# fasion-image-generator-project/discogan_modernized

Measured on AMD Instinct MI355X. Metric: images/sec per DiscoGAN train step, higher is better.
Workload: dtype f32x3; 1 GPU; tops2hanbok discogan image_size=512 batch_size=32 per GPU (BASELINE configs[3]); D,G,G cycle, fwd+bwd+Adam, dead backward work skipped; fp32-accurate conv products on the bf16 matrix path: every fp32 operand carried as three bf16 planes (24 significand bits), exact bf16 x bf16 products, fp32 accumulation (no operand rounding); image_size=512, global_batch=32, parallelism=dp1, hipgraph=True, hip_streams=2, allreduce_overlap=False

## Files before the change

discogan_modernized_amd/_lib.py:

```python
from __future__ import annotations

import ctypes as C
import os

_HERE = os.path.dirname(os.path.abspath(__file__))
LIB_PATH = os.environ.get("DG_LIB") or os.path.join(_HERE, "libdiscogan_hip.so")

_p = C.c_void_p
_i = C.c_int
_f = C.c_float
_d = C.c_double
_z = C.c_size_t
_l = C.c_int64

SIGNATURES = {
    "dg_version": (_i, []),
    "dg_build_flags": (_i, []),
    "dg_last_error": (C.c_char_p, []),
    "dg_set_option": (_i, [C.c_char_p, _i]),
    "dg_conv_workspace_bytes": (_z, [_i, _i, _i, _i, _i, _i, _i, _i]),
    "dg_conv_fwd": (_i, [_p, _p, _p, _i, _i, _i, _i, _i, _i, _i, _p, _z, _p]),
    "dg_conv_dgrad": (_i, [_p, _p, _p, _i, _i, _i, _i, _i, _i, _i, _p, _z, _p]),
    "dg_conv_wgrad": (_i, [_p, _p, _p, _i, _i, _i, _i, _i, _i, _i, _i, _p, _z, _p]),
    "dg_conv_workspace_bytes_p": (_z, [_i, _i, _i, _i, _i, _i, _i, _i, _i, _i]),
    "dg_conv_bnstats_rows_p": (_i, [_i, _i, _i, _i, _i, _i, _i, _i, _i]),
    "dg_conv_plan_splits_p": (_i, [_i, _i, _i, _i, _i, _i, _i, _i, _i, _i]),
    "dg_conv_plan_describe": (_i, [_i, _i, _i, _i, _i, _i, _i, _i, _i, _i, _i, _i, C.POINTER(_i), _i]),
    "dg_conv_fwd_g": (_i, [_i, _p, _p, _p, _i, _i, _i, _i, _i, _i, _i, _i, _i, _p, _z, _p, _z, _p]),
    "dg_conv_dgrad_g": (_i, [_i, _p, _p, _p, _i, _i, _i, _i, _i, _i, _i, _i, _i, _p, _z, _p, _z, _p]),
    "dg_conv_wgrad_g": (_i, [_i, _i, _p, _p, _p, _i, _i, _i, _i, _i, _i, _i, _i, _i, _i, _p, _z, _p]),
    "dg_conv4x4s2_c3_fwd_p": (_i, [_p, _p, _p, _i, _i, _i, _i, _i, _i, _f, _i, _p]),
    "dg_conv4x4s2_c3_dgrad_p": (_i, [_p, _i, _p, _p, _i, _i, _i, _i, _i, _i, _p, _z, _p]),
    "dg_c3_dgrad_act_ok": (_i, [_i, _i, _i, _i, _i]),
    "dg_conv4x4s2_c3_dgrad_act_p": (_i, [_p, _i, _p, _i, _f, _p, _p, _i, _i, _i, _i, _i, _i, _p, _z, _p]),
    "dg_conv4x4s2_c3_wgrad_p": (_i, [_p, _p, _i, _i, _f, _p, _p, _i, _i, _i, _i, _i, _i, _p, _z, _p]),
    "dg_conv4x4s2_c3_fwd_g": (_i, [_i, _p, _p, _p, _i, _i, _i, _i, _i, _f, _i, _p]),
    "dg_conv4x4s2_c3_dgrad_g": (_i, [_i, _p, _p, _p, _i, _i, _i, _i, _i, _i, _p]),
    "dg_conv4x4s2_c3_wgrad_g": (_i, [_i, _i, _p, _p, _i, _f, _p, _p, _i, _i, _i, _i, _i, _i, _p, _z, _p]),
    "dg_bn_train_stats_g": (_i, [_i, _i, _p, _i, _i, _f, _f, _p, _p, _p, _p, _p, _z, _p]),
    "dg_bn_act_fwd_g": (_i, [_i, _p, _p, _i, _i, _p, _p, _p, _i, _f, _p]),
    "dg_bn_act_bwd_g": (_i, [_i, _i, _p, _p, _p, _i, _i, _p, _p, _p, _i, _f, _p, _p, _i, _p, _z, _p]),
    "dg_act_fwd_g": (_i, [_i, _p, _p, _z, _i, _f, _p]),
    "dg_act_bwd_g": (_i, [_i, _p, _p, _p, _z, _i, _f, _p]),
    "dg_mse_fwd_g": (_i, [_i, _p, _p, _z, _p, _p, _z, _p]),
    "dg_mse_bwd_g": (_i, [_i, _p, _p, _z, _p, _p, _p]),
    "dg_bce_fwd_g": (_i, [_i, _p, _i, _p, _p, _p]),
    "dg_bce_bwd_g": (_i, [_i, _p, _i, _p, _p, _p, _p]),
    "dg_fm_fwd_g": (_i, [_i, _p, _p, _i, _z, _p, _p, _p, _z, _p]),
    "dg_fm_bwd_g": (_i, [_i, _p, _i, _z, _p, _p, _p, _p]),
    "dg_conv_fwd_bias_act": (_i, [_p, _p, _p, _p, _i, _i, _i, _i, _i, _i, _i, _i, _f, _p, _z, _p]),
    "dg_conv_dgrad_bias_act": (_i, [_p, _p, _p, _p, _i, _i, _i, _i, _i, _i, _i, _i, _f, _p, _z, _p]),
    "dg_conv_plan_splits": (_i, [_i, _i, _i, _i, _i, _i, _i, _i]),
    "dg_conv_bnstats_rows": (_i, [_i, _i, _i, _i, _i, _i, _i, _i]),
    "dg_conv_fwd_bnstats": (_i, [_p, _p, _p, _i, _i, _i, _i, _i, _p, _z, _p, _z, _p]),
    "dg_conv_dgrad_bnstats": (_i, [_p, _p, _p, _i, _i, _i, _i, _i, _p, _z, _p, _z, _p]),
    "dg_conv4x4s2_fwd": (_i, [_p, _p, _p, _i, _i, _i, _i, _i, _p, _z, _p]),
    "dg_conv4x4s2_dgrad": (_i, [_p, _p, _p, _i, _i, _i, _i, _i, _p, _z, _p]),
    "dg_conv4x4s2_wgrad": (_i, [_p, _p, _p, _i, _i, _i, _i, _i, _i, _p, _z, _p]),
    "dg_conv4x4_valid_fwd": (_i, [_p, _p, _p, _i, _i, _i, _p, _z, _p]),
    "dg_conv4x4_valid_dgrad": (_i, [_p, _p, _p, _i, _i, _i, _p, _z, _p]),
    "dg_conv4x4_valid_wgrad": (_i, [_p, _p, _p, _i, _i, _i, _i, _p, _z, _p]),
    "dg_convT4x4s2_fwd": (_i, [_p, _p, _p, _i, _i, _i, _i, _i, _p, _z, _p]),
    "dg_convT4x4s2_dgrad": (_i, [_p, _p, _p, _i, _i, _i, _i, _i, _p, _z, _p]),
    "dg_convT4x4s2_wgrad": (_i, [_p, _p, _p, _i, _i, _i, _i, _i, _i, _p, _z, _p]),
    "dg_convT4x4_1to4_fwd": (_i, [_p, _p, _p, _i, _i, _i, _p, _z, _p]),
    "dg_convT4x4_1to4_dgrad": (_i, [_p, _p, _p, _i, _i, _i, _p, _z, _p]),
    "dg_convT4x4_1to4_wgrad": (_i, [_p, _p, _p, _i, _i, _i, _i, _p, _z, _p]),
    "dg_conv4x4s2_c3_fwd": (_i, [_p, _p, _p, _i, _i, _i, _i, _i, _f, _p]),
    "dg_c3_dgrad_workspace_bytes": (_z, [_i]),
    "dg_conv4x4s2_c3_dgrad": (_i, [_p, _p, _p, _i, _i, _i, _i, _i, _p, _z, _p]),
    "dg_c3_wgrad_workspace_bytes": (_z, [_i, _i, _i, _i]),
    "dg_conv4x4s2_c3_wgrad": (_i, [_p, _p, _p, _i, _i, _i, _i, _i, _p, _z, _p]),
    "dg_conv4x4s2_c3_wgrad_act": (_i, [_p, _p, _i, _f, _p, _p, _i, _i, _i, _i, _i, _p, _z, _p]),
    "dg_bn_workspace_bytes": (_z, [_i, _i]),
    "dg_bn_train_stats": (_i, [_p, _i, _i, _f, _f, _p, _p, _p, _p, _p, _z, _p]),
    "dg_bn_partials_workspace_bytes": (_z, [_i, _i]),
    "dg_bn_stats_from_partials": (_i, [_p, _i, _i, _i, _f, _f, _p, _p, _p, _p, _p, _z, _p]),
    "dg_bn_act_fwd": (_i, [_p, _p, _i, _i, _p, _p, _p, _i, _f, _p]),
    "dg_bn_act_bwd": (_i, [_p, _p, _p, _i, _i, _p, _p, _p, _i, _f, _p, _p, _i, _p, _z, _p]),
    "dg_act_fwd": (_i, [_p, _p, _z, _i, _f, _p]),
    "dg_act_bwd": (_i, [_p, _p, _p, _z, _i, _f, _p]),
    "dg_loss_workspace_bytes": (_z, []),
    "dg_mse_fwd": (_i, [_p, _p, _z, _p, _p, _z, _p]),
    "dg_mse_bwd": (_i, [_p, _p, _z, _p, _p, _p]),
    "dg_bce_fwd": (_i, [_p, _i, _f, _p, _p, _z, _p]),
    "dg_bce_bwd": (_i, [_p, _i, _f, _p, _p, _p]),
    "dg_fm_workspace_bytes": (_z, [_i, _z]),
    "dg_fm_fwd": (_i, [_p, _p, _i, _z, _p, _p, _p, _z, _p]),
    "dg_fm_bwd": (_i, [_p, _i, _z, _p, _p, _p, _p]),
    "dg_debug_igemm_stamps": (_i, [_p, _z]),
    "dg_device_cu_count": (_i, []),
    "dg_loss_mix_fwd": (_i, [_p, _p, _i, _f, _i, _p]),
    "dg_loss_mix_bwd": (_i, [_p, _p, _i, _f, _i, _i, _p]),
    "dg_adam_advance": (_i, [_p, _d, _d, _d, _p]),
    "dg_adam_step_flat": (_i, [_p, _p, _p, _p, _z, _p, _f, _f, _f, _f, _f, _p]),
    "dg_ema_update_flat": (_i, [_p, _p, _z, _f, _p]),
    "dg_swap_flat": (_i, [_p, _p, _z, _p]),
    "dg_grad_stats_workspace_bytes": (_z, []),
    "dg_grad_sumsq_partial": (_i, [_p, _z, _p, _z, _i, C.POINTER(_i), _p]),
    "dg_grad_clip_finalize": (_i, [_p, _i, _d, _d, _i, _p, _p]),
    "dg_adam_advance_c": (_i, [_p, _d, _d, _d, _p, _p]),
    "dg_adam_step_flat_c": (_i, [_p, _p, _p, _p, _z, _p, _f, _f, _f, _f, _p, _p, _i, _z, _p]),
    "dg_bce_target_fwd": (_i, [_p, _p, _i, _p, _p]),
    "dg_bce_target_bwd": (_i, [_p, _p, _i, _p, _p, _p]),
    "dg_hinge_fwd": (_i, [_p, _p, _z, _f, _p, _p, _z, _p]),
    "dg_hinge_bwd": (_i, [_p, _p, _z, _f, _p, _p, _p]),
    "dg_dp_ready": (_i, [_p]),
    "dg_dp_unique_id_bytes": (_i, []),
    "dg_dp_get_unique_id": (_i, [_p, _z]),
    "dg_dp_init": (_i, [_i, _i, _p, _z]),
    "dg_dp_world_size": (_i, []),
    "dg_dp_rank": (_i, []),
    "dg_dp_allreduce_sum": (_i, [_p, _z, _p]),
    "dg_dp_allreduce_max": (_i, [_p, _z, _p]),
    "dg_dp_broadcast": (_i, [_p, _z, _i, _p]),
    "dg_dp_barrier": (_i, [_p, _p]),
    "dg_dp_destroy": (_i, []),
    "dg_u8hwc_to_f32chw": (_i, [_p, _p, _i, _i, _i, _i, _p]),
    "dg_image_prep": (_i, [_p, _p, _i, _i, _i, _i, _i, _i, _i, _i, _p]),
    "dg_sample_grid_u8": (_i, [_p, _i, _i, _i, _i, _i, _p, _p]),
    "dg_image_metrics_workspace_bytes": (_z, [_i, _i]),
    "dg_image_metrics": (_i, [_p, _p, _i, _i, _p, _p, _z, _p]),
    "dg_adam_step_flat_bf16": (_i, [_p, _p, _p, _p, _z, _p, _f, _f, _f, _f, _f, _p, _p]),
    "dg_f32_to_bf16": (_i, [_p, _p, _z, _p]),
    "dg_bn_act_fwd_bf16": (_i, [_p, _p, _p, _i, _i, _p, _p, _p, _i, _f, _p]),
    "dg_bn_act_bwd_bf16": (_i, [_p, _p, _p, _p, _i, _i, _p, _p, _p, _i, _f, _p, _p, _i, _p, _z, _p]),
    "dg_conv_bf16_operands_ok": (_i, [_i, _i, _i, _i, _i, _i, _i, _i]),
    "dg_f32_to_bf16x3": (_i, [_p, _p, _z, _z, _p]),
    "dg_adam_step_flat_x3": (_i, [_p, _p, _p, _p, _z, _p, _f, _f, _f, _f, _f, _p, _z, _p]),
    "dg_conv4x4s2_c3_fwd_x3": (_i, [_p, _p, _p, _p, _z, _i, _i, _i, _i, _i, _f, _p]),
    "dg_conv_x3_planes_ok": (_i, [_i, _i, _i, _i, _i, _i, _i, _i]),
    "dg_bn_act_fwd_x3": (_i, [_p, _p, _p, _z, _i, _i, _i, _p, _p, _p, _i, _f, _p]),
    "dg_bn_act_bwd_x3": (_i, [_p, _p, _p, _p, _z, _i, _i, _i, _p, _p, _p, _i, _f, _p, _p, _i, _p, _z, _p]),
    "dg_conv_x3_bnstats_rows": (_i, [_i, _i, _i, _i, _i, _i, _i, _i]),
    "dg_conv_fwd_x3": (_i, [_p, _l, _p, _l, _i, _p, _i, _i, _i, _i, _i, _i, _i, _p, _z, _p, _z, _p]),
    "dg_x3_transpose_planes": (_i, [_p, _p, _z, _p, _p, _p, _i, _p]),
    "dg_conv_dgrad_x3": (_i, [_p, _l, _i, _p, _l, _p, _i, _i, _i, _i, _i, _i, _i, _p, _z, _p, _z, _p]),
    "dg_conv_wgrad_x3": (_i, [_p, _l, _i, _p, _l, _p, _i, _i, _i, _i, _i, _i, _i, _i, _p, _z, _p]),
    "dg_conv_mixed_bnstats_rows": (_i, [_i, _i, _i, _i, _i, _i, _i, _i, _i, _i]),
    "dg_conv_fwd_mixed": (_i, [_p, _i, _p, _i, _p, _i, _i, _i, _i, _i, _i, _i, _i, _p, _z, _p, _z, _p]),
    "dg_conv_dgrad_mixed": (_i, [_p, _i, _p, _i, _p, _i, _i, _i, _i, _i, _i, _i, _i, _p, _z, _p, _z, _p]),
    "dg_bn_train_stats_t": (_i, [_p, _i, _i, _i, _f, _f, _p, _p, _p, _p, _p, _z, _p]),
    "dg_bn_act_fwd_t": (_i, [_p, _p, _i, _i, _i, _p, _p, _p, _i, _f, _p]),
    "dg_bn_act_bwd_t": (_i, [_p, _p, _p, _i, _i, _i, _p, _p, _p, _i, _f, _p, _p, _i, _p, _z, _p]),
    "dg_act_bwd_t": (_i, [_p, _p, _p, _i, _z, _i, _f, _p]),
    "dg_conv4x4s2_c3_fwd_t": (_i, [_p, _p, _p, _i, _i, _i, _i, _i, _i, _f, _p]),
    "dg_conv4x4s2_c3_dgrad_t": (_i, [_p, _i, _p, _p, _i, _i, _i, _i, _i, _p, _z, _p]),
    "dg_conv4x4s2_c3_wgrad_t": (_i, [_p, _p, _i, _i, _f, _p, _p, _i, _i, _i, _i, _i, _p, _z, _p]),
    "dg_fm_fwd_t": (_i, [_p, _p, _i, _i, _z, _p, _p, _p, _z, _p]),
    "dg_fm_bwd_t": (_i, [_p, _i, _z, _p, _p, _p, _i, _p]),
    "dg_conv_wgrad_mixed": (_i, [_p, _i, _p, _i, _p, _i, _i, _i, _i, _i, _i, _i, _i, _p, _z, _p]),
    "dg_nchw_to_nhwc": (_i, [_p, _p, _i, _i, _i, _i, _p]),
    "dg_nhwc_to_nchw": (_i, [_p, _p, _i, _i, _i, _i, _p]),
}

_lib = None


class DiscoganHipError(RuntimeError):
    pass


def load():
    global _lib
    if _lib is not None:
        return _lib
    if not os.path.exists(LIB_PATH):
        raise DiscoganHipError(
            f"{LIB_PATH} not found: the HIP kernel library is not built. "
            "Run `python -m discogan_modernized_amd.build` (hipcc --offload-arch=gfx950). "
            "There is no CPU fallback for the product path.")
    import torch
    lib = C.CDLL(LIB_PATH)
    for name, (res, args) in SIGNATURES.items():
        fn = getattr(lib, name)
        fn.restype = res
        fn.argtypes = args
    _lib = lib
    for key, val in os.environ.items():
        if key.startswith("DG_OPT_"):
            rc = lib.dg_set_option(key[7:].lower().encode(), int(val))
            if rc != 0:
                raise DiscoganHipError(f"bad option {key}: " + lib.dg_last_error().decode())
    return lib


def check(rc, what=""):
    if rc != 0:
# ... 7 lines not shown
```

discogan_modernized_amd/csrc/dg_common.h:

```cpp
#pragma once
#include <hip/hip_runtime.h>
#include <stdint.h>
#include <stdio.h>
#include <stdarg.h>
#include "../../include/discogan_hip.h"

typedef float f32x4 __attribute__((ext_vector_type(4)));
typedef float f32x16 __attribute__((ext_vector_type(16)));
typedef __bf16 dg_bf16x4_t __attribute__((ext_vector_type(4)));

extern thread_local char dg_err_buf[512];
int dg_fail(int code, const char* fmt, ...);

#define DG_CHECK_ARG(cond, ...)                                   \
    do {                                                          \
        if (!(cond)) return dg_fail(DG_ERR_INVALID, __VA_ARGS__); \
    } while (0)

#define DG_CHECK_LAUNCH(name)                                                                    \
    do {                                                                                         \
        hipError_t e__ = hipGetLastError();                                                      \
        if (e__ != hipSuccess) return dg_fail(DG_ERR_HIP, "%s: %s", name, hipGetErrorString(e__)); \
    } while (0)

static inline int dg_ilog2(int v) {
    int l = 0;
    while ((1 << l) < v) ++l;
    return l;
}
static inline bool dg_is_pow2(int v) { return v > 0 && (v & (v - 1)) == 0; }
static inline size_t dg_align_up(size_t v, size_t a) { return (v + a - 1) / a * a; }

int dg_get_option(int idx);
enum { DG_OPT_SPLITK = 0, DG_OPT_KT = 1, DG_OPT_TARGET_WGS = 2, DG_OPT_RESERVED = 3, DG_OPT_SPLIT_BELOW = 4, DG_OPT_POINTER_PATH = 5, DG_OPT_BF16 = 6, DG_OPT_DBG_ZERO = 7, DG_OPT_NO_DMA = 8, DG_OPT_DMA_MFMA = 9, DG_OPT_X3_MFMA = 10, DG_OPT_DGW_PERSIST = 11, DG_OPT_UNDERSTORY = 12, DG_OPT_BN_ITEMS = 13, DG_OPT_COUNT = 14 };
static inline int dg_resolve_prec(int prec) { return prec >= 0 ? prec : dg_get_option(DG_OPT_BF16); }
__attribute__((visibility("hidden"))) void dg_c3_fwd_tiled(const float* x_nchw, const float* w, float* y_nhwc, int N, int H, int W, int K, int act,
                                                           float slope, bool wide, hipStream_t st);

struct DgPtrs {
    const void* p[DG_MAX_GROUPS];
};
static inline DgPtrs dg_ptrs(const void* const* arr, int n) {
    DgPtrs r;
    for (int i = 0; i < DG_MAX_GROUPS; ++i) r.p[i] = (arr != nullptr && i < n) ? arr[i] : nullptr;
    return r;
}
static inline DgPtrs dg_ptrs1(const void* p0) {
    DgPtrs r;
    for (int i = 0; i < DG_MAX_GROUPS; ++i) r.p[i] = nullptr;
    r.p[0] = p0;
    return r;
}
template <typename T>
__device__ __forceinline__ T* dg_pick(const DgPtrs& t, int g) { return (T*)t.p[g]; }

__device__ __forceinline__ float dg_wave_sum(float v) {
#pragma unroll
    for (int off = 32; off > 0; off >>= 1) v += __shfl_down(v, off, 64);
    return v;
}
__device__ __forceinline__ double dg_wave_sum_d(double v) {
#pragma unroll
    for (int off = 32; off > 0; off >>= 1) v += __shfl_down(v, off, 64);
    return v;
}

__device__ __forceinline__ float dg_block_sum256(float v, float* red ) {
    v = dg_wave_sum(v);
    const int lane = threadIdx.x & 63, w = threadIdx.x >> 6;
    if (lane == 0) red[w] = v;
    __syncthreads();
    float r = 0.f;
    if (threadIdx.x == 0) r = red[0] + red[1] + red[2] + red[3];
    __syncthreads();
    return r;
}

__device__ __forceinline__ float dg_apply_act(float u, int act, float slope) {
    if (act == DG_ACT_LEAKY) return u > 0.f ? u : u * slope;
    if (act == DG_ACT_RELU) return u > 0.f ? u : 0.f;
    if (act == DG_ACT_SIGMOID) return 1.f / (1.f + __expf(-u));
    return u;
}

__device__ __forceinline__ void dg_split3(const f32x4& v, dg_bf16x4_t& hi, dg_bf16x4_t& mid, dg_bf16x4_t& lo) {
    hi = __builtin_convertvector(v, dg_bf16x4_t);
    const f32x4 r = v - __builtin_convertvector(hi, f32x4);
    mid = __builtin_convertvector(r, dg_bf16x4_t);
    lo = __builtin_convertvector(r - __builtin_convertvector(mid, f32x4), dg_bf16x4_t);
}
```

discogan_modernized_amd/csrc/edge.hip:

```cpp
#include "dg_common.h"
#include <type_traits>

__device__ float dg_zero_edge[64];

__device__ __forceinline__ int tap_of(int parity, int d) {
    if (parity == 0) return d == 0 ? 1 : (d == -1 ? 3 : -1);
    return d == 0 ? 2 : (d == 1 ? 0 : -1);
}

__global__ __launch_bounds__(256) void c3_dgrad_valu_kernel(const float* __restrict__ dy, const float* __restrict__ w,
                                                            float* __restrict__ dx, int N, int H, int W, int K,
                                                            int lgHo, int lgWo, int act) {
    const int Ho = H >> 1, Wo = W >> 1;
    const long nquad = (long)N * Ho * Wo;
    const long q = (long)blockIdx.x * 256 + threadIdx.x;
    if (q >= nquad) return;
    const int b = (int)(q & (Wo - 1)), a = (int)((q >> lgWo) & (Ho - 1)), n = (int)(q >> (lgWo + lgHo));
    float acc[3][2][2];
#pragma unroll
    for (int c = 0; c < 3; ++c) acc[c][0][0] = acc[c][0][1] = acc[c][1][0] = acc[c][1][1] = 0.f;
    const float* base = dy + ((long)(n * Ho + a) * Wo + b) * K;
    for (int k0 = 0; k0 < K; k0 += 4) {
        f32x4 g[3][3];
#pragma unroll
        for (int da = -1; da <= 1; ++da)
#pragma unroll
            for (int db = -1; db <= 1; ++db) {
                const bool ok = (unsigned)(a + da) < (unsigned)Ho && (unsigned)(b + db) < (unsigned)Wo;
                g[da + 1][db + 1] = ok ? *(const f32x4*)(base + (long)(da * Wo + db) * K + k0)
                                       : (f32x4){0.f, 0.f, 0.f, 0.f};
            }
#pragma unroll
        for (int kk = 0; kk < 4; ++kk) {
            const float* wk = w + (long)(k0 + kk) * 48;
#pragma unroll
            for (int c = 0; c < 3; ++c)
#pragma unroll
                for (int ph = 0; ph < 2; ++ph)
#pragma unroll
                    for (int ty = 0; ty < 2; ++ty) {
                        const int r = ph == 0 ? (ty == 0 ? 1 : 3) : (ty == 0 ? 2 : 0);
                        const int da = ph == 0 ? (ty == 0 ? 0 : -1) : (ty == 0 ? 0 : 1);
#pragma unroll
                        for (int pw = 0; pw < 2; ++pw)
#pragma unroll
                            for (int tx = 0; tx < 2; ++tx) {
                                const int s = pw == 0 ? (tx == 0 ? 1 : 3) : (tx == 0 ? 2 : 0);
                                const int db = pw == 0 ? (tx == 0 ? 0 : -1) : (tx == 0 ? 0 : 1);
                                acc[c][ph][pw] += g[da + 1][db + 1][kk] * wk[c * 16 + r * 4 + s];
                            }
                    }
        }
    }
#pragma unroll
    for (int c = 0; c < 3; ++c)
#pragma unroll
        for (int ph = 0; ph < 2; ++ph) {
            float v0 = acc[c][ph][0], v1 = acc[c][ph][1];
            if (act == DG_ACT_SIGMOID) {
                v0 = 1.f / (1.f + expf(-v0));
                v1 = 1.f / (1.f + expf(-v1));
            }
            *(float2*)(dx + ((long)(n * 3 + c) * H + 2 * a + ph) * W + 2 * b) = make_float2(v0, v1);
        }
}

#define CD_K 64
#define CD_TR 4
#define CD_TC 16
#define CD_PR (CD_TR + 2)
#define CD_PC (CD_TC + 2)
#define CD_LDP 66
#define CD_NK (9 * CD_K)

__global__ __launch_bounds__(256) void c3_wq_build_kernel(const float* __restrict__ w, float* __restrict__ wq) {
    const int e = blockIdx.x * 256 + threadIdx.x;
    if (e >= CD_NK * 16) return;
    const int col = e & 15, row = e >> 4;
    const int k = row & (CD_K - 1), nb = row >> 6;
    const int da = nb / 3 - 1, db = nb % 3 - 1;
    float v = 0.f;
    if (col < 12) {
        const int c = col >> 2, ph = (col >> 1) & 1, pw = col & 1;
        const int r = tap_of(ph, da), s = tap_of(pw, db);
        if (r >= 0 && s >= 0) v = w[(k * 3 + c) * 16 + r * 4 + s];
    }
    wq[e] = v;
}

#define CD_NV ((CD_PR * CD_PC * (CD_K / 4) + 255) / 256)
__global__ __launch_bounds__(256, 2) void c3_dgrad_mfma_kernel(const float* __restrict__ dy, const float* __restrict__ wq,
                                                               float* __restrict__ dx, int N, int H, int W, int act,
                                                               int tiles_r, int tiles_c, int ntiles) {
    __shared__ __attribute__((aligned(16))) float WqS[CD_NK * 16];
    __shared__ __attribute__((aligned(16))) float dyS[CD_PR * CD_PC * CD_LDP];
    __shared__ float outS[CD_TR][16 * 17];
    const int tid = threadIdx.x, lane = tid & 63, wave = tid >> 6;
    const int Ho = H >> 1, Wo = W >> 1;
    for (int e = tid; e < CD_NK * 4; e += 256) *(f32x4*)(WqS + e * 4) = *(const f32x4*)(wq + e * 4);

    f32x4 pre[CD_NV];
    auto prefetch = [&](int t) {
        const int tc = t % tiles_c, tr = (t / tiles_c) % tiles_r, n = t / (tiles_c * tiles_r);
        const int a0 = tr * CD_TR, b0 = tc * CD_TC;
#pragma unroll
        for (int i = 0; i < CD_NV; ++i) {
            const int idx = tid + i * 256;
            const int q4 = idx & (CD_K / 4 - 1), pix = idx >> 4;
            const int pr = pix / CD_PC, pc = pix - pr * CD_PC;
            const int a = a0 - 1 + pr, b = b0 - 1 + pc;
            const bool ok = idx < CD_PR * CD_PC * (CD_K / 4) && t < ntiles &&
                            (unsigned)a < (unsigned)Ho && (unsigned)b < (unsigned)Wo;
            pre[i] = ok ? *(const f32x4*)(dy + ((long)(n * Ho + a) * Wo + b) * CD_K + q4 * 4) : (f32x4){0.f, 0.f, 0.f, 0.f};
        }
    };
    const int bq = lane & 15, kk = lane >> 4;
    prefetch(blockIdx.x);
    for (int t = blockIdx.x; t < ntiles; t += gridDim.x) {
        const int tc = t % tiles_c, tr = (t / tiles_c) % tiles_r, n = t / (tiles_c * tiles_r);
        const int a0 = tr * CD_TR, b0 = tc * CD_TC;
        __syncthreads();
#pragma unroll
        for (int i = 0; i < CD_NV; ++i) {
            const int idx = tid + i * 256;
            if (idx < CD_PR * CD_PC * (CD_K / 4)) {
                float* d = dyS + (idx >> 4) * CD_LDP + (idx & (CD_K / 4 - 1)) * 4;
                *(float2*)d = make_float2(pre[i][0], pre[i][1]);
                *(float2*)(d + 2) = make_float2(pre[i][2], pre[i][3]);
            }
        }
        __syncthreads();
        prefetch(t + gridDim.x);
        f32x4 acc0 = {0.f, 0.f, 0.f, 0.f}, acc1 = {0.f, 0.f, 0.f, 0.f};
#pragma unroll
        for (int nb = 0; nb < 9; ++nb) {
            const int da = nb / 3 - 1, db = nb % 3 - 1;
            const float* ap = dyS + ((wave + 1 + da) * CD_PC + bq + 1 + db) * CD_LDP + kk;
            const float* bp = WqS + (nb * CD_K + kk) * 16 + bq;
#pragma unroll
            for (int ks = 0; ks < CD_K / 4; ks += 2) {
                acc0 = __builtin_amdgcn_mfma_f32_16x16x4f32(ap[ks * 4], bp[ks * 64], acc0, 0, 0, 0);
                acc1 = __builtin_amdgcn_mfma_f32_16x16x4f32(ap[ks * 4 + 4], bp[ks * 64 + 64], acc1, 0, 0, 0);
            }
        }
#pragma unroll
        for (int r = 0; r < 4; ++r) outS[wave][bq * 17 + kk * 4 + r] = acc0[r] + acc1[r];
        __syncthreads();
        const int a = a0 + wave;
        const int ph = lane >> 5, x = lane & 31;
        const int qd = x >> 1, pw = x & 1;
        if (a < Ho && b0 + qd < Wo) {
#pragma unroll
            for (int c = 0; c < 3; ++c) {
                float v = outS[wave][(c * 4 + ph * 2 + pw) * 17 + qd];
                if (act == DG_ACT_SIGMOID) v = 1.f / (1.f + expf(-v));
                dx[((long)(n * 3 + c) * H + 2 * a + ph) * W + 2 * b0 + x] = v;
            }
        }
    }
}

#define CS_TR 6
#define CS_TC 14
#define CS_PR (CS_TR + 2)
#define CS_PC 16
#define CS_LDP 52
template <bool IN16, bool MF16 = false, bool X3 = false, bool FACT = false>
__global__ __launch_bounds__(256, 2) void c3_dgrad_scatter_kernel(const DgPtrs dys, const DgPtrs ws_, const DgPtrs dxs, int N, int H, int W, int act,
                                                                  int tiles_r, int tiles_c, int ntiles, unsigned dybytes, const DgPtrs aos, float slope) {
    const float* __restrict__ dy = dg_pick<const float>(dys, blockIdx.y);
    const float* __restrict__ w = dg_pick<const float>(ws_, blockIdx.y);
    float* __restrict__ dx = dg_pick<float>(dxs, blockIdx.y);
    static_assert(!MF16 || IN16, "the bf16 MFMA form takes a bf16 dy");
    static_assert(!X3 || (!IN16 && !MF16), "the f32x3 form takes an fp32 dy");
    typedef __bf16 bf16x8_d __attribute__((ext_vector_type(8)));
    typedef float f32x8_d __attribute__((ext_vector_type(8)));
    __shared__ __attribute__((aligned(16))) float Ps[CS_PR * CS_PC * CS_LDP];
    const int tid = threadIdx.x, lane = tid & 63, wave = tid >> 6;
    const int p = lane & 15, kq = lane >> 4;
    const int Ho = H >> 1, Wo = W >> 1;
    float breg[3][(MF16 || X3) ? 1 : 16];
    bf16x8_d breg16[3][2];
    bf16x8_d breg3[X3 ? 3 : 1][3][2];
    auto split8 = [](const f32x8_d& v, bf16x8_d* pl) {
        pl[0] = __builtin_convertvector(v, bf16x8_d);
        const f32x8_d r1 = v - __builtin_convertvector(pl[0], f32x8_d);
        pl[1] = __builtin_convertvector(r1, bf16x8_d);
        pl[2] = __builtin_convertvector(r1 - __builtin_convertvector(pl[1], f32x8_d), bf16x8_d);
    };
#pragma unroll
    for (int blk = 0; blk < 3; ++blk) {
        if constexpr (X3) {
#pragma unroll
            for (int st = 0; st < 2; ++st) {
                f32x8_d t;
#pragma unroll
                for (int j = 0; j < 8; ++j) t[j] = w[(32 * st + 8 * kq + j) * 48 + blk * 16 + p];
                bf16x8_d pl[3];
                split8(t, pl);
#pragma unroll
                for (int q = 0; q < 3; ++q) breg3[q][blk][st] = pl[q];
            }
        } else if constexpr (MF16) {
#pragma unroll
            for (int st = 0; st < 2; ++st) {
                f32x8_d t;
#pragma unroll
                for (int j = 0; j < 8; ++j) t[j] = w[(32 * st + 8 * kq + j) * 48 + blk * 16 + p];
                breg16[blk][st] = __builtin_convertvector(t, bf16x8_d);
            }
        } else {
#pragma unroll
            for (int s = 0; s < 16; ++s) breg[blk][s] = w[(16 * kq + s) * 48 + blk * 16 + p];
        }
    }
    const __amdgpu_buffer_rsrc_t rdy = __builtin_amdgcn_make_buffer_rsrc((void*)dy, 0, (int)dybytes, 0x00020000);
    const __amdgpu_buffer_rsrc_t rao = __builtin_amdgcn_make_buffer_rsrc((void*)(FACT ? dg_pick<const float>(aos, blockIdx.y) : dy), 0, (int)dybytes, 0x00020000);
    constexpr int OOR = (int)0x80000000;
    f32x4 areg[2][2][4];
    f32x4 oreg[FACT ? 2 : 1][4];
    auto apply_act = [&](int set) {
        if constexpr (FACT) {
#pragma unroll
            for (int g = 0; g < 2; ++g)
#pragma unroll
                for (int j = 0; j < (IN16 ? 2 : 4); ++j)
#pragma unroll
                    for (int e = 0; e < 4; ++e) {
                        if constexpr (IN16) {
                            const unsigned dv = __float_as_uint(areg[set][g][j][e]), ov = __float_as_uint(oreg[g][j][e]);
                            float d0 = __builtin_bit_cast(float, dv << 16), d1 = __builtin_bit_cast(float, dv & 0xffff0000u);
                            d0 = __builtin_bit_cast(float, ov << 16) > 0.f ? d0 : d0 * slope;
                            d1 = __builtin_bit_cast(float, ov & 0xffff0000u) > 0.f ? d1 : d1 * slope;
                            typedef __bf16 bf16x2_a __attribute__((ext_vector_type(2)));
                            typedef float f32x2_a __attribute__((ext_vector_type(2)));
                            areg[set][g][j][e] = __uint_as_float(__builtin_bit_cast(unsigned, __builtin_convertvector((f32x2_a){d0, d1}, bf16x2_a)));
                        } else {
                            const float d = areg[set][g][j][e];
                            areg[set][g][j][e] = oreg[g][j][e] > 0.f ? d : d * slope;
                        }
                    }
        }
    };
    auto fetch = [&](int t, int set) {
        const int tc = t % tiles_c, tr = (t / tiles_c) % tiles_r, n = t / (tiles_c * tiles_r);
#pragma unroll
        for (int g = 0; g < 2; ++g) {
            const int a = tr * CS_TR - 1 + wave + 4 * g, b = tc * CS_TC - 1 + p;
            const bool ok = t < ntiles && (unsigned)a < (unsigned)Ho && (unsigned)b < (unsigned)Wo;
            const int off = ok ? (((n * Ho + a) * Wo + b) * CD_K + ((MF16 || X3) ? 8 : 16) * kq) * (IN16 ? 2 : 4) : OOR;
#pragma unroll
            for (int j = 0; j < (IN16 ? 2 : 4); ++j) {
                const int o = off + (X3 ? 128 * (j >> 1) + 16 * (j & 1) : (MF16 ? 64 : 16) * j);
                areg[set][g][j] = __builtin_bit_cast(f32x4, __builtin_amdgcn_raw_buffer_load_b128(rdy, o, 0, 0));
                if constexpr (FACT) oreg[g][j] = __builtin_bit_cast(f32x4, __builtin_amdgcn_raw_buffer_load_b128(rao, o, 0, 0));
            }
        }
    };
    fetch(blockIdx.x, 0);
    apply_act(0);
    auto tile = [&](auto SB, int t) {
        constexpr int S = decltype(SB)::value;
        const int tc = t % tiles_c, tr = (t / tiles_c) % tiles_r, n = t / (tiles_c * tiles_r);
        const int a0 = tr * CS_TR, b0 = tc * CS_TC;
        fetch(t + gridDim.x, S ^ 1);
        f32x4 acc[2][3];
#pragma unroll
        for (int g = 0; g < 2; ++g)
#pragma unroll
            for (int blk = 0; blk < 3; ++blk) acc[g][blk] = (f32x4){0.f, 0.f, 0.f, 0.f};
        if constexpr (X3) {
            constexpr int PA[6] = {2, 0, 1, 1, 0, 0}, PB[6] = {0, 2, 1, 0, 1, 0};
#pragma unroll
            for (int st = 0; st < 2; ++st)
#pragma unroll
                for (int g = 0; g < 2; ++g) {
                    const f32x4 v0 = areg[S][g][2 * st], v1 = areg[S][g][2 * st + 1];
                    bf16x8_d apl[3];
                    split8((f32x8_d){v0[0], v0[1], v0[2], v0[3], v1[0], v1[1], v1[2], v1[3]}, apl);
#pragma unroll
                    for (int blk = 0; blk < 3; ++blk)
#pragma unroll
                        for (int q = 0; q < 6; ++q)
                            acc[g][blk] = __builtin_amdgcn_mfma_f32_16x16x32_bf16(apl[PA[q]], breg3[PB[q]][blk][st], acc[g][blk], 0, 0, 0);
                }
        } else if constexpr (MF16) {
#pragma unroll
            for (int st = 0; st < 2; ++st)
#pragma unroll
                for (int g = 0; g < 2; ++g)
#pragma unroll
                    for (int blk = 0; blk < 3; ++blk)
                        acc[g][blk] = __builtin_amdgcn_mfma_f32_16x16x32_bf16(__builtin_bit_cast(bf16x8_d, areg[S][g][st]), breg16[blk][st],
                                                                              acc[g][blk], 0, 0, 0);
        } else
#pragma unroll
        for (int s = 0; s < 16; ++s)
#pragma unroll
            for (int g = 0; g < 2; ++g)
#pragma unroll
                for (int blk = 0; blk < 3; ++blk)
                {
                    float av;
                    if constexpr (IN16) {
                        const float fv = areg[S][g][s >> 3][(s >> 1) & 3];
                        const unsigned wv = __float_as_uint(fv);
                        av = __builtin_bit_cast(float, (s & 1) ? (wv & 0xffff0000u) : (wv << 16));
                    } else {
                        av = areg[S][g][s >> 2][s & 3];
                    }
                    acc[g][blk] = __builtin_amdgcn_mfma_f32_16x16x4f32(av, breg[blk][s], acc[g][blk], 0, 0, 0);
                }
        __syncthreads();
#pragma unroll
        for (int g = 0; g < 2; ++g)
#pragma unroll
            for (int blk = 0; blk < 3; ++blk)
#pragma unroll
                for (int j = 0; j < 4; ++j) Ps[((wave + 4 * g) * CS_PC + 4 * kq + j) * CS_LDP + blk * 16 + p] = acc[g][blk][j];
        __syncthreads();
        for (int e = tid; e < 3 * 2 * CS_TR * 2 * CS_TC; e += 256) {
            const int xx = e % (2 * CS_TC), yy = (e / (2 * CS_TC)) % (2 * CS_TR), c = e / (4 * CS_TR * CS_TC);
            const int y = 2 * a0 + yy, x = 2 * b0 + xx;
            const int ph = yy & 1, pw = xx & 1, la = (yy >> 1) + 1, lb = (xx >> 1) + 1;
            const int ra2 = la - 1 + 2 * ph, rr1 = 1 + ph, rr2 = 3 - 3 * ph;
            const int cb2 = lb - 1 + 2 * pw, ss1 = 1 + pw, ss2 = 3 - 3 * pw;
            const float* pc = Ps + c * 16;
            float v = pc[(la * CS_PC + lb) * CS_LDP + rr1 * 4 + ss1] + pc[(la * CS_PC + cb2) * CS_LDP + rr1 * 4 + ss2] +
                      pc[(ra2 * CS_PC + lb) * CS_LDP + rr2 * 4 + ss1] + pc[(ra2 * CS_PC + cb2) * CS_LDP + rr2 * 4 + ss2];
            if (act == DG_ACT_SIGMOID) v = 1.f / (1.f + expf(-v));
            if (y < H && x < W) dx[((long)(n * 3 + c) * H + y) * W + x] = v;
        }
        apply_act(S ^ 1);
    };
    for (int t = blockIdx.x; t < ntiles; t += 2 * gridDim.x) {
        tile(std::integral_constant<int, 0>{}, t);
        if (t + (int)gridDim.x < ntiles) tile(std::integral_constant<int, 1>{}, t + gridDim.x);
    }
}

extern "C" size_t dg_c3_dgrad_workspace_bytes(int K) { return K == CD_K ? (size_t)CD_NK * 16 * sizeof(float) : 0; }

using C3Yes = std::true_type;
using C3No = std::false_type;
template <typename F> static void c3_with_flag(bool b, F&& f) { if (b) f(C3Yes{}); else f(C3No{}); }
template <typename F> static void c3_with_fwd_act(int act, F&& f) {
    if (act == DG_ACT_LEAKY) f(std::integral_constant<int, DG_ACT_LEAKY>{});
    else if (act == DG_ACT_RELU) f(std::integral_constant<int, DG_ACT_RELU>{});
    else f(std::integral_constant<int, DG_ACT_NONE>{});
}
#define C3_CHECK_PREC(who, prec) DG_CHECK_ARG((prec) >= DG_PREC_DEFAULT && (prec) <= DG_PREC_F32X3, who ": prec=%d", prec)

struct C3Dgrad {
    const char* who;
    int groups;
    bool grouped;
    const void *const *dy, *const *w;
    void* const* dx;
    int dy_bf16, N, H, W, K, act, prec;
    const void* act_out;
    float slope;
    void* ws;
    size_t ws_bytes;
    hipStream_t st;
};
static C3Dgrad c3_dgrad_call(const char* who, const void* const* dy, int dy_bf16, const float* const* w, float* const* dx, int N, int H, int W, int K,
                             int act, int prec, void* ws, size_t ws_bytes, dg_stream_t stream) {
    C3Dgrad c = C3Dgrad();
    c.who = who; c.groups = 1; c.dy = dy; c.dy_bf16 = dy_bf16; c.w = (const void* const*)w; c.dx = (void* const*)dx;
    c.N = N; c.H = H; c.W = W; c.K = K; c.act = act; c.prec = dg_resolve_prec(prec);
    c.ws = ws; c.ws_bytes = ws_bytes; c.st = (hipStream_t)stream;
    return c;
}
static int c3_dgrad(const C3Dgrad& c);
extern "C" int dg_conv4x4s2_c3_dgrad(const float* dy_nhwc, const float* w, float* dx_nchw, int N, int H, int W, int K,
                                     int act, void* ws, size_t ws_bytes, dg_stream_t stream) {
    return c3_dgrad(c3_dgrad_call("dg_conv4x4s2_c3_dgrad", (const void* const*)&dy_nhwc, 0, &w, &dx_nchw, N, H, W, K, act, DG_PREC_DEFAULT, ws, ws_bytes,
                                  stream));
}
extern "C" int dg_conv4x4s2_c3_dgrad_t(const void* dy_nhwc, int dy_bf16, const float* w, float* dx_nchw, int N, int H, int W, int K,
                                       int act, void* ws, size_t ws_bytes, dg_stream_t stream) {
    return c3_dgrad(c3_dgrad_call("dg_conv4x4s2_c3_dgrad_t", &dy_nhwc, dy_bf16, &w, &dx_nchw, N, H, W, K, act, DG_PREC_DEFAULT, ws, ws_bytes, stream));
}
extern "C" int dg_conv4x4s2_c3_dgrad_p(const void* dy_nhwc, int dy_bf16, const float* w, float* dx_nchw, int N, int H, int W, int K,
                                       int act, int prec, void* ws, size_t ws_bytes, dg_stream_t stream) {
    C3_CHECK_PREC("dg_conv4x4s2_c3_dgrad_p", prec);
    return c3_dgrad(c3_dgrad_call("dg_conv4x4s2_c3_dgrad_p", &dy_nhwc, dy_bf16, &w, &dx_nchw, N, H, W, K, act, prec, ws, ws_bytes, stream));
}
extern "C" int dg_conv4x4s2_c3_dgrad_act_p(const void* dy_nhwc, int dy_bf16, const void* act_out, int in_act, float slope, const float* w, float* dx_nchw,
                                           int N, int H, int W, int K, int act, int prec, void* ws, size_t ws_bytes, dg_stream_t stream) {
    C3_CHECK_PREC("dg_conv4x4s2_c3_dgrad_act_p", prec);
    DG_CHECK_ARG(act_out && in_act == DG_ACT_LEAKY, "dg_conv4x4s2_c3_dgrad_act_p: needs the saved output of a fused LeakyReLU (in_act=%d)", in_act);
    C3Dgrad c = c3_dgrad_call("dg_conv4x4s2_c3_dgrad_act_p", &dy_nhwc, dy_bf16, &w, &dx_nchw, N, H, W, K, act, prec, ws, ws_bytes, stream);
    c.act_out = act_out; c.slope = slope;
    return c3_dgrad(c);
}
extern "C" int dg_conv4x4s2_c3_dgrad_g(int groups, const float* const* dy_nhwc, const float* const* w, float* const* dx_nchw, int N, int H, int W, int K,
                                       int act, int prec, dg_stream_t stream) {
    C3_CHECK_PREC("dg_conv4x4s2_c3_dgrad_g", prec);
    C3Dgrad c = c3_dgrad_call("dg_conv4x4s2_c3_dgrad_g", (const void* const*)dy_nhwc, 0, w, dx_nchw, N, H, W, K, act, prec, nullptr, 0, stream);
    c.groups = groups; c.grouped = true;
    return c3_dgrad(c);
}

static bool c3_dgrad_scatter_fits(int N, int H, int W, int K, int dy_bf16) {
    return K == CD_K && N >= 1 && (long)N * (H / 2) * (W / 2) * CD_K * (dy_bf16 ? 2 : 4) < (1L << 31);
}
extern "C" int dg_c3_dgrad_act_ok(int N, int H, int W, int K, int dy_bf16) {
    return c3_dgrad_scatter_fits(N, H, W, K, dy_bf16) && dg_get_option(DG_OPT_KT) != 16 ? 1 : 0;
}
enum C3DgradForm { C3_DGRAD_SCATTER, C3_DGRAD_GATHER, C3_DGRAD_VALU };
static C3DgradForm c3_dgrad_form(const C3Dgrad& c) {
    if (!c3_dgrad_scatter_fits(c.N, c.H, c.W, c.K, c.dy_bf16)) return C3_DGRAD_VALU;
    return dg_get_option(DG_OPT_KT) != 16 ? C3_DGRAD_SCATTER : C3_DGRAD_GATHER;
}
static int c3_dgrad(const C3Dgrad& c) {
    const int N = c.N, H = c.H, W = c.W, K = c.K, Ho = H / 2, Wo = W / 2;
    DG_CHECK_ARG(c.groups >= 1 && c.groups <= DG_MAX_GROUPS && c.dy && c.w && c.dx, "%s: bad group / null table", c.who);
    for (int i = 0; i < c.groups; ++i) DG_CHECK_ARG(c.dy[i] && c.w[i] && c.dx[i], "%s: null pointer", c.who);
    DG_CHECK_ARG(!c.grouped || (K == CD_K && dg_get_option(DG_OPT_KT) != 16), "%s: the grouped form is the scatter kernel (K == 64, option kt != 16)", c.who);
    DG_CHECK_ARG(!c.dy_bf16 || (K == CD_K && dg_get_option(DG_OPT_KT) != 16), "%s: a bf16 dy needs K == 64 (scatter form)", c.who);
    DG_CHECK_ARG(N >= 1 && K >= 4 && K % 4 == 0, "%s: bad N/K (%d,%d)", c.who, N, K);
    DG_CHECK_ARG(dg_is_pow2(H) && dg_is_pow2(W) && H >= 2 && W >= 2, "%s: H,W must be powers of two", c.who);
    DG_CHECK_ARG(c.act == DG_ACT_NONE || c.act == DG_ACT_SIGMOID, "%s: bad act %d", c.who, c.act);
    DG_CHECK_ARG((long)N * 3 * H * W < (1L << 31), "%s: tensor too large", c.who);
    const C3DgradForm form = c3_dgrad_form(c);
    if (form != C3_DGRAD_SCATTER) {
        DG_CHECK_ARG(c.groups == 1 && !c.act_out, "%s: several problems and the fused form are the scatter kernel (K == 64, dy under 2^31 bytes, option kt != 16)",
                     c.who);
        DG_CHECK_ARG(!c.dy_bf16, "%s: the VALU form reads an fp32 dy (a bf16 dy of %ld bytes is past the scatter form's 2^31)", c.who, (long)N * Ho * Wo * K * 2);
    }
    switch (form) {
    case C3_DGRAD_SCATTER: {
        const int tiles_r = (Ho + CS_TR - 1) / CS_TR, tiles_c = (Wo + CS_TC - 1) / CS_TC;
        const long ntiles = (long)N * tiles_r * tiles_c;
        const dim3 grid((unsigned)(ntiles < 512 ? ntiles : 512), c.groups);
        const DgPtrs pd = dg_ptrs(c.dy, c.groups), pw = dg_ptrs(c.w, c.groups), px = dg_ptrs(c.dx, c.groups);
        const DgPtrs pa = dg_ptrs1(c.act_out ? c.act_out : c.dy[0]);
        const unsigned dyb = (unsigned)((long)N * Ho * Wo * CD_K * (c.dy_bf16 ? 2 : 4));
        auto scatter = [&](auto IN16, auto MF16, auto X3) {
            c3_with_flag(c.act_out != nullptr, [&](auto FACT) {
                hipLaunchKernelGGL((c3_dgrad_scatter_kernel<decltype(IN16)::value, decltype(MF16)::value, decltype(X3)::value, decltype(FACT)::value>), grid,
                                   dim3(256), 0, c.st, pd, pw, px, N, H, W, c.act, tiles_r, tiles_c, (int)ntiles, dyb, pa, c.slope);
            });
        };
        if (c.dy_bf16 && c.prec == DG_PREC_BF16) scatter(C3Yes{}, C3Yes{}, C3No{});
        else if (c.dy_bf16) scatter(C3Yes{}, C3No{}, C3No{});
        else if (c.prec == DG_PREC_F32X3) scatter(C3No{}, C3No{}, C3Yes{});
        else scatter(C3No{}, C3No{}, C3No{});
        break;
    }
    case C3_DGRAD_GATHER: {
        const int tiles_r = (Ho + CD_TR - 1) / CD_TR, tiles_c = (Wo + CD_TC - 1) / CD_TC;
        const long ntiles = (long)N * tiles_r * tiles_c;
        if (c.ws == nullptr || c.ws_bytes < dg_c3_dgrad_workspace_bytes(K))
            return dg_fail(DG_ERR_WORKSPACE, "%s: workspace %zu < %zu", c.who, c.ws_bytes, dg_c3_dgrad_workspace_bytes(K));
        hipLaunchKernelGGL(c3_wq_build_kernel, dim3((CD_NK * 16 + 255) / 256), dim3(256), 0, c.st, (const float*)c.w[0], (float*)c.ws);
        DG_CHECK_LAUNCH("c3_wq_build");
        hipLaunchKernelGGL(c3_dgrad_mfma_kernel, dim3((unsigned)(ntiles < 512 ? ntiles : 512)), dim3(256), 0, c.st, (const float*)c.dy[0], (const float*)c.ws,
                           (float*)c.dx[0], N, H, W, c.act, tiles_r, tiles_c, (int)ntiles);
        break;
    }
    case C3_DGRAD_VALU: {
        const long nquad = (long)N * Ho * Wo;
        hipLaunchKernelGGL(c3_dgrad_valu_kernel, dim3((unsigned)((nquad + 255) / 256)), dim3(256), 0, c.st, (const float*)c.dy[0], (const float*)c.w[0],
                           (float*)c.dx[0], N, H, W, K, dg_ilog2(Ho), dg_ilog2(Wo), c.act);
        break;
    }
    }
    DG_CHECK_LAUNCH(c.who);
    return DG_OK;
}

#define CF_K 64
#define CF_S 24
template <int ACT, bool OUT16>
__global__ __launch_bounds__(256, 2) void c3_fwd_mfma_kernel(const DgPtrs xs, const DgPtrs ws_, const DgPtrs ys, int N, int H, int W, int lgHo, int lgWo,
                                                             long npix, int ngroups, float slope, int xbytes) {
    const float* __restrict__ x = dg_pick<const float>(xs, blockIdx.y);
    const float* __restrict__ w = dg_pick<const float>(ws_, blockIdx.y);
    float* __restrict__ y = dg_pick<float>(ys, blockIdx.y);
    const int lane = threadIdx.x & 63;
    const int p = lane & 31, h = lane >> 5;
    const int Ho = H >> 1, Wo = W >> 1;
    const int wave = blockIdx.x * 4 + (threadIdx.x >> 6), nwaves = gridDim.x * 4;
    const float* const zp = dg_zero_edge;
    __shared__ float wS[CF_K * 49];
    for (int e = threadIdx.x; e < CF_K * 48; e += 256) wS[(e / 48) * 49 + e % 48] = w[e];
    __syncthreads();
    float wb[2][CF_S];
#pragma unroll
    for (int nb = 0; nb < 2; ++nb)
#pragma unroll
        for (int s = 0; s < CF_S; ++s) {
            const int c = s >> 3, r = (s >> 1) & 3, q = 2 * (s & 1) + h;
            wb[nb][s] = wS[(OUT16 ? 2 * p + nb : nb * 32 + p) * 49 + c * 16 + r * 4 + q];
        }
    float a[2][CF_S];
    const __amdgpu_buffer_rsrc_t rx = __builtin_amdgcn_make_buffer_rsrc((void*)x, 0, xbytes, 0x00020000);
    const int HW4 = H * W * 4;
    constexpr int BIG = 0x40000000;
    auto gather = [&](int g, float* dst) {
        const int pix = g * 32 + p;
        const bool okp = g < ngroups && pix < (int)npix;
        const int ox = pix & (Wo - 1), oy = (pix >> lgWo) & (Ho - 1), n = pix >> (lgWo + lgHo);
        const int base = n * 3 * HW4;
        int colb[2];
#pragma unroll
        for (int j = 0; j < 2; ++j) {
            const int ix = 2 * ox - 1 + 2 * j + h;
            colb[j] = (unsigned)ix < (unsigned)W ? ix * 4 : BIG;
        }
#pragma unroll
        for (int r = 0; r < 4; ++r) {
            const int iy = 2 * oy - 1 + r;
            const int rowb = (okp && (unsigned)iy < (unsigned)H) ? base + iy * W * 4 : BIG;
#pragma unroll
            for (int j = 0; j < 2; ++j) {
                const int voff = rowb + colb[j];
#pragma unroll
                for (int c = 0; c < 3; ++c)
                    dst[c * 8 + r * 2 + j] = __builtin_bit_cast(float, __builtin_amdgcn_raw_buffer_load_b32(rx, voff, c * HW4, 0));
            }
        }
    };
    int g = wave;
    if (g < ngroups) gather(g, a[0]);
    auto body = [&](auto PB, int gcur) {
        constexpr int P = decltype(PB)::value;
        gather(gcur + nwaves, a[P ^ 1]);
        f32x16 acc0 = {0.f}, acc1 = {0.f};
#pragma unroll
        for (int s = 0; s < CF_S; ++s) {
            acc0 = __builtin_amdgcn_mfma_f32_32x32x2f32(a[P][s], wb[0][s], acc0, 0, 0, 0);
            acc1 = __builtin_amdgcn_mfma_f32_32x32x2f32(a[P][s], wb[1][s], acc1, 0, 0, 0);
        }
        const long pix0 = (long)gcur * 32;
        if constexpr (OUT16) {
            typedef __bf16 bf16x2_e __attribute__((ext_vector_type(2)));
            typedef float f32x2_e __attribute__((ext_vector_type(2)));
            unsigned* o16 = (unsigned*)((__bf16*)y + (pix0 + h * 4) * CF_K + 2 * p);
            const bool whole = pix0 + 32 <= npix;
#pragma unroll
            for (int v = 0; v < 16; ++v) {
                const int i = (v >> 2) * 8 + (v & 3);
                const f32x2_e pr = {dg_apply_act(acc0[v], ACT, slope), dg_apply_act(acc1[v], ACT, slope)};
                if (whole || pix0 + h * 4 + i < npix)
                    o16[i * (CF_K / 2)] = __builtin_bit_cast(unsigned, __builtin_convertvector(pr, bf16x2_e));
            }
            return;
        }
        float* o = y + (pix0 + h * 4) * CF_K + p;
        if (pix0 + 32 <= npix) {
#pragma unroll
            for (int v = 0; v < 16; ++v) {
                const int i = (v >> 2) * 8 + (v & 3);
                o[i * CF_K] = dg_apply_act(acc0[v], ACT, slope);
                o[i * CF_K + 32] = dg_apply_act(acc1[v], ACT, slope);
            }
        } else {
#pragma unroll
            for (int v = 0; v < 16; ++v) {
                const int i = (v >> 2) * 8 + (v & 3);
                if (pix0 + h * 4 + i < npix) {
                    o[i * CF_K] = dg_apply_act(acc0[v], ACT, slope);
                    o[i * CF_K + 32] = dg_apply_act(acc1[v], ACT, slope);
                }
            }
        }
    };
    for (; g < ngroups; g += 2 * nwaves) {
        body(std::integral_constant<int, 0>{}, g);
        if (g + nwaves < ngroups) body(std::integral_constant<int, 1>{}, g + nwaves);
    }
}

typedef __bf16 bf16x8_e __attribute__((ext_vector_type(8)));
typedef float f32x8_e __attribute__((ext_vector_type(8)));
typedef float f32x2_g __attribute__((ext_vector_type(2)));
template <int ACT, bool OUT16, bool X3 = false, bool PL = false>
__global__ __launch_bounds__(256, 2) void c3_fwd_bf16mfma_kernel(const DgPtrs xs, const DgPtrs ws_, const DgPtrs ys, int N, int H, int W, int lgHo, int lgWo,
                                                                 long npix, int ngroups, float slope, int xbytes,
                                                                 __bf16* __restrict__ planes = nullptr, long pstride = 0) {
    const float* __restrict__ x = dg_pick<const float>(xs, blockIdx.y);
    const float* __restrict__ w = dg_pick<const float>(ws_, blockIdx.y);
    float* __restrict__ y = dg_pick<float>(ys, blockIdx.y);
    static_assert(!PL || (X3 && !OUT16), "planes are written by the f32x3 form with an fp32 output");
    const int lane = threadIdx.x & 63;
    const int p = lane & 31, h = lane >> 5;
    const int Ho = H >> 1, Wo = W >> 1;
    const int wave = blockIdx.x * 4 + (threadIdx.x >> 6), nwaves = gridDim.x * 4;
    constexpr int NPL = X3 ? 3 : 1;
    bf16x8_e wb[NPL][2][3];
    auto split8 = [](const f32x8_e& v, bf16x8_e* pl) {
        pl[0] = __builtin_convertvector(v, bf16x8_e);
        if constexpr (X3) {
            const f32x8_e r1 = v - __builtin_convertvector(pl[0], f32x8_e);
            pl[1] = __builtin_convertvector(r1, bf16x8_e);
            pl[2] = __builtin_convertvector(r1 - __builtin_convertvector(pl[1], f32x8_e), bf16x8_e);
// ... 67 lines not shown
            for (int v = 0; v < 16; ++v) {
                const int i = (v >> 2) * 8 + (v & 3);
                const f32x2_e pr = {dg_apply_act(acc0[v], ACT, slope), dg_apply_act(acc1[v], ACT, slope)};
                if (whole || pix0 + h * 4 + i < npix)
                    o16[i * (CF_K / 2)] = __builtin_bit_cast(unsigned, __builtin_convertvector(pr, bf16x2_e));
            }
        } else if constexpr (PL) {
            typedef __bf16 bf16x2_p __attribute__((ext_vector_type(2)));
            typedef float f32x2_p __attribute__((ext_vector_type(2)));
            float* o = y + (pix0 + h * 4) * CF_K + 2 * p;
            __bf16* pb = planes + (pix0 + h * 4) * CF_K + 2 * p;
#pragma unroll
            for (int v = 0; v < 16; ++v) {
                const int i = (v >> 2) * 8 + (v & 3);
                if (whole || pix0 + h * 4 + i < npix) {
                    const f32x2_p pr = {dg_apply_act(acc0[v], ACT, slope), dg_apply_act(acc1[v], ACT, slope)};
                    *(f32x2_p*)(o + i * CF_K) = pr;
                    const bf16x2_p hi2 = __builtin_convertvector(pr, bf16x2_p);
                    const f32x2_p r1 = pr - __builtin_convertvector(hi2, f32x2_p);
                    const bf16x2_p mid2 = __builtin_convertvector(r1, bf16x2_p);
                    const bf16x2_p lo2 = __builtin_convertvector(r1 - __builtin_convertvector(mid2, f32x2_p), bf16x2_p);
                    *(bf16x2_p*)(pb + i * CF_K) = hi2;
                    *(bf16x2_p*)(pb + pstride + i * CF_K) = mid2;
                    *(bf16x2_p*)(pb + 2 * pstride + i * CF_K) = lo2;
                }
            }
        } else {
            float* o = y + (pix0 + h * 4) * CF_K + p;
#pragma unroll
            for (int v = 0; v < 16; ++v) {
                const int i = (v >> 2) * 8 + (v & 3);
                if (whole || pix0 + h * 4 + i < npix) {
                    o[i * CF_K] = dg_apply_act(acc0[v], ACT, slope);
                    o[i * CF_K + 32] = dg_apply_act(acc1[v], ACT, slope);
                }
            }
        }
    };
    for (; g < ngroups; g += 2 * nwaves) {
        body(std::integral_constant<int, 0>{}, g);
        if (g + nwaves < ngroups) body(std::integral_constant<int, 1>{}, g + nwaves);
    }
}

struct C3Fwd {
    const char* who;
    int groups;
    bool streaming_only;
    const void *const *x, *const *w;
    void* const* y;
    void* planes;
    size_t plane_elems;
    int y_bf16, N, H, W, K, act, prec;
    float slope;
    hipStream_t st;
};
static C3Fwd c3_fwd_call(const char* who, const float* const* x, const float* const* w, void* const* y, int y_bf16, int N, int H, int W, int K, int act,
                         float slope, int prec, dg_stream_t stream) {
    C3Fwd c = C3Fwd();
    c.who = who; c.groups = 1; c.x = (const void* const*)x; c.w = (const void* const*)w; c.y = y; c.y_bf16 = y_bf16;
    c.N = N; c.H = H; c.W = W; c.K = K; c.act = act; c.slope = slope; c.prec = dg_resolve_prec(prec); c.st = (hipStream_t)stream;
    return c;
}
static int c3_fwd(const C3Fwd& c);
extern "C" int dg_conv4x4s2_c3_fwd(const float* x_nchw, const float* w, float* y_nhwc, int N, int H, int W, int K,
                                   int act, float slope, dg_stream_t stream) {
    return c3_fwd(c3_fwd_call("dg_conv4x4s2_c3_fwd", &x_nchw, &w, (void* const*)&y_nhwc, 0, N, H, W, K, act, slope, DG_PREC_DEFAULT, stream));
}
extern "C" int dg_conv4x4s2_c3_fwd_t(const float* x_nchw, const float* w, void* y_nhwc, int y_bf16, int N, int H, int W, int K,
                                     int act, float slope, dg_stream_t stream) {
    return c3_fwd(c3_fwd_call("dg_conv4x4s2_c3_fwd_t", &x_nchw, &w, &y_nhwc, y_bf16, N, H, W, K, act, slope, DG_PREC_DEFAULT, stream));
}
extern "C" int dg_conv4x4s2_c3_fwd_p(const float* x_nchw, const float* w, void* y_nhwc, int y_bf16, int N, int H, int W, int K,
                                     int act, float slope, int prec, dg_stream_t stream) {
    C3_CHECK_PREC("dg_conv4x4s2_c3_fwd_p", prec);
    return c3_fwd(c3_fwd_call("dg_conv4x4s2_c3_fwd_p", &x_nchw, &w, &y_nhwc, y_bf16, N, H, W, K, act, slope, prec, stream));
}
extern "C" int dg_conv4x4s2_c3_fwd_g(int groups, const float* const* x_nchw, const float* const* w, float* const* y_nhwc, int N, int H, int W, int K,
                                     int act, float slope, int prec, dg_stream_t stream) {
    C3_CHECK_PREC("dg_conv4x4s2_c3_fwd_g", prec);
    C3Fwd c = c3_fwd_call("dg_conv4x4s2_c3_fwd_g", x_nchw, w, (void* const*)y_nhwc, 0, N, H, W, K, act, slope, prec, stream);
    c.groups = groups; c.streaming_only = true;
    return c3_fwd(c);
}
extern "C" int dg_conv4x4s2_c3_fwd_x3(const float* x_nchw, const float* w, float* y_nhwc, void* y_planes, size_t plane_elems, int N, int H,
                                      int W, int K, int act, float slope, dg_stream_t stream) {
    DG_CHECK_ARG(y_planes, "dg_conv4x4s2_c3_fwd_x3: null pointer");
    C3Fwd c = c3_fwd_call("dg_conv4x4s2_c3_fwd_x3", &x_nchw, &w, (void* const*)&y_nhwc, 0, N, H, W, K, act, slope, DG_PREC_F32X3, stream);
    c.planes = y_planes; c.plane_elems = plane_elems; c.streaming_only = true;
    return c3_fwd(c);
}

enum C3FwdForm { C3_FWD_MFMA_F32, C3_FWD_MFMA_BF16, C3_FWD_X3, C3_FWD_X3_PLANES, C3_FWD_TILED_NARROW, C3_FWD_TILED_WIDE };
static C3FwdForm c3_fwd_form(const C3Fwd& c) {
    const bool streams = c.K == CF_K && (long)c.N * 3 * c.H * c.W * 4 < (1L << 30) && (long)c.N * (c.H / 2) * (c.W / 2) < (1L << 30) &&
                         (dg_get_option(DG_OPT_KT) != 16 || c.planes);
    if (!streams) return c.K <= 64 ? C3_FWD_TILED_NARROW : C3_FWD_TILED_WIDE;
    if (c.planes) return C3_FWD_X3_PLANES;
    if (c.prec == DG_PREC_F32X3 && !c.y_bf16) return C3_FWD_X3;
    return c.prec == DG_PREC_BF16 ? C3_FWD_MFMA_BF16 : C3_FWD_MFMA_F32;
}
static int c3_fwd(const C3Fwd& c) {
    const int N = c.N, H = c.H, W = c.W, K = c.K, Ho = H / 2, Wo = W / 2;
    DG_CHECK_ARG(c.groups >= 1 && c.groups <= DG_MAX_GROUPS && c.x && c.w && c.y, "%s: bad group / null table", c.who);
    for (int i = 0; i < c.groups; ++i) DG_CHECK_ARG(c.x[i] && c.w[i] && c.y[i], "%s: null pointer", c.who);
    DG_CHECK_ARG(N >= 1 && K >= 4 && K % 4 == 0, "%s: bad N/K (%d,%d)", c.who, N, K);
    DG_CHECK_ARG(dg_is_pow2(H) && dg_is_pow2(W) && H >= 2 && W >= 2, "%s: H,W must be powers of two", c.who);
    DG_CHECK_ARG((long)N * 3 * H * W < (1L << 31), "%s: tensor too large", c.who);
    DG_CHECK_ARG(c.act == DG_ACT_NONE || c.act == DG_ACT_LEAKY || c.act == DG_ACT_RELU, "%s: bad act %d", c.who, c.act);
    const long npix = (long)N * Ho * Wo;
    const C3FwdForm form = c3_fwd_form(c);
    if (form == C3_FWD_TILED_NARROW || form == C3_FWD_TILED_WIDE) {
        DG_CHECK_ARG(!c.streaming_only, "%s: only the streaming kernel has this form: it needs K == 64 (K=%d) and tensors below 1 GiB%s", c.who, K,
                     c.planes ? "" : ", and option kt = 16 asks for the tiled kernel");
        DG_CHECK_ARG(!c.y_bf16, "%s: a bf16 output needs K == 64 and tensors < 1 GiB (the streaming kernel)", c.who);
        dg_c3_fwd_tiled((const float*)c.x[0], (const float*)c.w[0], (float*)c.y[0], N, H, W, K, c.act, c.slope, form == C3_FWD_TILED_WIDE, c.st);
        DG_CHECK_LAUNCH(c.who);
        return DG_OK;
    }
    if (c.planes)
        DG_CHECK_ARG(c.plane_elems >= (size_t)npix * CF_K && c.plane_elems % 8 == 0, "%s: plane distance %zu for %ld elements", c.who, c.plane_elems, npix * CF_K);
    const long ngroups = (npix + 31) / 32;
    long per = 32;
    while (form != C3_FWD_X3_PLANES && per > 4 && ((ngroups + per - 1) / per) * c.groups < 256) per >>= 1;
    long wgs = (ngroups + per - 1) / per;
    if (wgs > 4096) wgs = 4096;
    const dim3 grid((unsigned)wgs, c.groups);
    const DgPtrs px = dg_ptrs(c.x, c.groups), pw = dg_ptrs(c.w, c.groups), py = dg_ptrs(c.y, c.groups);
    const int lgHo = dg_ilog2(Ho), lgWo = dg_ilog2(Wo), xbytes = (int)((long)N * 3 * H * W * 4);
    auto mfma_f32 = [&](auto O16) {
        c3_with_fwd_act(c.act, [&](auto ACT) {
            static const hipError_t once = hipFuncSetAttribute((const void*)c3_fwd_mfma_kernel<decltype(ACT)::value, decltype(O16)::value>,
                                                               hipFuncAttributeMaxDynamicSharedMemorySize, 96 * 1024);
            (void)once;
            hipLaunchKernelGGL((c3_fwd_mfma_kernel<decltype(ACT)::value, decltype(O16)::value>), grid, dim3(256), 96 * 1024, c.st, px, pw, py, N, H, W,
                               lgHo, lgWo, npix, (int)ngroups, c.slope, xbytes);
        });
    };
    auto mfma_bf16 = [&](auto O16, auto X3, auto PL) {
        c3_with_fwd_act(c.act, [&](auto ACT) {
            hipLaunchKernelGGL((c3_fwd_bf16mfma_kernel<decltype(ACT)::value, decltype(O16)::value, decltype(X3)::value, decltype(PL)::value>), grid, dim3(256), 0,
                               c.st, px, pw, py, N, H, W, lgHo, lgWo, npix, (int)ngroups, c.slope, xbytes, (__bf16*)c.planes, (long)c.plane_elems);
        });
    };
    if (form == C3_FWD_X3_PLANES) mfma_bf16(C3No{}, C3Yes{}, C3Yes{});
    else if (form == C3_FWD_X3) mfma_bf16(C3No{}, C3Yes{}, C3No{});
    else if (form == C3_FWD_MFMA_BF16) { if (c.y_bf16) mfma_bf16(C3Yes{}, C3No{}, C3No{}); else mfma_bf16(C3No{}, C3No{}, C3No{}); }
    else { if (c.y_bf16) mfma_f32(C3Yes{}); else mfma_f32(C3No{}); }
    DG_CHECK_LAUNCH(c.who);
    return DG_OK;
}

#define CW_B 8
template <bool BUF, bool FACT, bool IN16 = false>
__global__ __launch_bounds__(256, 2) void c3_wgrad_mfma_kernel(const DgPtrs dys, const DgPtrs xs, const DgPtrs parts, int N, int H, int W, int K,
                                                               int lgHo, int lgWo, long npix, int pix_per_wave,
                                                               const DgPtrs act_outs, float slope) {
    const float* __restrict__ dy = dg_pick<const float>(dys, blockIdx.z);
    const float* __restrict__ x = dg_pick<const float>(xs, blockIdx.z);
    float* __restrict__ part = dg_pick<float>(parts, blockIdx.z);
    const float* __restrict__ act_out = dg_pick<const float>(act_outs, blockIdx.z);
    const int tid = threadIdx.x, lane = tid & 63, wave = tid >> 6;
    const int l31 = lane & 31, lh = lane >> 5;
    const int Ho = H >> 1, Wo = W >> 1;
    const int kg = blockIdx.y;
    const float* const zp = dg_zero_edge;
    f32x16 acc[2][2];
#pragma unroll
    for (int i = 0; i < 2; ++i)
#pragma unroll
        for (int j = 0; j < 2; ++j)
#pragma unroll
            for (int r = 0; r < 16; ++r) acc[i][j][r] = 0.f;
    int jr[2], js[2];
    long joff[2];
    bool jok[2];
#pragma unroll
    for (int jn = 0; jn < 2; ++jn) {
        const int j = jn * 32 + l31;
        jok[jn] = j < 48;
        const int c = (j >> 4) % 3;
        jr[jn] = (j >> 2) & 3;
        js[jn] = j & 3;
        joff[jn] = ((long)c * H + jr[jn]) * W + js[jn];
    }
    const long wave_id = (long)blockIdx.x * 4 + wave;
    const long p_begin = wave_id * pix_per_wave;
    const long p_end = min(npix, p_begin + pix_per_wave);
    const float* dyk = dy + kg * 64 + l31;

    float fa[2][CW_B][2], fb[2][CW_B][2];
    constexpr int BIG = 0x40000000;
    static_assert(!IN16 || BUF, "bf16 operands: buffer path only");
    const __amdgpu_buffer_rsrc_t rdy = __builtin_amdgcn_make_buffer_rsrc((void*)dy, 0, BUF ? (int)(npix * K * (IN16 ? 2 : 4)) : 0, 0x00020000);
    const __amdgpu_buffer_rsrc_t rao = __builtin_amdgcn_make_buffer_rsrc((void*)(FACT ? act_out : dy), 0, BUF ? (int)(npix * K * (IN16 ? 2 : 4)) : 0, 0x00020000);
    const __amdgpu_buffer_rsrc_t rx = __builtin_amdgcn_make_buffer_rsrc((void*)x, 0, BUF ? N * 3 * H * W * 4 : 0, 0x00020000);
    auto bload = [](const __amdgpu_buffer_rsrc_t& r, int off) {
        return __builtin_bit_cast(float, __builtin_amdgcn_raw_buffer_load_b32(r, off, 0, 0));
    };
    auto load_batch = [&](int set, long p0) {
#pragma unroll
        for (int st = 0; st < CW_B; ++st) {
            if constexpr (BUF) {
                const int pp = (int)p0 + 2 * st + lh;
                const bool pok = pp < (int)p_end;
                const int ox = pp & (Wo - 1), oy = (pp >> lgWo) & (Ho - 1), n = pp >> (lgWo + lgHo);
                const int iy0 = 2 * oy - 1, ix0 = 2 * ox - 1;
                const int xb = (n * 3 * H + iy0) * W + ix0;
                float a0, a1;
                if constexpr (IN16) {
                    const int aoff = pok ? (pp * K + kg * 64 + 2 * l31) * 2 : BIG;
                    const unsigned wv = __builtin_bit_cast(unsigned, bload(rdy, aoff));
                    a0 = __builtin_bit_cast(float, wv << 16);
                    a1 = __builtin_bit_cast(float, wv & 0xffff0000u);
                    if constexpr (FACT) {
                        const unsigned ov = __builtin_bit_cast(unsigned, bload(rao, aoff));
                        a0 = __builtin_bit_cast(float, ov << 16) > 0.f ? a0 : a0 * slope;
                        a1 = __builtin_bit_cast(float, ov & 0xffff0000u) > 0.f ? a1 : a1 * slope;
                    }
                } else {
                const int aoff = pok ? (pp * K + kg * 64 + l31) * 4 : BIG;
                a0 = bload(rdy, aoff);
                a1 = bload(rdy, aoff + 128);
                if constexpr (FACT) {
                    const float o0 = bload(rao, aoff), o1 = bload(rao, aoff + 128);
                    a0 = o0 > 0.f ? a0 : a0 * slope;
                    a1 = o1 > 0.f ? a1 : a1 * slope;
                }
                }
                fa[set][st][0] = a0;
                fa[set][st][1] = a1;
#pragma unroll
                for (int jn = 0; jn < 2; ++jn) {
                    const bool ok = pok && jok[jn] && (unsigned)(iy0 + jr[jn]) < (unsigned)H && (unsigned)(ix0 + js[jn]) < (unsigned)W;
                    fb[set][st][jn] = bload(rx, ok ? (xb + (int)joff[jn]) * 4 : BIG);
                }
            } else {
                const long pp = p0 + 2 * st + lh;
                const bool pok = pp < p_end;
                const int ox = (int)(pp & (Wo - 1)), oy = (int)((pp >> lgWo) & (Ho - 1)), n = (int)(pp >> (lgWo + lgHo));
                const int iy0 = 2 * oy - 1, ix0 = 2 * ox - 1;
                const long xb = ((long)n * 3 * H + iy0) * W + ix0;
                const float* ap = pok ? dyk + pp * K : zp;
                float a0 = ap[0], a1 = ap[32];
                if constexpr (FACT) {
                    const float* op = pok ? act_out + kg * 64 + l31 + pp * K : zp;
                    const float o0 = op[0], o1 = op[32];
                    a0 = o0 > 0.f ? a0 : a0 * slope;
                    a1 = o1 > 0.f ? a1 : a1 * slope;
                }
                fa[set][st][0] = a0;
                fa[set][st][1] = a1;
#pragma unroll
                for (int jn = 0; jn < 2; ++jn) {
                    const bool ok = pok && jok[jn] && (unsigned)(iy0 + jr[jn]) < (unsigned)H && (unsigned)(ix0 + js[jn]) < (unsigned)W;
                    const float* bp = ok ? x + xb + joff[jn] : zp;
                    fb[set][st][jn] = *bp;
                }
            }
        }
    };
    auto mma_batch = [&](int set) {
#pragma unroll
        for (int st = 0; st < CW_B; ++st)
#pragma unroll
            for (int i = 0; i < 2; ++i)
#pragma unroll
                for (int jn = 0; jn < 2; ++jn)
                    acc[i][jn] = __builtin_amdgcn_mfma_f32_32x32x2f32(fa[set][st][i], fb[set][st][jn], acc[i][jn], 0, 0, 0);
    };
    load_batch(0, p_begin);
    for (long p0 = p_begin; p0 < p_end; p0 += 4 * CW_B) {
        load_batch(1, p0 + 2 * CW_B);
        mma_batch(0);
        load_batch(0, p0 + 4 * CW_B);
        mma_batch(1);
    }
    __shared__ float slabS[4][64 * 48];
#pragma unroll
    for (int i = 0; i < 2; ++i)
#pragma unroll
        for (int r = 0; r < 16; ++r) {
            const int rho = (r & 3) + 8 * (r >> 2) + 4 * lh;
            const int k = IN16 ? 2 * rho + i : i * 32 + rho;
#pragma unroll
            for (int jn = 0; jn < 2; ++jn) {
                const int j = jn * 32 + l31;
                if (j < 48) slabS[wave][k * 48 + j] = acc[i][jn][r];
            }
        }
    __syncthreads();
    float* slab = part + ((long)blockIdx.x * K + kg * 64) * 48;
    for (int e = tid; e < 64 * 48; e += 256) slab[e] = ((slabS[0][e] + slabS[1][e]) + slabS[2][e]) + slabS[3][e];
}

typedef __bf16 bf16x8_w __attribute__((ext_vector_type(8)));
typedef float f32x8_w __attribute__((ext_vector_type(8)));
typedef unsigned u32x4_w __attribute__((ext_vector_type(4)));
template <bool FACT>
__global__ __launch_bounds__(256, 2) void c3_wgrad_bf16mfma_kernel(const float* __restrict__ dy, const float* __restrict__ x,
                                                                   float* __restrict__ part, int N, int H, int W, int K,
                                                                   int lgHo, int lgWo, long npix, int pix_per_wave,
                                                                   const float* __restrict__ act_out, float slope) {
    const int tid = threadIdx.x, lane = tid & 63, wave = tid >> 6;
    const int l31 = lane & 31, lh = lane >> 5;
    const int Ho = H >> 1, Wo = W >> 1;
    const int kg = blockIdx.y;
    f32x16 acc[2][2];
#pragma unroll
    for (int i = 0; i < 2; ++i)
#pragma unroll
        for (int j = 0; j < 2; ++j)
#pragma unroll
            for (int r = 0; r < 16; ++r) acc[i][j][r] = 0.f;
    int jr[2], js[2], joff[2];
    bool jok[2];
#pragma unroll
    for (int jn = 0; jn < 2; ++jn) {
        const int j = jn * 32 + l31;
        jok[jn] = j < 48;
        const int c = (j >> 4) % 3;
        jr[jn] = (j >> 2) & 3;
        js[jn] = j & 3;
        joff[jn] = (c * H + jr[jn]) * W + js[jn];
    }
    const long wave_id = (long)blockIdx.x * 4 + wave;
    const long p_begin = wave_id * pix_per_wave;
    const long p_end = min(npix, p_begin + pix_per_wave);
    constexpr int BIG = 0x40000000;
    const __amdgpu_buffer_rsrc_t rdy = __builtin_amdgcn_make_buffer_rsrc((void*)dy, 0, (int)(npix * K * 2), 0x00020000);
    const __amdgpu_buffer_rsrc_t rao = __builtin_amdgcn_make_buffer_rsrc((void*)(FACT ? act_out : dy), 0, (int)(npix * K * 2), 0x00020000);
    const __amdgpu_buffer_rsrc_t rx = __builtin_amdgcn_make_buffer_rsrc((void*)x, 0, N * 3 * H * W * 4, 0x00020000);
    auto bload = [](const __amdgpu_buffer_rsrc_t& r, int off) -> unsigned {
        return (unsigned)__builtin_amdgcn_raw_buffer_load_b32(r, off, 0, 0);
    };
    unsigned wa[2][8], wo[2][FACT ? 8 : 1];
    float fb[2][2][8];
    auto load_batch = [&](int set, long p0) {
#pragma unroll
        for (int t = 0; t < 8; ++t) {
            const int pp = (int)p0 + 8 * lh + t;
            const bool pok = pp < (int)p_end;
            const int ox = pp & (Wo - 1), oy = (pp >> lgWo) & (Ho - 1), n = pp >> (lgWo + lgHo);
            const int iy0 = 2 * oy - 1, ix0 = 2 * ox - 1;
            const int xb = (n * 3 * H + iy0) * W + ix0;
            const int aoff = pok ? (pp * K + kg * 64 + 2 * l31) * 2 : BIG;
            wa[set][t] = bload(rdy, aoff);
            if constexpr (FACT) wo[set][t] = bload(rao, aoff);
#pragma unroll
            for (int jn = 0; jn < 2; ++jn) {
                const bool ok = pok && jok[jn] && (unsigned)(iy0 + jr[jn]) < (unsigned)H && (unsigned)(ix0 + js[jn]) < (unsigned)W;
                fb[set][jn][t] = __builtin_bit_cast(float, bload(rx, ok ? (xb + joff[jn]) * 4 : BIG));
            }
        }
    };
    auto mma_batch = [&](int set) {
        unsigned w8[8];
#pragma unroll
        for (int t = 0; t < 8; ++t) {
            unsigned wv = wa[set][t];
            if constexpr (FACT) {
                const unsigned ov = wo[set][t];
                float a0 = __builtin_bit_cast(float, wv << 16), a1 = __builtin_bit_cast(float, wv & 0xffff0000u);
                a0 = __builtin_bit_cast(float, ov << 16) > 0.f ? a0 : a0 * slope;
                a1 = __builtin_bit_cast(float, ov & 0xffff0000u) > 0.f ? a1 : a1 * slope;
                typedef __bf16 bf16x2_w __attribute__((ext_vector_type(2)));
                typedef float f32x2_w __attribute__((ext_vector_type(2)));
                wv = __builtin_bit_cast(unsigned, __builtin_convertvector((f32x2_w){a0, a1}, bf16x2_w));
            }
            w8[t] = wv;
        }
        bf16x8_w fa[2], fbv[2];
        u32x4_w ev, od;
#pragma unroll
        for (int u = 0; u < 4; ++u) {
            ev[u] = __builtin_amdgcn_perm(w8[2 * u + 1], w8[2 * u], 0x05040100u);
            od[u] = __builtin_amdgcn_perm(w8[2 * u + 1], w8[2 * u], 0x07060302u);
        }
        fa[0] = __builtin_bit_cast(bf16x8_w, ev);
        fa[1] = __builtin_bit_cast(bf16x8_w, od);
#pragma unroll
        for (int jn = 0; jn < 2; ++jn) {
            f32x8_w t8;
#pragma unroll
            for (int t = 0; t < 8; ++t) t8[t] = fb[set][jn][t];
            fbv[jn] = __builtin_convertvector(t8, bf16x8_w);
        }
#pragma unroll
        for (int i = 0; i < 2; ++i)
#pragma unroll
            for (int jn = 0; jn < 2; ++jn) acc[i][jn] = __builtin_amdgcn_mfma_f32_32x32x16_bf16(fa[i], fbv[jn], acc[i][jn], 0, 0, 0);
    };
    load_batch(0, p_begin);
    for (long p0 = p_begin; p0 < p_end; p0 += 32) {
        load_batch(1, p0 + 16);
        mma_batch(0);
        load_batch(0, p0 + 32);
        mma_batch(1);
    }
    __shared__ float slabS[4][64 * 48];
#pragma unroll
    for (int i = 0; i < 2; ++i)
#pragma unroll
        for (int r = 0; r < 16; ++r) {
            const int rho = (r & 3) + 8 * (r >> 2) + 4 * lh;
            const int k = 2 * rho + i;
#pragma unroll
            for (int jn = 0; jn < 2; ++jn) {
                const int j = jn * 32 + l31;
                if (j < 48) slabS[wave][k * 48 + j] = acc[i][jn][r];
            }
        }
    __syncthreads();
    float* slab = part + ((long)blockIdx.x * K + kg * 64) * 48;
    for (int e = tid; e < 64 * 48; e += 256) slab[e] = ((slabS[0][e] + slabS[1][e]) + slabS[2][e]) + slabS[3][e];
}

#define CWL_WOMAX 256
template <typename F>
__device__ __forceinline__ void c3_static_for4(F&& f) {
    f(std::integral_constant<int, 0>{});
    f(std::integral_constant<int, 1>{});
    f(std::integral_constant<int, 2>{});
    f(std::integral_constant<int, 3>{});
}
template <bool FACT, bool X3 = false>
__global__ __launch_bounds__(256, X3 ? 1 : 2) void c3_wgrad_lds_kernel(const DgPtrs dys, const DgPtrs xs, const DgPtrs parts, int N, int H, int W, int K,
                                                              long npix, int rows_per_wg, const DgPtrs act_outs, float slope) {
    const float* __restrict__ dy = dg_pick<const float>(dys, blockIdx.z);
    const float* __restrict__ x = dg_pick<const float>(xs, blockIdx.z);
    float* __restrict__ part = dg_pick<float>(parts, blockIdx.z);
    const float* __restrict__ act_out = dg_pick<const float>(act_outs, blockIdx.z);
    constexpr int ROWE = CWL_WOMAX + 8;
    typedef typename std::conditional<X3, float, __bf16>::type ET;
    __shared__ __attribute__((aligned(16))) ET img[2][4][12][ROWE];
    const int tid = threadIdx.x, lane = tid & 63, wave = tid >> 6;
    const int l31 = lane & 31, lh = lane >> 5;
    const int Ho = H >> 1, Wo = W >> 1;
    const int kg = blockIdx.y;
    f32x16 acc[2][2];
#pragma unroll
    for (int i = 0; i < 2; ++i)
#pragma unroll
        for (int j = 0; j < 2; ++j)
#pragma unroll
            for (int r = 0; r < 16; ++r) acc[i][j][r] = 0.f;
    int jrow[2], jarr[2];
    bool jok[2];
#pragma unroll
    for (int jn = 0; jn < 2; ++jn) {
        const int j = jn * 32 + l31;
        jok[jn] = j < 48;
        const int jj = jok[jn] ? j : 0;
        jarr[jn] = jj & 3;
        jrow[jn] = (jj >> 4) * 4 + ((jj >> 2) & 3);
    }
    const int nrows = N * Ho;
    const int u0 = blockIdx.x * rows_per_wg, u1 = min(nrows, u0 + rows_per_wg);
    constexpr int BIG = 0x40000000;
    constexpr int EB = X3 ? 4 : 2;
    const __amdgpu_buffer_rsrc_t rdy = __builtin_amdgcn_make_buffer_rsrc((void*)dy, 0, (int)(npix * K * EB), 0x00020000);
    const __amdgpu_buffer_rsrc_t rao = __builtin_amdgcn_make_buffer_rsrc((void*)(FACT ? act_out : dy), 0, (int)(npix * K * EB), 0x00020000);
    auto bload = [](const __amdgpu_buffer_rsrc_t& r, int off) -> unsigned {
        return (unsigned)__builtin_amdgcn_raw_buffer_load_b32(r, off, 0, 0);
    };
    typedef float f32x2_w __attribute__((ext_vector_type(2)));
    auto bload2 = [](const __amdgpu_buffer_rsrc_t& r, int off) -> f32x2_w {
        return __builtin_bit_cast(f32x2_w, __builtin_amdgcn_raw_buffer_load_b64(r, off, 0, 0));
    };
    const int wq = W >> 2, chunks = 12 * wq;
    f32x4 sv[6];
    auto stage_load = [&](int u) {
        const int n = u / Ho, oy = u - n * Ho;
#pragma unroll
        for (int k = 0; k < 6; ++k) {
            const int e = tid + 256 * k;
            const int rowi = e / wq, m = e - rowi * wq;
            const int c = rowi >> 2, r = rowi & 3;
            const int iy = 2 * oy - 1 + r;
            sv[k] = (f32x4){0.f, 0.f, 0.f, 0.f};
            if (e < chunks && (unsigned)iy < (unsigned)H) sv[k] = *(const f32x4*)(x + ((long)(n * 3 + c) * H + iy) * W + 4 * m);
        }
    };
    auto stage_store = [&](int st) {
#pragma unroll
        for (int k = 0; k < 6; ++k) {
            const int e = tid + 256 * k;
            if (e >= chunks) continue;
            const int rowi = e / wq, m = e - rowi * wq;
            typedef ET etx4_s __attribute__((ext_vector_type(4)));
            typedef ET etx2_s __attribute__((ext_vector_type(2)));
            const etx4_s b = __builtin_convertvector(sv[k], etx4_s);
            ET* E = &img[st][1][rowi][0];
            ET* O = &img[st][2][rowi][0];
            ET* O0 = &img[st][0][rowi][0];
            ET* E1 = &img[st][3][rowi][0];
            *(etx2_s*)(E + 2 * m) = (etx2_s){b[0], b[2]};
            *(etx2_s*)(O + 2 * m) = (etx2_s){b[1], b[3]};
            O0[2 * m + 1] = b[1];
            if (2 * m + 2 < Wo) O0[2 * m + 2] = b[3];
            E1[2 * m] = b[2];
            if (m > 0) E1[2 * m - 1] = b[0];
            if (m == 0) O0[0] = (ET)0.f;
            if (2 * m + 2 == Wo) E1[Wo - 1] = (ET)0.f;
        }
    };
    constexpr int NSET = X3 ? 4 : 2;
    unsigned wa[2][X3 ? 1 : 8], wo[2][(FACT && !X3) ? 8 : 1];
    f32x2_w fa2[NSET][X3 ? 8 : 1], fo2[NSET][(FACT && X3) ? 8 : 1];
    const int nbatch = Wo >> 4;
    auto load_a = [&](int set, int u, int b) {
#pragma unroll
        for (int t = 0; t < 8; ++t) {
            const int pp = u * Wo + 16 * b + 8 * lh + t;
            const int aoff = (u < u1 && b < nbatch) ? (pp * K + kg * 64 + 2 * l31) * EB : BIG;
            if constexpr (X3) {
                fa2[set][t] = bload2(rdy, aoff);
                if constexpr (FACT) fo2[set][t] = bload2(rao, aoff);
            } else {
                wa[set][t] = bload(rdy, aoff);
                if constexpr (FACT) wo[set][t] = bload(rao, aoff);
            }
        }
    };
    typedef __bf16 bf16x8_l __attribute__((ext_vector_type(8)));
    typedef unsigned u32x4_l __attribute__((ext_vector_type(4)));
    typedef float f32x8_l __attribute__((ext_vector_type(8)));
    auto split8 = [](const f32x8_l& v, bf16x8_l* pl) {
        pl[0] = __builtin_convertvector(v, bf16x8_l);
        const f32x8_l r1 = v - __builtin_convertvector(pl[0], f32x8_l);
        pl[1] = __builtin_convertvector(r1, bf16x8_l);
        pl[2] = __builtin_convertvector(r1 - __builtin_convertvector(pl[1], f32x8_l), bf16x8_l);
    };
    auto mma_x3 = [&](int set, int st, int b) {
        if constexpr (X3) {
            f32x8_l a0, a1;
#pragma unroll
            for (int t = 0; t < 8; ++t) {
                f32x2_w v = fa2[set][t];
                if constexpr (FACT) {
                    const f32x2_w o = fo2[set][t];
                    v[0] = o[0] > 0.f ? v[0] : v[0] * slope;
                    v[1] = o[1] > 0.f ? v[1] : v[1] * slope;
                }
                a0[t] = v[0];
                a1[t] = v[1];
            }
            bf16x8_l pa0[3], pa1[3];
            split8(a0, pa0);
            split8(a1, pa1);
            constexpr int PA[6] = {2, 0, 1, 1, 0, 0}, PB[6] = {0, 2, 1, 0, 1, 0};
#pragma unroll
            for (int jn = 0; jn < 2; ++jn) {
                const float* src = (const float*)&img[st][jarr[jn]][jrow[jn]][16 * b + 8 * lh];
                const f32x4 lo = *(const f32x4*)src, hi = *(const f32x4*)(src + 4);
                f32x8_l bv = {lo[0], lo[1], lo[2], lo[3], hi[0], hi[1], hi[2], hi[3]};
                if (!jok[jn]) bv = (f32x8_l){0.f, 0.f, 0.f, 0.f, 0.f, 0.f, 0.f, 0.f};
                bf16x8_l pb[3];
                split8(bv, pb);
#pragma unroll
                for (int q = 0; q < 6; ++q) {
                    acc[0][jn] = __builtin_amdgcn_mfma_f32_32x32x16_bf16(pa0[PA[q]], pb[PB[q]], acc[0][jn], 0, 0, 0);
                    acc[1][jn] = __builtin_amdgcn_mfma_f32_32x32x16_bf16(pa1[PA[q]], pb[PB[q]], acc[1][jn], 0, 0, 0);
                }
            }
        }
    };
    auto mma = [&](int set, int st, int b) {
        if constexpr (X3) {
            mma_x3(set, st, b);
            return;
        } else {
        unsigned w8[8];
#pragma unroll
        for (int t = 0; t < 8; ++t) {
            unsigned wv = wa[set][t];
            if constexpr (FACT) {
                const unsigned ov = wo[set][t];
                float a0 = __builtin_bit_cast(float, wv << 16), a1 = __builtin_bit_cast(float, wv & 0xffff0000u);
                a0 = __builtin_bit_cast(float, ov << 16) > 0.f ? a0 : a0 * slope;
                a1 = __builtin_bit_cast(float, ov & 0xffff0000u) > 0.f ? a1 : a1 * slope;
                typedef __bf16 bf16x2_l __attribute__((ext_vector_type(2)));
                typedef float f32x2_l __attribute__((ext_vector_type(2)));
                wv = __builtin_bit_cast(unsigned, __builtin_convertvector((f32x2_l){a0, a1}, bf16x2_l));
            }
            w8[t] = wv;
        }
        u32x4_l ev, od;
#pragma unroll
        for (int q = 0; q < 4; ++q) {
            ev[q] = __builtin_amdgcn_perm(w8[2 * q + 1], w8[2 * q], 0x05040100u);
            od[q] = __builtin_amdgcn_perm(w8[2 * q + 1], w8[2 * q], 0x07060302u);
        }
        const bf16x8_l fa0 = __builtin_bit_cast(bf16x8_l, ev), fa1 = __builtin_bit_cast(bf16x8_l, od);
        bf16x8_l fb[2];
#pragma unroll
        for (int jn = 0; jn < 2; ++jn) {
            fb[jn] = *(const bf16x8_l*)(const void*)&img[st][jarr[jn]][jrow[jn]][16 * b + 8 * lh];
            if (!jok[jn]) fb[jn] = __builtin_bit_cast(bf16x8_l, (u32x4_l){0u, 0u, 0u, 0u});
        }
#pragma unroll
        for (int jn = 0; jn < 2; ++jn) {
            acc[0][jn] = __builtin_amdgcn_mfma_f32_32x32x16_bf16(fa0, fb[jn], acc[0][jn], 0, 0, 0);
            acc[1][jn] = __builtin_amdgcn_mfma_f32_32x32x16_bf16(fa1, fb[jn], acc[1][jn], 0, 0, 0);
        }
        }
    };
    for (int e = tid; e < 2 * 4 * 12 * ROWE; e += 256) (&img[0][0][0][0])[e] = (ET)0.f;
    __syncthreads();
    if (u0 < u1) {
        stage_load(u0);
        stage_store(0);
    }
    load_a(0, u0, wave);
    __syncthreads();
    if constexpr (X3) {
        if (nbatch == 16) {
            load_a(1, u0, wave + 4);
            load_a(2, u0, wave + 8);
            for (int u = u0; u < u1; ++u) {
                const int st = (u - u0) & 1;
                if (u + 1 < u1) stage_load(u + 1);
                c3_static_for4([&](auto J_) {
                    constexpr int J = decltype(J_)::value;
                    constexpr int JN = (J + 3) & 3;
                    load_a(JN, J + 3 >= 4 ? u + 1 : u, wave + 4 * JN);
                    mma_x3(J, st, wave + 4 * J);
                });
                if (u + 1 < u1) stage_store(st ^ 1);
                __syncthreads();
            }
        }
    }
    bool odd = false;
    auto item = [&](auto S_, int u, int b, int st) {
        constexpr int S = decltype(S_)::value;
        const bool last = b + 4 >= nbatch;
        load_a(S ^ 1, last ? u + 1 : u, last ? wave : b + 4);
        mma(S, st, b);
    };
    for (int u = (X3 && nbatch == 16) ? u1 : u0; u < u1; ++u) {
        const int st = (u - u0) & 1;
        if (u + 1 < u1) stage_load(u + 1);
        for (int b = wave; b < nbatch; b += 4) {
            if (odd) item(std::integral_constant<int, 1>{}, u, b, st);
            else item(std::integral_constant<int, 0>{}, u, b, st);
            odd = !odd;
        }
        if (u + 1 < u1) stage_store(st ^ 1);
        __syncthreads();
    }
    static_assert(sizeof(img) >= 4 * 64 * 48 * sizeof(float), "slab reduction lives in the image stages");
    float (*slabS)[64 * 48] = (float (*)[64 * 48]) & img[0][0][0][0];
#pragma unroll
    for (int i = 0; i < 2; ++i)
#pragma unroll
        for (int r = 0; r < 16; ++r) {
            const int rho = (r & 3) + 8 * (r >> 2) + 4 * lh;
            const int k = 2 * rho + i;
#pragma unroll
            for (int jn = 0; jn < 2; ++jn) {
                const int j = jn * 32 + l31;
                if (j < 48) slabS[wave][k * 48 + j] = acc[i][jn][r];
            }
        }
    __syncthreads();
    float* slab = part + ((long)blockIdx.x * K + kg * 64) * 48;
    for (int e = tid; e < 64 * 48; e += 256) slab[e] = ((slabS[0][e] + slabS[1][e]) + slabS[2][e]) + slabS[3][e];
}

__global__ __launch_bounds__(256) void c3_wgrad_reduce_kernel(const DgPtrs parts, const DgPtrs dws, int nslabs, int total, int accumulate) {
    const float* __restrict__ part = dg_pick<const float>(parts, blockIdx.y);
    float* __restrict__ dw = dg_pick<float>(dws, blockIdx.y);
    __shared__ float red[16][17];
    const int el = threadIdx.x & 15, sl = threadIdx.x >> 4;
    const int e = blockIdx.x * 16 + el;
    float s = 0.f;
    if (e < total)
        for (int b = sl; b < nslabs; b += 16) s += part[(long)b * total + e];
    red[sl][el] = s;
    __syncthreads();
    if (sl == 0 && e < total) {
#pragma unroll
        for (int j = 1; j < 16; ++j) s += red[j][el];
        if (accumulate) s += dw[e];
        dw[e] = s;
    }
}

static void c3_wgrad_plan(long npix, int* nb, int* ppw) {
    const int unit = 4 * CW_B;
    long per = (npix + 2047) / 2048;
    per = (per + unit - 1) / unit * unit;
    if (per < unit) per = unit;
    *ppw = (int)per;
    const long nwaves = (npix + per - 1) / per;
    *nb = (int)((nwaves + 3) / 4);
}
extern "C" size_t dg_c3_wgrad_workspace_bytes(int N, int H, int W, int K) {
    const long npix = (long)N * (H / 2) * (W / 2);
    int nb, ppw;
    c3_wgrad_plan(npix, &nb, &ppw);
    return (size_t)nb * K * 48 * sizeof(float);
}
struct C3Wgrad {
    const char* who;
    int groups, share;
    const void *const *dy, *const *x;
    const void* const* act_out;
    int act;
    float slope;
    float* const* dw;
    int io_bf16, N, H, W, K, prec, accumulate;
    void* const* ws;
    size_t ws_bytes;
    hipStream_t st;
};
static C3Wgrad c3_wgrad_call(const char* who, const void* const* dy, const void* const* act_out, int io_bf16, int act, float slope, const float* const* x,
                             float* const* dw, int N, int H, int W, int K, int prec, int accumulate, void* const* ws, size_t ws_bytes, dg_stream_t stream) {
    C3Wgrad c = C3Wgrad();
    c.who = who; c.groups = c.share = 1; c.dy = dy; c.x = (const void* const*)x; c.act_out = act_out; c.act = act; c.slope = slope; c.io_bf16 = io_bf16;
    c.dw = dw; c.N = N; c.H = H; c.W = W; c.K = K; c.prec = dg_resolve_prec(prec); c.accumulate = accumulate;
    c.ws = ws; c.ws_bytes = ws_bytes; c.st = (hipStream_t)stream;
    return c;
}
static int c3_wgrad(const C3Wgrad& c);
extern "C" int dg_conv4x4s2_c3_wgrad(const float* dy_nhwc, const float* x_nchw, float* dw, int N, int H, int W, int K,
                                     int accumulate, void* ws, size_t ws_bytes, dg_stream_t stream) {
    return c3_wgrad(c3_wgrad_call("dg_conv4x4s2_c3_wgrad", (const void* const*)&dy_nhwc, nullptr, 0, DG_ACT_NONE, 0.f, &x_nchw, &dw, N, H, W, K,
                                  DG_PREC_DEFAULT, accumulate, &ws, ws_bytes, stream));
}
extern "C" int dg_conv4x4s2_c3_wgrad_act(const float* dy_nhwc, const float* act_out_nhwc, int act, float slope,
                                         const float* x_nchw, float* dw, int N, int H, int W, int K, int accumulate,
                                         void* ws, size_t ws_bytes, dg_stream_t stream) {
    return c3_wgrad(c3_wgrad_call("dg_conv4x4s2_c3_wgrad_act", (const void* const*)&dy_nhwc, (const void* const*)&act_out_nhwc, 0, act, slope, &x_nchw, &dw,
                                  N, H, W, K, DG_PREC_DEFAULT, accumulate, &ws, ws_bytes, stream));
}
extern "C" int dg_conv4x4s2_c3_wgrad_t(const void* dy_nhwc, const void* act_out_nhwc, int io_bf16, int act, float slope,
                                       const float* x_nchw, float* dw, int N, int H, int W, int K, int accumulate,
                                       void* ws, size_t ws_bytes, dg_stream_t stream) {
    return c3_wgrad(c3_wgrad_call("dg_conv4x4s2_c3_wgrad_t", &dy_nhwc, &act_out_nhwc, io_bf16, act, slope, &x_nchw, &dw, N, H, W, K, DG_PREC_DEFAULT,
                                  accumulate, &ws, ws_bytes, stream));
}
extern "C" int dg_conv4x4s2_c3_wgrad_p(const void* dy_nhwc, const void* act_out_nhwc, int io_bf16, int act, float slope,
                                       const float* x_nchw, float* dw, int N, int H, int W, int K, int prec, int accumulate,
                                       void* ws, size_t ws_bytes, dg_stream_t stream) {
    C3_CHECK_PREC("dg_conv4x4s2_c3_wgrad_p", prec);
    return c3_wgrad(c3_wgrad_call("dg_conv4x4s2_c3_wgrad_p", &dy_nhwc, &act_out_nhwc, io_bf16, act, slope, &x_nchw, &dw, N, H, W, K, prec, accumulate, &ws,
                                  ws_bytes, stream));
}
extern "C" int dg_conv4x4s2_c3_wgrad_g(int groups, int share, const float* const* dy_nhwc, const float* const* act_out_nhwc, int act, float slope,
                                       const float* const* x_nchw, float* const* dw, int N, int H, int W, int K, int prec, int accumulate,
                                       void* const* ws, size_t ws_bytes, dg_stream_t stream) {
    C3_CHECK_PREC("dg_conv4x4s2_c3_wgrad_g", prec);
    C3Wgrad c = c3_wgrad_call("dg_conv4x4s2_c3_wgrad_g", (const void* const*)dy_nhwc, (const void* const*)act_out_nhwc, 0, act, slope, x_nchw, dw, N, H, W, K,
                              prec, accumulate, ws, ws_bytes, stream);
    c.groups = groups; c.share = share;
    return c3_wgrad(c);
}
static int c3_wgrad_reduce_g(int groups, int share, void* const* ws_tab, float* const* dw_tab, int nb, int total, int accumulate, hipStream_t st) {
    const int nout = groups / share;
    for (int j = 0; j < share; ++j) {
        const void* pp[DG_MAX_GROUPS];
        const void* dd[DG_MAX_GROUPS];
        for (int z = 0; z < nout; ++z) { pp[z] = ws_tab[z * share + j]; dd[z] = dw_tab[z * share + j]; }
        hipLaunchKernelGGL(c3_wgrad_reduce_kernel, dim3((total + 15) / 16, nout), dim3(256), 0, st, dg_ptrs(pp, nout), dg_ptrs(dd, nout), nb, total,
                           (accumulate || j > 0) ? 1 : 0);
        DG_CHECK_LAUNCH("c3_wgrad_reduce");
    }
    return DG_OK;
}
enum C3WgradForm { C3_WGRAD_LDS_X3, C3_WGRAD_LDS_BF16, C3_WGRAD_LANE_BF16, C3_WGRAD_MFMA };
static bool c3_wgrad_buf(const C3Wgrad& c) {
    return (long)c.N * (c.H / 2) * (c.W / 2) * c.K * 4 < (1L << 30) && (long)c.N * 3 * c.H * c.W * 4 < (1L << 30) && dg_get_option(DG_OPT_POINTER_PATH) == 0;
}
static C3WgradForm c3_wgrad_form(const C3Wgrad& c) {
    const bool lds = c.W / 2 <= CWL_WOMAX && dg_get_option(DG_OPT_KT) != 16;
    if (!c.io_bf16 && c.prec == DG_PREC_F32X3 && c3_wgrad_buf(c) && c.W >= 256 && lds) return C3_WGRAD_LDS_X3;
    if (c.io_bf16 && c.prec == DG_PREC_BF16) return c.W >= 32 && lds ? C3_WGRAD_LDS_BF16 : C3_WGRAD_LANE_BF16;
    return C3_WGRAD_MFMA;
}
static int c3_wgrad(const C3Wgrad& c) {
    const int N = c.N, H = c.H, W = c.W, K = c.K, groups = c.groups;
    DG_CHECK_ARG(groups >= 1 && groups <= DG_MAX_GROUPS && c.dy && c.x && c.dw && c.ws, "%s: bad group / null table", c.who);
    DG_CHECK_ARG(c.share >= 1 && groups % c.share == 0, "%s: share=%d", c.who, c.share);
    DG_CHECK_ARG(c.act == DG_ACT_NONE || ((c.act == DG_ACT_LEAKY || c.act == DG_ACT_RELU) && c.act_out),
                 "%s: act %d needs the saved activation output (LeakyReLU / ReLU only)", c.who, c.act);
    const bool fact = c.act != DG_ACT_NONE;
    const float slope = c.act == DG_ACT_RELU ? 0.f : c.slope;
    for (int i = 0; i < groups; ++i) DG_CHECK_ARG(c.dy[i] && c.x[i] && c.dw[i] && (!fact || c.act_out[i]), "%s: null pointer", c.who);
    for (int i = 0; i < groups; ++i) DG_CHECK_ARG(c.dw[i] == c.dw[i / c.share * c.share], "%s: problems of one share set must name the same dw", c.who);
    DG_CHECK_ARG(N >= 1 && K >= 64 && K % 64 == 0, "%s: K=%d must be a multiple of 64", c.who, K);
    DG_CHECK_ARG(dg_is_pow2(H) && dg_is_pow2(W) && H >= 2 && W >= 2, "%s: H,W must be powers of two", c.who);
    DG_CHECK_ARG((long)N * 3 * H * W < (1L << 31), "%s: tensor too large", c.who);
    const long npix = (long)N * (H / 2) * (W / 2);
    int nb, ppw;
    c3_wgrad_plan(npix, &nb, &ppw);
    const size_t need = (size_t)nb * K * 48 * sizeof(float);
    for (int i = 0; i < groups; ++i)
        if (c.ws[i] == nullptr || c.ws_bytes < need) return dg_fail(DG_ERR_WORKSPACE, "%s: workspace %zu < %zu", c.who, c.ws_bytes, need);
    const bool buf = c3_wgrad_buf(c);
    DG_CHECK_ARG(!c.io_bf16 || buf, "%s: bf16 operands need tensors < 1 GiB", c.who);
    const C3WgradForm form = c3_wgrad_form(c);
    DG_CHECK_ARG(form != C3_WGRAD_LANE_BF16 || groups == 1, "%s: this kernel takes one problem", c.who);
    const DgPtrs pdy = dg_ptrs(c.dy, groups), px = dg_ptrs(c.x, groups), pws = dg_ptrs(c.ws, groups), pao = dg_ptrs(fact ? c.act_out : nullptr, groups);
    const dim3 grid(nb, K / 64, groups);
    const int lgHo = dg_ilog2(H / 2), lgWo = dg_ilog2(W / 2);
    const int rpw = (N * (H / 2) + nb - 1) / nb;
    auto lds = [&](auto X3) {
        c3_with_flag(fact, [&](auto FACT) {
            hipLaunchKernelGGL((c3_wgrad_lds_kernel<decltype(FACT)::value, decltype(X3)::value>), grid, dim3(256), 0, c.st, pdy, px, pws, N, H, W, K, npix, rpw,
                               pao, slope);
        });
    };
    auto mfma = [&](auto BUF, auto IN16) {
        c3_with_flag(fact, [&](auto FACT) {
            hipLaunchKernelGGL((c3_wgrad_mfma_kernel<decltype(BUF)::value, decltype(FACT)::value, decltype(IN16)::value>), grid, dim3(256), 0, c.st, pdy, px, pws,
                               N, H, W, K, lgHo, lgWo, npix, ppw, pao, slope);
        });
    };
    switch (form) {
    case C3_WGRAD_LDS_X3: lds(C3Yes{}); break;
    case C3_WGRAD_LDS_BF16: lds(C3No{}); break;
    case C3_WGRAD_LANE_BF16:
        c3_with_flag(fact, [&](auto FACT) {
            hipLaunchKernelGGL(c3_wgrad_bf16mfma_kernel<decltype(FACT)::value>, dim3(nb, K / 64), dim3(256), 0, c.st, (const float*)c.dy[0], (const float*)c.x[0],
                               (float*)c.ws[0], N, H, W, K, lgHo, lgWo, npix, ppw, (const float*)(fact ? c.act_out[0] : nullptr), slope);
        });
        break;
    case C3_WGRAD_MFMA:
        if (c.io_bf16) mfma(C3Yes{}, C3Yes{});
        else if (buf) mfma(C3Yes{}, C3No{});
        else mfma(C3No{}, C3No{});
        break;
    }
    DG_CHECK_LAUNCH(c.who);
    return c3_wgrad_reduce_g(groups, c.share, c.ws, c.dw, nb, K * 48, c.accumulate, c.st);
}
```

discogan_modernized_amd/csrc/norm_act.hip:

```cpp
#include "dg_common.h"
#include <string.h>
#include <initializer_list>

#define BN_U 8

typedef __bf16 bf16x8_n __attribute__((ext_vector_type(8)));
typedef float f32x8_n __attribute__((ext_vector_type(8)));
template <typename T> struct BnV;
template <> struct BnV<float> { static constexpr int V = 4; };
template <> struct BnV<__bf16> { static constexpr int V = 8; };
__device__ __forceinline__ void bn_ld(const float* p, float (&v)[4]) {
    const f32x4 t = *(const f32x4*)p;
    v[0] = t[0]; v[1] = t[1]; v[2] = t[2]; v[3] = t[3];
}
__device__ __forceinline__ void bn_ld(const __bf16* p, float (&v)[8]) {
    const f32x8_n t = __builtin_convertvector(*(const bf16x8_n*)p, f32x8_n);
#pragma unroll
    for (int j = 0; j < 8; ++j) v[j] = t[j];
}
template <int V>
__device__ __forceinline__ void bn_ldp(const float* p, float (&v)[V]) {
#pragma unroll
    for (int h = 0; h < V / 4; ++h) {
        const f32x4 t = *(const f32x4*)(p + 4 * h);
        v[4 * h] = t[0]; v[4 * h + 1] = t[1]; v[4 * h + 2] = t[2]; v[4 * h + 3] = t[3];
    }
}
__device__ __forceinline__ void bn_st(float* p, const float (&v)[4]) { *(f32x4*)p = (f32x4){v[0], v[1], v[2], v[3]}; }
__device__ __forceinline__ void bn_st(__bf16* p, const float (&v)[8]) {
    f32x8_n t;
#pragma unroll
    for (int j = 0; j < 8; ++j) t[j] = v[j];
    *(bf16x8_n*)p = __builtin_convertvector(t, bf16x8_n);
}

template <int V>
__device__ __forceinline__ void bn_stp(float* p, const float (&v)[V]) {
#pragma unroll
    for (int h = 0; h < V / 4; ++h) *(f32x4*)(p + 4 * h) = (f32x4){v[4 * h], v[4 * h + 1], v[4 * h + 2], v[4 * h + 3]};
}

__device__ __forceinline__ float bn_norm(float y, float mean, float gs, float beta) { return fmaf(y - mean, gs, beta); }

struct BnProb {
    const void* y;
    const void* dz;
    void* out;
    void* out16;
    void* ws;
    float* saved;
    const float* gamma;
    const float* beta;
    float* rmean;
    float* rvar;
    int64_t* nbt;
    float* dgamma;
    float* dbeta;
};
struct BnGroup {
    BnProb p[DG_MAX_GROUPS];
};

struct BnGrid { int tx, ty, cchunks, rchunks; };
static BnGrid bn_grid(int M, int C, int V = 4) {
    BnGrid g;
    int q = C / V, tx = 1;
    while (tx < q && tx < 64) tx <<= 1;
    g.tx = tx;
    g.ty = 256 / tx;
    g.cchunks = (q + tx - 1) / tx;
    int rc = M / (g.ty * BN_U);
    int cap = 2048 / g.cchunks;
    if (cap > 512) cap = 512;
    if (rc > cap) rc = cap;
    if (rc < 1) rc = 1;
    g.rchunks = rc;
    return g;
}

template <typename T>
__global__ __launch_bounds__(256) void bn_stats_partial_kernel(const BnGroup G, int M, int C, int rchunks, int TX) {
    constexpr int V = BnV<T>::V;
    const T* __restrict__ y = (const T*)G.p[blockIdx.z].y;
    float* __restrict__ part = (float*)G.p[blockIdx.z].ws;
    __shared__ float red[2][256][V];
    const int TY = 256 / TX;
    const int tx = threadIdx.x % TX, ty = threadIdx.x / TX;
    const int c = (blockIdx.x * TX + tx) * V;
    const int rows_per = (M + rchunks - 1) / rchunks;
    const int r0 = blockIdx.y * rows_per, r1 = min(M, r0 + rows_per);
    float s[V], q[V];
#pragma unroll
    for (int j = 0; j < V; ++j) s[j] = q[j] = 0.f;
    if (c < C) {
        float sh[V];
        bn_ld(y + c, sh);
        const T* p = y + c;
        int r = r0 + ty;
        for (; r + (BN_U - 1) * TY < r1; r += BN_U * TY) {
            float v[BN_U][V];
#pragma unroll
            for (int u = 0; u < BN_U; ++u) bn_ld(p + (long)(r + u * TY) * C, v[u]);
#pragma unroll
            for (int u = 0; u < BN_U; ++u)
#pragma unroll
                for (int j = 0; j < V; ++j) {
                    const float d = v[u][j] - sh[j];
                    s[j] += d;
                    q[j] += d * d;
                }
        }
        for (; r < r1; r += TY) {
            float v[V];
            bn_ld(p + (long)r * C, v);
#pragma unroll
            for (int j = 0; j < V; ++j) {
                const float d = v[j] - sh[j];
                s[j] += d;
                q[j] += d * d;
            }
        }
    }
#pragma unroll
    for (int j = 0; j < V; ++j) {
        red[0][threadIdx.x][j] = s[j];
        red[1][threadIdx.x][j] = q[j];
    }
    __syncthreads();
    for (int h = TY >> 1; h > 0; h >>= 1) {
        if (ty < h) {
#pragma unroll
            for (int j = 0; j < V; ++j) {
                red[0][threadIdx.x][j] += red[0][threadIdx.x + h * TX][j];
                red[1][threadIdx.x][j] += red[1][threadIdx.x + h * TX][j];
            }
        }
        __syncthreads();
    }
    if (ty == 0 && c < C) {
#pragma unroll
        for (int j = 0; j < V; ++j) {
            part[(long)blockIdx.y * C + c + j] = red[0][tx][j];
            part[((long)rchunks + blockIdx.y) * C + c + j] = red[1][tx][j];
        }
    }
}

#define BN_FIN_CH 8
__device__ __forceinline__ int bn_reduce_partials(const float* __restrict__ part, int C, int rchunks, double* s_out, double* q_out) {
    __shared__ double red[2][32][BN_FIN_CH];
    const int cl = threadIdx.x % BN_FIN_CH, pl = threadIdx.x / BN_FIN_CH;
    const int c = blockIdx.x * BN_FIN_CH + cl;
    double s = 0.0, q = 0.0;
    if (c < C) {
        int r = pl;
        for (; r + 96 < rchunks; r += 128) {
            float vs[4], vq[4];
#pragma unroll
            for (int u = 0; u < 4; ++u) {
                vs[u] = part[(long)(r + 32 * u) * C + c];
                vq[u] = part[((long)rchunks + r + 32 * u) * C + c];
            }
#pragma unroll
            for (int u = 0; u < 4; ++u) {
                s += (double)vs[u];
                q += (double)vq[u];
            }
        }
        for (; r < rchunks; r += 32) {
            s += (double)part[(long)r * C + c];
            q += (double)part[((long)rchunks + r) * C + c];
        }
    }
    red[0][pl][cl] = s;
    red[1][pl][cl] = q;
    __syncthreads();
    if (pl != 0 || c >= C) return -1;
    for (int j = 1; j < 32; ++j) {
        s += red[0][j][cl];
        q += red[1][j][cl];
    }
    *s_out = s;
    *q_out = q;
    return c;
}

template <typename T>
__global__ __launch_bounds__(256) void bn_stats_finalize_kernel(const BnGroup G, int share, int M, int C, int rchunks, float eps, float momentum) {
    for (int j = 0; j < share; ++j) {
        const BnProb& P = G.p[blockIdx.y * share + j];
        const T* __restrict__ y = (const T*)P.y;
        float* __restrict__ running_mean = P.rmean;
        float* __restrict__ running_var = P.rvar;
        int64_t* __restrict__ nbt = P.nbt;
        float* __restrict__ saved = P.saved;
// ... 1134 lines not shown
```

discogan_modernized_amd/functional.py:

```python
from __future__ import annotations

import functools

import torch
from torch.autograd import Function

from . import ops


def _fwd(f):
    @functools.wraps(f)
    def w(ctx, *a, **k):
        ctx.dgc = ops.current()
        return f(ctx, *a, **k)
    return staticmethod(w)


def _bwd(f):
    @functools.wraps(f)
    def w(ctx, *g):
        with ops.use(ctx.dgc):
            return f(ctx, *g)
    return staticmethod(w)

# ... 66 lines not shown
            else:
                dw = ops.conv_wgrad(dy, x, stride, pad)
        _release_after_backward(dy, x)
        return dx, dw, None, None, None


class ConvTransposeFn(Function):

    @_fwd
    def forward(ctx, x, w, stride, pad, want_stats=False):
        x = ops.as_nhwc(x)
        ctx.save_for_backward(x, w)
        ctx.sp = (stride, pad)
        ctx.wref = w
        ctx.final = FINAL_PASS
        hin, win = x.shape[2], x.shape[3]
        hout, wout = (hin - 1) * stride - 2 * pad + 4, (win - 1) * stride - 2 * pad + 4
        ctx.out_hw = (hout, wout)
        if not want_stats:
            y = ops.conv_dgrad(x, w, (hout, wout), stride, pad)
            _release_unless_wgrad(ctx, x)
            return y
        y, stat = ops.conv_dgrad(x, w, (hout, wout), stride, pad, want_stats=want_stats)
        _release_unless_wgrad(ctx, x)
        if stat is None:
            stat = torch.empty(0, device=y.device)
        ctx.mark_non_differentiable(stat)
        ctx.set_materialize_grads(False)
        return y, stat

    @_bwd
    def backward(ctx, dy, dstat=None):
        if dy is None:
            return None, None, None, None, None
        x, w = ctx.saved_tensors
        w = ctx.wref
        stride, pad = ctx.sp
        dy = ops.as_nhwc(dy)
        dx = ops.conv_fwd(dy, w, stride, pad) if ctx.needs_input_grad[0] else None
        dw = None
        if ctx.needs_input_grad[1]:
            fg = _flat_grad_of(ctx.wref)
            if fg is not None:
                ops.conv_wgrad(x, dy, stride, pad, out=fg, accumulate=True)
                _final(ctx.final, ctx.wref)
            else:
                dw = ops.conv_wgrad(x, dy, stride, pad)
        _release_after_backward(dy, x)
        return dx, dw, None, None, None


class ConvC3Fn(Function):

    @_fwd
    def forward(ctx, x, w, act, slope, want_planes=False):
        y = ops.c3_fwd(x, w, act, slope, want_planes=want_planes)
        ctx.save_for_backward(x, w, y)
        ctx.act = (act, slope)
        ctx.wref = w
        ctx.final = FINAL_PASS
        return y

    @_bwd
    def backward(ctx, dy):
        x, w, y = ctx.saved_tensors
        act, slope = ctx.act
        fused_dgrad = FUSE_C3_DGRAD_ACT and act == ops.ACT_LEAKY and ops.c3_dgrad_act_ok(w.shape[0], x.shape[0], x.shape[2], x.shape[3],
                                                                                          dy.dtype == torch.bfloat16)
        if act == ops.ACT_NONE or (ctx.needs_input_grad[0] and not fused_dgrad):
            g = ops.act_bwd(dy, y, act, slope) if act != ops.ACT_NONE else ops.as_nhwc(dy)
            fuse = {}
        else:
            g = ops.as_nhwc(dy)
            fuse = dict(act_out=y, act=act, slope=slope)
        dx = None
        if ctx.needs_input_grad[0]:
            dx = ops.c3_dgrad(g, w, ops.ACT_NONE, act_out=y, in_act=act, slope=slope) if fuse else ops.c3_dgrad(g, w, ops.ACT_NONE)
        dw = None
        if ctx.needs_input_grad[1]:
            fg = _flat_grad_of(ctx.wref)
            if fg is not None and fg.is_contiguous():
                ops.c3_wgrad(g, x, out=fg, accumulate=True, **fuse)
                _final(ctx.final, ctx.wref)
            else:
                dw = ops.c3_wgrad(g, x, **fuse)
        return dx, dw, None, None, None


class ConvTransposeC3Fn(Function):

    @_fwd
    def forward(ctx, x, w, act):
        x = ops.as_nhwc(x)
        out = ops.c3_dgrad(x, w, act)
        ctx.save_for_backward(x, w, out)
        ctx.act = act
        ctx.wref = w
        ctx.final = FINAL_PASS
        return out

    @_bwd
    def backward(ctx, dout):
        x, w, out = ctx.saved_tensors
        g = ops.act_bwd(dout, out, ctx.act) if ctx.act != ops.ACT_NONE else dout.contiguous()
        dx = ops.c3_fwd(g, w, ops.ACT_NONE) if ctx.needs_input_grad[0] else None
        dw = None
        if ctx.needs_input_grad[1]:
            fg = _flat_grad_of(ctx.wref)
            if fg is not None and fg.is_contiguous():
                ops.c3_wgrad(x, g, out=fg, accumulate=True)
                _final(ctx.final, ctx.wref)
            else:
                dw = ops.c3_wgrad(x, g)
        return dx, dw, None


class BatchNormActFn(Function):

    @_fwd
    def forward(ctx, y, gamma, beta, running_mean, running_var, nbt, training, eps, momentum, act, slope,
                partials=None, z_cm=False, dy_cm=False, z_po=False, dy_po=False):
        y = ops.as_nhwc(y)
        if training and partials is not None and partials.numel() > 0:
            saved = ops.bn_stats_from_partials(partials, y, running_mean, running_var, nbt, eps, momentum)
        elif training:
            saved = ops.bn_train_stats(y, running_mean, running_var, nbt, eps, momentum)
        else:
            saved = torch.stack([running_mean, torch.rsqrt(running_var + eps)])
        z = ops.bn_act_fwd(y, saved, gamma, beta, act, slope, planes_cm=z_cm, planes_only=z_po and training)
        ctx.save_for_backward(y, saved, gamma, beta)
        ctx.cfg = (act, slope, training)
        ctx.dy_cm = bool(dy_cm)
        ctx.dy_po = bool(dy_po)
        ctx.prefs = (gamma, beta)
        ctx.final = FINAL_PASS
        return z

    @_bwd
    def backward(ctx, dz):
        y, saved, gamma, beta = ctx.saved_tensors
        act, slope, training = ctx.cfg
        if not training:
            raise RuntimeError("BatchNormActFn: backward in eval mode is not supported")
        need_p = ctx.needs_input_grad[1] or ctx.needs_input_grad[2]
        fg, fb = _flat_grad_of(ctx.prefs[0]), _flat_grad_of(ctx.prefs[1])
        if need_p and fg is not None and fb is not None:
            dy, _, _ = ops.bn_act_bwd(dz, y, saved, gamma, beta, act, slope, out_grads=(fg, fb), planes_cm=ctx.dy_cm, planes_only=ctx.dy_po)
            _final(ctx.final, ctx.prefs[0], ctx.prefs[1])
            return (dy,) + (None,) * 15
        dy, dgamma, dbeta = ops.bn_act_bwd(dz, y, saved, gamma, beta, act, slope, need_param_grads=need_p, planes_cm=ctx.dy_cm,
                                           planes_only=ctx.dy_po)
        return (dy, dgamma if ctx.needs_input_grad[1] else None, dbeta if ctx.needs_input_grad[2] else None,
                None, None, None, None, None, None, None, None, None, None, None, None, None)


class ActFn(Function):

    @_fwd
    def forward(ctx, x, act, slope):
        out = ops.act_fwd(x, act, slope)
        ctx.save_for_backward(out)
        ctx.cfg = (act, slope)
        return out

    @_bwd
    def backward(ctx, dy):
        (out,) = ctx.saved_tensors
        act, slope = ctx.cfg
        return ops.act_bwd(dy, out, act, slope), None, None


class MSELossFn(Function):
    @_fwd
    def forward(ctx, x, t, out=None):
        loss, xd, td = ops.mse_fwd(x, t, out)
        ctx.save_for_backward(xd, td)
        ctx.in_strides = x.stride()
        return loss

    @_bwd
    def backward(ctx, gout):
        xd, td = ctx.saved_tensors
        gout = gout.contiguous()
        dx = ops.mse_bwd(xd, td, gout) if ctx.needs_input_grad[0] else None
        dt = None
        if ctx.needs_input_grad[1]:
            dt = ops.mse_bwd(td, xd, gout)
        return dx, dt, None


class BCELossFn(Function):

    @_fwd
    def forward(ctx, p, label, out=None):
        shape = p.shape
        loss, pc = ops.bce_fwd(p.reshape(-1), label, out)
        ctx.save_for_backward(pc)
        ctx.cfg = (label, shape)
        return loss

    @_bwd
    def backward(ctx, gout):
        (pc,) = ctx.saved_tensors
        label, shape = ctx.cfg
        return ops.bce_bwd(pc, label, gout.contiguous()).reshape(shape), None, None


class BCETargetLossFn(Function):

    @_fwd
    def forward(ctx, p, target):
        shape = p.shape
        loss, pc, tc = ops.bce_target_fwd(p.reshape(-1), target.detach().reshape(-1))
        ctx.save_for_backward(pc, tc)
        ctx.shape = shape
        return loss

    @_bwd
    def backward(ctx, gout):
        pc, tc = ctx.saved_tensors
        return ops.bce_target_bwd(pc, tc, gout.contiguous()).reshape(ctx.shape), None


class HingeEmbeddingLossFn(Function):

    @_fwd
    def forward(ctx, x, y, margin):
        loss, xd, yd = ops.hinge_fwd(x, y.detach(), margin)
        ctx.save_for_backward(xd, yd)
        ctx.margin = margin
        ctx.in_shape = x.shape
        return loss

    @_bwd
    def backward(ctx, gout):
        xd, yd = ctx.saved_tensors
        return ops.hinge_bwd(xd, yd, ctx.margin, gout.contiguous()), None, None


class FeatureMatchFn(Function):

    @_fwd
    def forward(ctx, real, fake, out=None):
        loss, diff, rd, fd = ops.fm_fwd(real, fake, out)
        ctx.save_for_backward(diff, rd, fd)
        return loss

    @_bwd
    def backward(ctx, gout):
        diff, rd, fd = ctx.saved_tensors
        dreal, dfake = ops.fm_bwd(diff, rd, fd, gout.contiguous(), ctx.needs_input_grad[0], ctx.needs_input_grad[1])
        return dreal, dfake, None


class LossMixFn(Function):

    @_fwd
    def forward(ctx, lossvec, nfm, rate, arch, which, idx, *slots):
        out = ops.loss_mix_fwd(lossvec, nfm, rate, arch)
        ctx.cfg = (lossvec.numel(), nfm, rate, arch, which, idx)
        ctx.set_materialize_grads(False)
        return tuple(out.unbind(0))

    @_bwd
    def backward(ctx, *gouts):
        nslots, nfm, rate, arch, which, idx = ctx.cfg
        gout = gouts[which]
        if gout is None:
            return (None,) * (6 + len(idx))
        gv = ops.loss_mix_bwd(gout.contiguous(), nslots, nfm, rate, arch, which)
        return (None, None, None, None, None, None) + tuple(gv[i] for i in idx)


def _all_or_none(grads, who):
    live = [g_ is not None for g_ in grads]
    if any(live) and not all(live):
        raise RuntimeError(f"{who}: gradients arrived for some problems of a grouped node only")
    return all(live)


def _flat_grads_of(params):
    fgs = [_flat_grad_of(p) for p in params]
    if any(f is None for f in fgs):
        raise RuntimeError("grouped launches need parameters whose .grad is the optimiser's flat gradient view (optim.Adam)")
    return fgs


class ConvGroupFn(Function):

    @_fwd
    def forward(ctx, g, stride, pad, transposed, *xw):
        xs = [ops.as_nhwc(x) for x in xw[:g]]
        ws = list(xw[g:])
        ctx.g, ctx.sp, ctx.tr = g, (stride, pad), transposed
        ctx.wrefs = ws
        ctx.final = FINAL_PASS
        ctx.save_for_backward(*xs, *ws)
        if transposed:
            hin, win = xs[0].shape[2], xs[0].shape[3]
            hw = ((hin - 1) * stride - 2 * pad + 4, (win - 1) * stride - 2 * pad + 4)
            ys = ops.conv_dgrad_g(xs, ws, hw, stride, pad)
        else:
            ys = ops.conv_fwd_g(xs, ws, stride, pad)
        ctx.set_materialize_grads(False)
        return tuple(ys)

# ... 229 lines not shown
```

discogan_modernized_amd/model.py:

```python
from __future__ import annotations

import math

import torch
import torch.nn as nn

from . import functional as F
from . import ops


FUSE_BN_STATS = {"auto": "auto", "0": False, "1": True, "split": "split"}[__import__("os").environ.get("DG_FUSE_BN", "auto")]
FUSE_BN_MIN_FLOP = 4e10


def _fuse_stats(conv=None, x=None):
    if ops.SHADOW or ops.ACT16:
        return True if ops.FUSE_STATS16 else False
    if FUSE_BN_STATS != "auto":
        return FUSE_BN_STATS
    if conv is None or x is None:
        return False
    n, _, h, w = x.shape
    pixels = h * w if isinstance(conv, ConvTranspose2d) else (h * w) // 4
    return 2.0 * n * pixels * 16 * conv.in_channels * conv.out_channels >= FUSE_BN_MIN_FLOP
# ... 25 lines not shown
                    p.grad = None
                else:
                    p.grad.detach_()
                    p.grad.zero_()


class Conv2d(nn.Module):

    def __init__(self, in_channels, out_channels, kernel_size=4, stride=2, padding=1, bias=False):
        super().__init__()
        if kernel_size != 4 or bias or (stride, padding) not in ((2, 1), (1, 0)):
            raise ValueError("only Conv2d(k=4, (s,p) in {(2,1),(1,0)}, bias=False) exists in the DiscoGAN path")
        self.in_channels, self.out_channels = in_channels, out_channels
        self.stride, self.padding = stride, padding
        w = _init_weight((out_channels, in_channels, 4, 4))
        if in_channels != 3:
            w = ops.krsc_param(w)
        self.weight = nn.Parameter(w)

    def forward(self, x, fused_act=ops.ACT_NONE, slope=0.2, want_stats=False, want_planes=False):
        if self.in_channels == 3:
            return F.ConvC3Fn.apply(x, self.weight, fused_act, slope, want_planes)
        if want_stats:
            return F.ConvFn.apply(x, self.weight, self.stride, self.padding, want_stats)
        return F.ConvFn.apply(x, self.weight, self.stride, self.padding)

    @property
    def emits_bn_stats(self):
        return self.in_channels != 3 and self.stride == 2

    def extra_repr(self):
        return f"{self.in_channels}, {self.out_channels}, kernel_size=(4, 4), stride={self.stride}, padding={self.padding}, bias=False"


class ConvTranspose2d(nn.Module):

    def __init__(self, in_channels, out_channels, kernel_size=4, stride=2, padding=1, bias=False):
        super().__init__()
        if kernel_size != 4 or bias or (stride, padding) not in ((2, 1), (1, 0)):
            raise ValueError("only ConvTranspose2d(k=4, (s,p) in {(2,1),(1,0)}, bias=False) exists in the DiscoGAN path")
        self.in_channels, self.out_channels = in_channels, out_channels
        self.stride, self.padding = stride, padding
        w = _init_weight((in_channels, out_channels, 4, 4))
        if out_channels != 3:
            w = ops.krsc_param(w)
        self.weight = nn.Parameter(w)

    def forward(self, x, fused_act=ops.ACT_NONE, want_stats=False):
        if self.out_channels == 3:
            return F.ConvTransposeC3Fn.apply(x, self.weight, fused_act)
        if want_stats:
            return F.ConvTransposeFn.apply(x, self.weight, self.stride, self.padding, want_stats)
        return F.ConvTransposeFn.apply(x, self.weight, self.stride, self.padding)

    @property
    def emits_bn_stats(self):
        return self.out_channels != 3 and self.stride == 2

    def extra_repr(self):
        return f"{self.in_channels}, {self.out_channels}, kernel_size=(4, 4), stride={self.stride}, padding={self.padding}, bias=False"


class BatchNorm2d(nn.Module):

    def __init__(self, num_features, eps=1e-5, momentum=0.1):
        super().__init__()
        self.num_features, self.eps, self.momentum = num_features, eps, momentum
        self.weight = nn.Parameter(torch.ones(num_features))
        self.bias = nn.Parameter(torch.zeros(num_features))
        self.register_buffer("running_mean", torch.zeros(num_features))
        self.register_buffer("running_var", torch.ones(num_features))
        self.register_buffer("num_batches_tracked", torch.tensor(0, dtype=torch.long))

    def forward(self, y, fused_act=ops.ACT_NONE, slope=0.2, partials=None, z_cm=False, dy_cm=False, z_po=False, dy_po=False):
        if self.training and y.shape[0] * y.shape[2] * y.shape[3] <= 1:
            raise ValueError(f"Expected more than 1 value per channel when training, got input size {tuple(y.shape)}")
        return F.BatchNormActFn.apply(y, self.weight, self.bias, self.running_mean, self.running_var,
                                      self.num_batches_tracked, self.training, self.eps, self.momentum, fused_act, slope,
                                      partials, z_cm, dy_cm, z_po, dy_po)

    def extra_repr(self):
        return f"{self.num_features}, eps={self.eps}, momentum={self.momentum}, affine=True, track_running_stats=True"


class _Act(nn.Module):
    act = ops.ACT_NONE

    def __init__(self, slope=0.0, inplace=False):
        super().__init__()
        self.negative_slope, self.inplace = slope, inplace

    def forward(self, x):
        return F.ActFn.apply(x, self.act, self.negative_slope)


class LeakyReLU(_Act):
    act = ops.ACT_LEAKY

    def __init__(self, negative_slope=0.01, inplace=False):
        super().__init__(negative_slope, inplace)


class ReLU(_Act):
    act = ops.ACT_RELU

    def __init__(self, inplace=False):
        super().__init__(0.0, inplace)


class Sigmoid(_Act):
    act = ops.ACT_SIGMOID

    def __init__(self):
        super().__init__(0.0, False)


def _plane_hints(conv, x, nxt, z_is_output=False):
    if not ops.X3:
        return False, False, False, False
    n, _, h, w = x.shape
    dy_cm = z_cm = dy_po = z_po = False
    s2conv = isinstance(conv, Conv2d) and conv.stride == 2 and conv.in_channels != 3
    s2convT = isinstance(conv, ConvTranspose2d) and conv.stride == 2 and conv.out_channels != 3
    if s2conv:
        dy_cm = ops.x3_window_dgrad(n, h, w, conv.in_channels, conv.out_channels)
        dy_po = ops.x3_all_plane_readers(n, h, w, conv.in_channels, conv.out_channels, forward_is_dgrad=True)
        ho, wo = h // 2, w // 2
    elif s2convT:
        dy_po = ops.x3_all_plane_readers(n, 2 * h, 2 * w, conv.out_channels, conv.in_channels, forward_is_dgrad=False)
        ho, wo = 2 * h, 2 * w
    else:
        ho, wo = (4, 4) if isinstance(conv, ConvTranspose2d) else (1, 1)
    if not z_is_output and isinstance(nxt, ConvTranspose2d) and nxt.stride == 2 and nxt.out_channels != 3:
        z_cm = ops.x3_window_dgrad(n, 2 * ho, 2 * wo, nxt.out_channels, nxt.in_channels)
        z_po = ops.x3_all_plane_readers(n, 2 * ho, 2 * wo, nxt.out_channels, nxt.in_channels, forward_is_dgrad=True)
    elif not z_is_output and isinstance(nxt, Conv2d) and nxt.stride == 2 and nxt.in_channels != 3:
        z_po = ops.x3_all_plane_readers(n, ho, wo, nxt.in_channels, nxt.out_channels, forward_is_dgrad=False)
    return z_cm and ops.X3_CM, dy_cm and ops.X3_CM, z_po, dy_po


C3_PLANES = __import__("os").environ.get("DG_X3_C3_PLANES", "1") != "0"


def _first_layer_planes(x, nxt):
    if not (ops.X3 and C3_PLANES and isinstance(nxt, Conv2d) and nxt.stride == 2):
        return False
    n, _, h, w = x.shape
    if ops._x3_ok(0, n, h // 2, w // 2, nxt.in_channels, nxt.out_channels, 2, 1) and \
            (ops.X3_RSP or getattr(nxt.weight, "_dg_x3", (None, 0, None))[2] is not None):
        return True
    return torch.is_grad_enabled() and nxt.weight.requires_grad and ops._x3_ok(2, n, h // 2, w // 2, nxt.in_channels, nxt.out_channels, 2, 1)


def drain(gen):
    try:
        while True:
            next(gen)
    except StopIteration as e:
        return e.value


def _run_fused(layers, x):
    return drain(_run_fused_steps(layers, x))


def _run_fused_steps(layers, x):
    i, n = 0, len(layers)
    while i < n:
        conv = layers[i]
        bn = layers[i + 1] if i + 1 < n and isinstance(layers[i + 1], BatchNorm2d) else None
        j = i + (2 if bn is not None else 1)
        act_mod = layers[j] if j < n and isinstance(layers[j], _Act) else None
        act = act_mod.act if act_mod is not None else ops.ACT_NONE
        slope = act_mod.negative_slope if act_mod is not None else 0.0
        if bn is not None and bn.training and not ops.X3 and _fuse_stats(conv, x) and conv.emits_bn_stats:
            y, st = conv(x, want_stats=_fuse_stats(conv, x))
            x = bn(y, act, slope, st)
        elif bn is not None:
            nxt = layers[j + (1 if act_mod is not None else 0)] if j + (1 if act_mod is not None else 0) < n else None
            z_cm, dy_cm, z_po, dy_po = _plane_hints(conv, x, nxt, z_is_output=nxt is None)
            st = None
            if ops.X3 and ops.X3_FUSE_STATS and bn.training and conv.emits_bn_stats:
                y, st = conv(x, want_stats=True)
                st = st if st.numel() > 0 else None
            else:
                y = conv(x)
            yield
            x = bn(y, act, slope, st, z_cm, dy_cm, z_po, dy_po)
        elif isinstance(conv, Conv2d) and conv.in_channels == 3 and act in (ops.ACT_LEAKY, ops.ACT_RELU, ops.ACT_NONE):
            nxt = layers[j + (1 if act_mod is not None else 0)] if j + (1 if act_mod is not None else 0) < n else None
            x = conv(x, act, slope, want_planes=_first_layer_planes(x, nxt))
        elif isinstance(conv, ConvTranspose2d) and conv.out_channels == 3 and act in (ops.ACT_SIGMOID, ops.ACT_NONE):
            x = conv(x, act)
        else:
            x = conv(x)
            if act_mod is not None:
                x = act_mod(x)
        i = j + (1 if act_mod is not None else 0)
        if i < n:
            yield
    return x


def _fire_forward_hooks(records):
    for rec in records:
        for mod, inp, out in rec:
            for hook in list(mod._forward_hooks.values()):
                hook(mod, (inp,), out)


def _group_layers(layer_lists, xs):
    g, n = len(xs), len(layer_lists[0])
    records = [[] for _ in range(g)]
    i = 0
    while i < n:
        convs = [L[i] for L in layer_lists]
        conv = convs[0]
        has_bn = i + 1 < n and isinstance(layer_lists[0][i + 1], BatchNorm2d)
        j = i + (2 if has_bn else 1)
        act_mod = layer_lists[0][j] if j < n and isinstance(layer_lists[0][j], _Act) else None
        act = act_mod.act if act_mod is not None else ops.ACT_NONE
        slope = act_mod.negative_slope if act_mod is not None else 0.0
        ws = [c.weight for c in convs]
        if has_bn:
            bns = [L[i + 1] for L in layer_lists]
            if not all(b.training for b in bns):
                raise RuntimeError("grouped passes run BatchNorm in training mode only")
            ys = F.ConvGroupFn.apply(g, conv.stride, conv.padding, isinstance(conv, ConvTranspose2d), *xs, *ws)
            if ys[0].shape[0] * ys[0].shape[2] * ys[0].shape[3] <= 1:
                raise ValueError(f"Expected more than 1 value per channel when training, got input size {tuple(ys[0].shape)}")
            xs = F.BatchNormActGroupFn.apply(g, bns[0].eps, bns[0].momentum, act, slope, *ys, *[b.weight for b in bns], *[b.bias for b in bns],
                                             *[b.running_mean for b in bns], *[b.running_var for b in bns], *[b.num_batches_tracked for b in bns])
            for k in range(g):
                records[k].append((bns[k], ys[k], xs[k]))
        elif isinstance(conv, Conv2d) and conv.in_channels == 3 and act in (ops.ACT_LEAKY, ops.ACT_RELU, ops.ACT_NONE):
            ins = xs
            xs = F.ConvC3GroupFn.apply(g, act, slope, *xs, *ws)
            for k in range(g):
                records[k].append((convs[k], ins[k], xs[k]))
        elif isinstance(conv, ConvTranspose2d) and conv.out_channels == 3 and act in (ops.ACT_SIGMOID, ops.ACT_NONE):
            xs = F.ConvTransposeC3GroupFn.apply(g, act, *xs, *ws)
        else:
            xs = F.ConvGroupFn.apply(g, conv.stride, conv.padding, isinstance(conv, ConvTranspose2d), *xs, *ws)
            if act_mod is not None:
                xs = F.ActGroupFn.apply(g, act, slope, *xs)
        xs = list(xs)
        i = j + (1 if act_mod is not None else 0)
    _fire_forward_hooks(records)
    return xs


def group_generators(nets, xs, cut_at_bottleneck=False):
    if any(n_.main is not None for n_ in nets):
        raise RuntimeError("grouped passes need the encoder / decoder form of the generators")
    if not cut_at_bottleneck:
        return _group_layers([list(n_.encoder) + list(n_.decoder) for n_ in nets], list(xs))
    hs = _group_layers([list(n_.encoder) for n_ in nets], list(xs))
    leaves = [h.detach().requires_grad_(True) for h in hs]
    return _group_layers([list(n_.decoder) for n_ in nets], leaves), hs, leaves


def group_discriminators(nets, xs):
    g = len(xs)
    d0 = nets[0]
    hs = list(F.ConvC3GroupFn.apply(g, ops.ACT_LEAKY, d0.relu1.negative_slope, *xs, *[d.conv1.weight for d in nets]))
    feats = [[] for _ in range(g)]
    records = [[(nets[k].conv1, xs[k], hs[k])] for k in range(g)]
    for i in range(2, d0.n_stages + 1):
        convs = [getattr(d, f"conv{i}") for d in nets]
        bns = [getattr(d, f"bn{i}") for d in nets]
        if not all(b.training for b in bns):
            raise RuntimeError("grouped passes run BatchNorm in training mode only")
        ys = F.ConvGroupFn.apply(g, convs[0].stride, convs[0].padding, False, *hs, *[c.weight for c in convs])
        hs = list(F.BatchNormActGroupFn.apply(g, bns[0].eps, bns[0].momentum, ops.ACT_LEAKY, getattr(d0, f"relu{i}").negative_slope, *ys,
                                              *[b.weight for b in bns], *[b.bias for b in bns], *[b.running_mean for b in bns],
                                              *[b.running_var for b in bns], *[b.num_batches_tracked for b in bns]))
        for k in range(g):
            feats[k].append(hs[k])
            records[k].append((bns[k], ys[k], hs[k]))
    heads = [getattr(d, f"conv{d0.n_stages + 1}") for d in nets]
    ys = F.ConvGroupFn.apply(g, heads[0].stride, heads[0].padding, False, *hs, *[c.weight for c in heads])
    outs = F.ActGroupFn.apply(g, ops.ACT_SIGMOID, 0.0, *ys)
    _fire_forward_hooks(records)
    return [(outs[k], feats[k]) for k in range(g)]


class Discriminator(_FlatGradMixin, nn.Module):

    def __init__(self, image_size: int = 512):
        super().__init__()
        ch = stage_channels(image_size)
        self.image_size, self.n_stages = image_size, len(ch)
        cin = 3
        for i, c in enumerate(ch, start=1):
            setattr(self, f"conv{i}", Conv2d(cin, c, 4, 2, 1, bias=False))
            if i >= 2:
                setattr(self, f"bn{i}", BatchNorm2d(c))
            setattr(self, f"relu{i}", LeakyReLU(0.2, inplace=True))
            cin = c
        setattr(self, f"conv{len(ch) + 1}", Conv2d(cin, 1, 4, 1, 0, bias=False))
        self.sigmoid = Sigmoid()

    def forward(self, input_tensor):
        return drain(self.forward_steps(input_tensor))

    def forward_steps(self, input_tensor):
        feats = []
        h = self.conv1(input_tensor, ops.ACT_LEAKY, self.relu1.negative_slope,
                       want_planes=_first_layer_planes(input_tensor, getattr(self, "conv2", None)))
        yield
        for i in range(2, self.n_stages + 1):
            relu, bn, conv = getattr(self, f"relu{i}"), getattr(self, f"bn{i}"), getattr(self, f"conv{i}")
            if bn.training and not ops.X3 and _fuse_stats(conv, h):
                y, st = conv(h, want_stats=_fuse_stats(conv, h))
                h = bn(y, ops.ACT_LEAKY, relu.negative_slope, st)
            else:
                _, dy_cm, _, dy_po = _plane_hints(conv, h, None, z_is_output=True)
                st = None
                if ops.X3 and ops.X3_FUSE_STATS and bn.training:
                    y, st = conv(h, want_stats=True)
                    st = st if st.numel() > 0 else None
                else:
                    y = conv(h)
                yield
                h = bn(y, ops.ACT_LEAKY, relu.negative_slope, st, False, dy_cm, False, dy_po)
            feats.append(h)
            yield
        out = self.sigmoid(getattr(self, f"conv{self.n_stages + 1}")(h))
        return out, feats


class Generator(_FlatGradMixin, nn.Module):

    def __init__(self, extra_layers: bool = False, image_size: int = 512):
        super().__init__()
        ch = stage_channels(image_size)
        self.image_size = image_size
        enc = []
        cin = 3
        for i, c in enumerate(ch):
# ... 26 lines not shown
```

discogan_modernized_amd/ops.py:

```python
from __future__ import annotations

import torch

from . import _lib

ACT_NONE, ACT_LEAKY, ACT_RELU, ACT_SIGMOID = 0, 1, 2, 3
PREC_DEFAULT, PREC_F32, PREC_BF16, PREC_F32X3 = -1, 0, 1, 2


class Context:

    def __init__(self, prec=None, shadow=False, act16=False, x3=False, group_plan="launch"):
        self.prec = prec
        self.group_plan = group_plan
        self.shadow, self.act16, self.x3 = bool(shadow), bool(act16), bool(x3)
        self.shadow_tab, self.plane_tab = {}, {}

    @property
    def cprec(self):
        return PREC_DEFAULT if self.prec is None else int(self.prec)

    def clear(self):
        self.shadow_tab.clear()
        self.plane_tab.clear()
# ... 487 lines not shown
                                             stride, pad, _ptr(stat), stat.numel() if stat is not None else 0, _ptr(ws), wsb, _stream()),
                       "dg_conv_dgrad_mixed")
        else:
            stat = torch.empty((rows, 3 * c + 4), device=dy.device, dtype=torch.float32) if rows > 0 else None
            _lib.check(L.dg_conv_dgrad_g(1, _tab([dy]), _tab([w]), _tab([dx]), n, h, wd, c, k, stride, pad, prec, 1, _tab([stat]) if rows > 0 else None,
                                         stat.numel() if rows > 0 else 0, _tab([ws]), wsb, _stream()), "dg_conv_dgrad_g")
    return (dx, stat) if want_stats else dx


def conv_fwd_bias_act(x, w, bias, stride, pad, act=ACT_NONE, slope=0.2):
    _check_dev(x, w, bias)
    x, w = as_nhwc(x), _krsc(w)
    n, c, h, wd = x.shape
    k = w.shape[0]
    ho, wo = _out_hw(h, wd, stride, pad)
    y = empty_nhwc(n, k, ho, wo, x.device)
    L = _lib.load()
    ws, wsb = _ws(L.dg_conv_workspace_bytes(0, n, h, wd, c, k, stride, pad), x.device)
    _lib.check(L.dg_conv_fwd_bias_act(_ptr(x), _ptr(w), _ptr(bias), _ptr(y), n, h, wd, c, k, stride, pad, act, slope, _ptr(ws), wsb,
                                      _stream()), "dg_conv_fwd_bias_act")
    return y


def conv_dgrad_bias_act(x, w, bias, out_hw, stride, pad, act=ACT_NONE, slope=0.0):
    _check_dev(x, w, bias)
    x, w = as_nhwc(x), _krsc(w)
    n, k = x.shape[0], x.shape[1]
    c = w.shape[1]
    h, wd = out_hw
    y = empty_nhwc(n, c, h, wd, x.device)
    L = _lib.load()
    ws, wsb = _ws(L.dg_conv_workspace_bytes(1, n, h, wd, c, k, stride, pad), x.device)
    _lib.check(L.dg_conv_dgrad_bias_act(_ptr(x), _ptr(w), _ptr(bias), _ptr(y), n, h, wd, c, k, stride, pad, act, slope, _ptr(ws), wsb,
                                        _stream()), "dg_conv_dgrad_bias_act")
    return y


def conv_wgrad(dy, x, stride, pad, out=None, accumulate=False):
    _check_dev(dy, x, allow16=True, planes_ok=True)
    dy = as_nhwc(dy)
    x = as_nhwc(x)
    n, c, h, wd = x.shape
    k = dy.shape[1]
    dw = out if out is not None else empty_krsc(k, c, x.device)
    L = _lib.load()
    prec = _CUR.cprec
    ws, wsb = _ws(L.dg_conv_workspace_bytes_p(2, n, h, wd, c, k, stride, pad, prec, 1), x.device)
    if _x3_ok(2, n, h, wd, c, k, stride, pad):
        dp, dd, dcm = planes_of(dy, allow_cm=True)
        xp, xd, _ = planes_of(x)
        with _prof("conv_wgrad", 2.0 * n * dy.shape[2] * dy.shape[3] * k * c * 16):
            _lib.check(L.dg_conv_wgrad_x3(dp, dd, dcm, xp, xd, _ptr(dw), n, h, wd, c, k, stride, pad, int(accumulate), _ptr(ws), wsb,
                                          _stream()), "dg_conv_wgrad_x3")
        return dw
    _need_fp32(dy, "conv_wgrad")
    _need_fp32(x, "conv_wgrad")
    da, d16, xa, x16 = dy, 0, x, 0
    if k == 1:
        x16 = int(_is16(x))
    elif _bf16_ok(2, n, h, wd, c, k, stride, pad) or _is16(x) or _is16(dy):
        if c % 8 == 0:
            xa, x16 = _mixed_operand(x)
        if k % 8 == 0:
            da, d16 = _mixed_operand(dy)
    if (_is16(dy) and not d16) or (_is16(x) and not x16):
        raise _lib.DiscoganHipError(f"conv_wgrad: no bf16 kernel for bf16 operands of shapes {tuple(dy.shape)}, {tuple(x.shape)}")
    with _prof("conv_wgrad" if k > 1 else "head1", 2.0 * n * dy.shape[2] * dy.shape[3] * k * c * 16):
        if d16 or x16:
            _lib.check(L.dg_conv_wgrad_mixed(_ptr(da), d16, _ptr(xa), x16, _ptr(dw), n, h, wd, c, k,
                                             stride, pad, int(accumulate), _ptr(ws), wsb, _stream()), "dg_conv_wgrad_mixed")
        else:
            _lib.check(L.dg_conv_wgrad_g(1, 1, _tab([dy]), _tab([x]), _tab([dw]), n, h, wd, c, k, stride, pad, prec, 1, int(accumulate),
                                         _tab([ws]), wsb, _stream()), "dg_conv_wgrad_g")
    return dw


def c3_fwd(x_nchw, w, act=ACT_NONE, slope=0.2, want_planes=False):
    _check_dev(x_nchw, w)
    x = x_nchw.contiguous()
    w = w.contiguous()
    n, _, h, wd = x.shape
    k = w.shape[0]
    if want_planes and _CUR.x3 and k == 64 and x.numel() * 4 < (1 << 30) and n * (h // 2) * (wd // 2) < (1 << 30):
        y = empty_nhwc(n, k, h // 2, wd // 2, x.device)
        y3 = torch.empty((3, y.numel()), device=x.device, dtype=torch.bfloat16)
        with _prof("c3_fwd", 2.0 * n * (h // 2) * (wd // 2) * k * 48), _hbm("edge_c3_fwd", 4.0 * x.numel() + 10.0 * y.numel()):
            _lib.check(_lib.load().dg_conv4x4s2_c3_fwd_x3(_ptr(x), _ptr(w), _ptr(y), _ptr(y3), y3.stride(0), n, h, wd, k, act, slope, _stream()),
                       "dg_conv4x4s2_c3_fwd_x3")
        planes_put(y, y3)
        return y
    o16 = _CUR.act16 and k == 64 and x.numel() * 4 < (1 << 30)
    y = empty_nhwc(n, k, h // 2, wd // 2, x.device, torch.bfloat16 if o16 else torch.float32)
    with _prof("c3_fwd", 2.0 * n * (h // 2) * (wd // 2) * k * 48), \
            _hbm("edge_c3_fwd", 4.0 * x.numel() + y.numel() * y.element_size()):
        _lib.check(_lib.load().dg_conv4x4s2_c3_fwd_p(_ptr(x), _ptr(w), _ptr(y), int(o16), n, h, wd, k, act, slope, _CUR.cprec, _stream()),
                   "dg_conv4x4s2_c3_fwd_p")
    if _CUR.shadow and not o16 and k % 8 == 0:
        shadow_put(y, f32_to_bf16(y, empty_nhwc_bf16(n, k, h // 2, wd // 2, x.device)))
    return y


def c3_dgrad_act_ok(k, n=1, h=2, wd=2, dy_bf16=False):
    return bool(_lib.load().dg_c3_dgrad_act_ok(int(n), int(h), int(wd), int(k), int(bool(dy_bf16))))


def c3_dgrad(dy, w, act=ACT_NONE, act_out=None, in_act=ACT_NONE, slope=0.2):
    _check_dev(dy, act_out, allow16=True)
    _check_dev(w)
    dy = as_nhwc(dy)
    w = w.contiguous()
    n, k, ho, wo = dy.shape
    dx = torch.empty((n, 3, 2 * ho, 2 * wo), device=dy.device, dtype=torch.float32)
    L = _lib.load()
    ws, wsb = _ws(L.dg_c3_dgrad_workspace_bytes(k), dy.device)
    if act_out is not None and in_act != ACT_NONE:
        ao = as_nhwc(act_out)
        if ao.shape != dy.shape or ao.dtype != dy.dtype or ao.stride() != dy.stride():
            raise _lib.DiscoganHipError("c3_dgrad: act_out must have dy's shape, type and layout")
        with _hbm("edge_c3_dgrad", 2.0 * dy.numel() * dy.element_size() + 4.0 * dx.numel()):
            _lib.check(L.dg_conv4x4s2_c3_dgrad_act_p(_ptr(dy), int(_is16(dy)), _ptr(ao), in_act, float(slope), _ptr(w), _ptr(dx), n, 2 * ho, 2 * wo, k,
                                                     act, _CUR.cprec, _ptr(ws), wsb, _stream()), "dg_conv4x4s2_c3_dgrad_act_p")
        return dx
    if _is16(dy) and not L.dg_c3_dgrad_act_ok(n, 2 * ho, 2 * wo, k, 1):
        dyf = torch.empty_like(dy, dtype=torch.float32)
        dyf.copy_(dy)
        dy = dyf
    with _hbm("edge_c3_dgrad", dy.numel() * dy.element_size() + 4.0 * dx.numel()):
        _lib.check(L.dg_conv4x4s2_c3_dgrad_p(_ptr(dy), int(_is16(dy)), _ptr(w), _ptr(dx), n, 2 * ho, 2 * wo, k, act, _CUR.cprec, _ptr(ws), wsb,
                                             _stream()), "dg_conv4x4s2_c3_dgrad_p")
    return dx


def c3_wgrad(dy, x_nchw, out=None, accumulate=False, act_out=None, act=ACT_NONE, slope=0.0):
    _check_dev(dy, act_out, allow16=True)
    _check_dev(x_nchw)
    dy = as_nhwc(dy)
    x = x_nchw.contiguous()
    n, k, ho, wo = dy.shape
    h, wd = x.shape[2], x.shape[3]
    dw = out if out is not None else torch.empty((k, 3, 4, 4), device=dy.device, dtype=torch.float32)
    L = _lib.load()
    ws, wsb = _ws(L.dg_c3_wgrad_workspace_bytes(n, h, wd, k), dy.device)
    fuse = act_out is not None and act != ACT_NONE
    ao = None
    if fuse:
        ao = as_nhwc(act_out)
        assert ao.shape == dy.shape and ao.dtype == dy.dtype
    with _hbm("edge_c3_wgrad", float(dy.element_size()) * ((2 if fuse else 1) * dy.numel()) + 4.0 * x.numel()):
        _lib.check(L.dg_conv4x4s2_c3_wgrad_p(_ptr(dy), _ptr(ao), int(_is16(dy)), act if fuse else ACT_NONE, float(slope), _ptr(x), _ptr(dw),
                                             n, h, wd, k, _CUR.cprec, int(accumulate), _ptr(ws), wsb, _stream()), "dg_conv4x4s2_c3_wgrad_p")
    return dw


def bn_train_stats(y, running_mean, running_var, nbt, eps, momentum):
    _check_dev(y, allow16=True)
    y = as_nhwc(y)
    n, c, h, w = y.shape
    m = n * h * w
    saved = torch.empty((2, c), device=y.device, dtype=torch.float32)
    L = _lib.load()
    ws, wsb = _ws(L.dg_bn_workspace_bytes(m, c), y.device)
    with _hbm("bn_stats", float(y.element_size()) * m * c):
        _lib.check(L.dg_bn_train_stats_t(_ptr(y), int(_is16(y)), m, c, eps, momentum, _ptr(running_mean), _ptr(running_var), _ptr(nbt),
                                         _ptr(saved), _ptr(ws), wsb, _stream()), "dg_bn_train_stats")
    return saved


_PARTIALS_ONE_LAUNCH = __import__("os").environ.get("DG_BN_PARTIALS_ONE_LAUNCH", "0") == "1"


def bn_stats_from_partials(stat, y, running_mean, running_var, nbt, eps, momentum):
    _check_dev(stat)
    n, c, h, w = y.shape
    saved = torch.empty((2, c), device=y.device, dtype=torch.float32)
    L = _lib.load()
    ws, wsb = (None, 0) if _PARTIALS_ONE_LAUNCH else _ws(L.dg_bn_partials_workspace_bytes(stat.shape[0], c), y.device)
    _lib.check(L.dg_bn_stats_from_partials(_ptr(stat), stat.shape[0], n * h * w, c, eps, momentum,
                                           _ptr(running_mean), _ptr(running_var), _ptr(nbt), _ptr(saved),
                                           _ptr(ws), wsb, _stream()), "dg_bn_stats_from_partials")
    return saved


def _bn_out(y, planes_cm, planes_only):
    n, c, h, w = y.shape
    if _is16(y):
        return "bf16", empty_nhwc(n, c, h, w, y.device, torch.bfloat16), None, 0, False
    out = empty_nhwc(n, c, h, w, y.device)
    if _CUR.x3 and c % 8 == 0:
        extra = torch.empty((3, out.numel()), device=y.device, dtype=torch.bfloat16)
        cm = int(bool(planes_cm) and c % 64 == 0 and (n * h * w) % 4 == 0)
        return "planes", out, extra, cm, bool(planes_only) and X3_PLANES_ONLY
    if _CUR.shadow and c % 8 == 0:
        return "shadow", out, empty_nhwc_bf16(n, c, h, w, y.device), 0, False
    return "plain", out, None, 0, False


def _bn_publish(form, out, extra, cm, plane_only):
    if form == "planes":
        planes_put(out, extra, cm)
        if plane_only:
            out._dg_planes_only = True
            if POISON_PLANES_ONLY:
                out.fill_(float("nan"))
    elif form == "shadow":
        shadow_put(out, extra)
    return out


_BN_FWD_BYTES = {"bf16": 4.0, "planes": 14.0, "planes_only": 10.0, "shadow": 10.0, "plain": 8.0}
_BN_BWD_BYTES = {"bf16": 10.0, "planes": 26.0, "planes_only": 22.0, "shadow": 22.0, "plain": 20.0}


def bn_act_fwd(y, saved, gamma, beta, act, slope=0.2, planes_cm=False, planes_only=False):
    _check_dev(y, allow16=True)
    y = as_nhwc(y)
    n, c, h, w = y.shape
    m = n * h * w
    form, z, extra, cm, po = _bn_out(y, planes_cm, planes_only)
    L = _lib.load()
    rest = (m, c, _ptr(saved), _ptr(gamma), _ptr(beta), act, slope, _stream())
    with _hbm("bn_apply", _BN_FWD_BYTES["planes_only" if po else form] * m * c):
        if form == "bf16":
            _lib.check(L.dg_bn_act_fwd_t(_ptr(y), _ptr(z), 1, *rest), "dg_bn_act_fwd_t")
        elif form == "planes":
            _lib.check(L.dg_bn_act_fwd_x3(_ptr(y), None if po else _ptr(z), _ptr(extra), extra.stride(0), cm, *rest), "dg_bn_act_fwd_x3")
        elif form == "shadow":
            _lib.check(L.dg_bn_act_fwd_bf16(_ptr(y), _ptr(z), _ptr(extra), *rest), "dg_bn_act_fwd_bf16")
        else:
            _lib.check(L.dg_bn_act_fwd(_ptr(y), _ptr(z), *rest), "dg_bn_act_fwd")
    return _bn_publish(form, z, extra, cm, po)


def bn_act_bwd(dz, y, saved, gamma, beta, act, slope=0.2, need_param_grads=True, out_grads=None, planes_cm=False, planes_only=False):
    _check_dev(dz, y, allow16=True)
    dz = as_nhwc(dz)
    y = as_nhwc(y)
    n, c, h, w = y.shape
    m = n * h * w
    acc = 0
    if out_grads is not None:
        dgamma, dbeta = out_grads
        acc = 1
    else:
        dgamma = torch.empty(c, device=y.device, dtype=torch.float32) if need_param_grads else None
        dbeta = torch.empty(c, device=y.device, dtype=torch.float32) if need_param_grads else None
    L = _lib.load()
    ws, wsb = _ws(L.dg_bn_workspace_bytes(m, c), y.device)
    if _is16(y) and not _is16(dz):
        raise _lib.DiscoganHipError("bn_act_bwd: bf16 y needs a bf16 dz")
    form, dy, extra, cm, po = _bn_out(y, planes_cm, planes_only)
    rest = (m, c, _ptr(saved), _ptr(gamma), _ptr(beta), act, slope, _ptr(dgamma), _ptr(dbeta), acc, _ptr(ws), wsb, _stream())
    with _hbm("bn_backward", _BN_BWD_BYTES["planes_only" if po else form] * m * c):
        if form == "bf16":
            _lib.check(L.dg_bn_act_bwd_t(_ptr(dz), _ptr(y), _ptr(dy), 1, *rest), "dg_bn_act_bwd_t")
        elif form == "planes":
            _lib.check(L.dg_bn_act_bwd_x3(_ptr(dz), _ptr(y), None if po else _ptr(dy), _ptr(extra), extra.stride(0), cm, *rest), "dg_bn_act_bwd_x3")
        elif form == "shadow":
            _lib.check(L.dg_bn_act_bwd_bf16(_ptr(dz), _ptr(y), _ptr(dy), _ptr(extra), *rest), "dg_bn_act_bwd_bf16")
        else:
            _lib.check(L.dg_bn_act_bwd(_ptr(dz), _ptr(y), _ptr(dy), *rest), "dg_bn_act_bwd")
    return _bn_publish(form, dy, extra, cm, po), dgamma, dbeta


def _dense_like(x):
    return torch.empty_like(x, memory_format=torch.preserve_format)


def _dense(x):
    if x.is_contiguous() or is_nhwc(x):
        return x
    return x.contiguous()


def act_fwd(x, act, slope=0.2):
    _check_dev(x)
    x = _dense(x)
    y = _dense_like(x)
    _lib.check(_lib.load().dg_act_fwd(_ptr(x), _ptr(y), x.numel(), act, slope, _stream()), "dg_act_fwd")
    return y


def act_bwd(dy, out, act, slope=0.2):
    _check_dev(dy, out, allow16=True)
    out = _dense(out)
    if dy.stride() != out.stride():
        dyl = _dense_like(out)
        dyl.copy_(dy)
        dy = dyl
    dx = _dense_like(out)
    if _is16(out) or _is16(dy):
        if dy.dtype != out.dtype:
            raise _lib.DiscoganHipError("act_bwd: dy and out must have the same dtype")
        _lib.check(_lib.load().dg_act_bwd_t(_ptr(dy), _ptr(out), _ptr(dx), 1, out.numel(), act, slope, _stream()), "dg_act_bwd_t")
        return dx
    _lib.check(_lib.load().dg_act_bwd(_ptr(dy), _ptr(out), _ptr(dx), out.numel(), act, slope, _stream()), "dg_act_bwd")
    return dx


def _loss_ws(device):
    L = _lib.load()
    return _ws(L.dg_loss_workspace_bytes(), device)


def same_layout_pair(a, b):
    a = _dense(a)
    if b.stride() != a.stride():
# ... 491 lines not shown
```

include/discogan_hip.h:

```cpp
#ifndef DISCOGAN_HIP_H
#define DISCOGAN_HIP_H

#include <stddef.h>
#include <stdint.h>

#ifdef __cplusplus
extern "C" {
#endif

#define DG_OK 0
#define DG_ERR_INVALID (-1)
#define DG_ERR_WORKSPACE (-2)
#define DG_ERR_HIP (-3)

#define DG_ACT_NONE 0
#define DG_ACT_LEAKY 1
#define DG_ACT_RELU 2
#define DG_ACT_SIGMOID 3

typedef void* dg_stream_t;

#define DG_PREC_DEFAULT (-1)
#define DG_PREC_F32 0
#define DG_PREC_BF16 1
#define DG_PREC_F32X3 2

#define DG_MAX_GROUPS 4

int dg_version(void);
int dg_build_flags(void);
const char* dg_last_error(void);

int dg_set_option(const char* name, int value);

size_t dg_conv_workspace_bytes(int op , int N, int H, int W, int C, int K,
                               int stride, int pad);
int dg_conv_fwd(const float* x, const float* w, float* y, int N, int H, int W, int C, int K,
                int stride, int pad, void* ws, size_t ws_bytes, dg_stream_t stream);
int dg_conv_dgrad(const float* dy, const float* w, float* dx, int N, int H, int W, int C, int K,
                  int stride, int pad, void* ws, size_t ws_bytes, dg_stream_t stream);
int dg_conv_wgrad(const float* dy, const float* x, float* dw, int N, int H, int W, int C, int K,
                  int stride, int pad, int accumulate, void* ws, size_t ws_bytes, dg_stream_t stream);

size_t dg_conv_workspace_bytes_p(int op, int N, int H, int W, int C, int K, int stride, int pad, int prec, int plan_groups);
int dg_conv_bnstats_rows_p(int op, int N, int H, int W, int C, int K, int stride, int pad, int prec);
int dg_conv_plan_splits_p(int op, int N, int H, int W, int C, int K, int stride, int pad, int prec, int plan_groups);
#define DG_PLAN_FIELDS 20
int dg_conv_plan_describe(int op, int N, int H, int W, int C, int K, int stride, int pad, int prec, int plan_groups, int a_form, int b_form,
                          int* out, int n_out);
int dg_conv_fwd_g(int groups, const float* const* x, const float* const* w, float* const* y, int N, int H, int W, int C, int K, int stride,
                  int pad, int prec, int plan_groups, float* const* stat, size_t stat_floats, void* const* ws, size_t ws_bytes, dg_stream_t stream);
int dg_conv_dgrad_g(int groups, const float* const* dy, const float* const* w, float* const* dx, int N, int H, int W, int C, int K, int stride,
                    int pad, int prec, int plan_groups, float* const* stat, size_t stat_floats, void* const* ws, size_t ws_bytes, dg_stream_t stream);
int dg_conv_wgrad_g(int groups, int share, const float* const* dy, const float* const* x, float* const* dw, int N, int H, int W, int C, int K,
                    int stride, int pad, int prec, int plan_groups, int accumulate, void* const* ws, size_t ws_bytes, dg_stream_t stream);

int dg_conv_fwd_bias_act(const float* x, const float* w, const float* bias, float* y, int N, int H, int W, int C, int K,
                         int stride, int pad, int act, float slope, void* ws, size_t ws_bytes, dg_stream_t stream);
int dg_conv_dgrad_bias_act(const float* dy, const float* w, const float* bias, float* dx, int N, int H, int W, int C, int K,
                           int stride, int pad, int act, float slope, void* ws, size_t ws_bytes, dg_stream_t stream);

int dg_conv_bnstats_rows(int op, int N, int H, int W, int C, int K, int stride, int pad);
int dg_conv_plan_splits(int op, int N, int H, int W, int C, int K, int stride, int pad);
int dg_conv_fwd_bnstats(const float* x, const float* w, float* y, int N, int H, int W, int C, int K,
                        float* stat, size_t stat_floats, void* ws, size_t ws_bytes, dg_stream_t stream);
int dg_conv_dgrad_bnstats(const float* dy, const float* w, float* dx, int N, int H, int W, int C, int K,
                          float* stat, size_t stat_floats, void* ws, size_t ws_bytes, dg_stream_t stream);

int dg_conv4x4s2_fwd(const float* x, const float* w, float* y, int N, int H, int W, int C, int K,
                     void* ws, size_t ws_bytes, dg_stream_t s);
int dg_conv4x4s2_dgrad(const float* dy, const float* w, float* dx, int N, int H, int W, int C, int K,
                       void* ws, size_t ws_bytes, dg_stream_t s);
int dg_conv4x4s2_wgrad(const float* dy, const float* x, float* dw, int N, int H, int W, int C, int K,
                       int accumulate, void* ws, size_t ws_bytes, dg_stream_t s);
int dg_conv4x4_valid_fwd(const float* x, const float* w, float* y, int N, int C, int K,
                         void* ws, size_t ws_bytes, dg_stream_t s);
int dg_conv4x4_valid_dgrad(const float* dy, const float* w, float* dx, int N, int C, int K,
                           void* ws, size_t ws_bytes, dg_stream_t s);
int dg_conv4x4_valid_wgrad(const float* dy, const float* x, float* dw, int N, int C, int K,
                           int accumulate, void* ws, size_t ws_bytes, dg_stream_t s);
int dg_convT4x4s2_fwd(const float* x, const float* w, float* y, int N, int Hin, int Win, int Cin, int Cout,
                      void* ws, size_t ws_bytes, dg_stream_t s);
int dg_convT4x4s2_dgrad(const float* dy, const float* w, float* dx, int N, int Hin, int Win, int Cin, int Cout,
                        void* ws, size_t ws_bytes, dg_stream_t s);
int dg_convT4x4s2_wgrad(const float* dy, const float* x, float* dw, int N, int Hin, int Win, int Cin, int Cout,
                        int accumulate, void* ws, size_t ws_bytes, dg_stream_t s);
int dg_convT4x4_1to4_fwd(const float* x, const float* w, float* y, int N, int Cin, int Cout,
                         void* ws, size_t ws_bytes, dg_stream_t s);
int dg_convT4x4_1to4_dgrad(const float* dy, const float* w, float* dx, int N, int Cin, int Cout,
                           void* ws, size_t ws_bytes, dg_stream_t s);
int dg_convT4x4_1to4_wgrad(const float* dy, const float* x, float* dw, int N, int Cin, int Cout,
                           int accumulate, void* ws, size_t ws_bytes, dg_stream_t s);

int dg_conv4x4s2_c3_fwd(const float* x_nchw, const float* w, float* y_nhwc, int N, int H, int W, int K,
                        int act, float slope, dg_stream_t s);
size_t dg_c3_dgrad_workspace_bytes(int K);
int dg_conv4x4s2_c3_dgrad(const float* dy_nhwc, const float* w, float* dx_nchw, int N, int H, int W, int K,
                          int act, void* ws, size_t ws_bytes, dg_stream_t s);
size_t dg_c3_wgrad_workspace_bytes(int N, int H, int W, int K);
int dg_conv4x4s2_c3_wgrad(const float* dy_nhwc, const float* x_nchw, float* dw, int N, int H, int W, int K,
                          int accumulate, void* ws, size_t ws_bytes, dg_stream_t s);
int dg_conv4x4s2_c3_wgrad_act(const float* dy_nhwc, const float* act_out_nhwc, int act, float slope,
                              const float* x_nchw, float* dw, int N, int H, int W, int K, int accumulate,
                              void* ws, size_t ws_bytes, dg_stream_t s);

int dg_conv4x4s2_c3_fwd_p(const float* x_nchw, const float* w, void* y_nhwc, int y_bf16, int N, int H, int W, int K,
                          int act, float slope, int prec, dg_stream_t s);
int dg_conv4x4s2_c3_dgrad_p(const void* dy_nhwc, int dy_bf16, const float* w, float* dx_nchw, int N, int H, int W, int K,
                            int act, int prec, void* ws, size_t ws_bytes, dg_stream_t s);
int dg_conv4x4s2_c3_wgrad_p(const void* dy_nhwc, const void* act_out_nhwc, int io_bf16, int act, float slope,
                            const float* x_nchw, float* dw, int N, int H, int W, int K, int prec, int accumulate,
                            void* ws, size_t ws_bytes, dg_stream_t s);
int dg_c3_dgrad_act_ok(int N, int H, int W, int K, int dy_bf16);
int dg_conv4x4s2_c3_dgrad_act_p(const void* dy_nhwc, int dy_bf16, const void* act_out_nhwc, int in_act, float slope, const float* w,
                                float* dx_nchw, int N, int H, int W, int K, int act, int prec, void* ws, size_t ws_bytes, dg_stream_t s);
int dg_conv4x4s2_c3_fwd_g(int groups, const float* const* x_nchw, const float* const* w, float* const* y_nhwc, int N, int H, int W, int K,
                          int act, float slope, int prec, dg_stream_t s);
int dg_conv4x4s2_c3_dgrad_g(int groups, const float* const* dy_nhwc, const float* const* w, float* const* dx_nchw, int N, int H, int W, int K,
                            int act, int prec, dg_stream_t s);
int dg_conv4x4s2_c3_wgrad_g(int groups, int share, const float* const* dy_nhwc, const float* const* act_out_nhwc, int act, float slope,
                            const float* const* x_nchw, float* const* dw, int N, int H, int W, int K, int prec, int accumulate,
                            void* const* ws, size_t ws_bytes, dg_stream_t s);

size_t dg_bn_workspace_bytes(int M, int C);
int dg_bn_train_stats(const float* y, int M, int C, float eps, float momentum,
                      float* running_mean, float* running_var, int64_t* num_batches_tracked,
                      float* saved, void* ws, size_t ws_bytes, dg_stream_t s);
size_t dg_bn_partials_workspace_bytes(int P, int C);
int dg_bn_stats_from_partials(const float* stat, int P, int M, int C, float eps, float momentum,
                              float* running_mean, float* running_var, int64_t* num_batches_tracked,
                              float* saved, void* ws, size_t ws_bytes, dg_stream_t s);
int dg_bn_act_fwd(const float* y, float* z, int M, int C, const float* saved, const float* gamma,
                  const float* beta, int act, float slope, dg_stream_t s);
int dg_bn_act_bwd(const float* dz, const float* y, float* dy, int M, int C, const float* saved,
                  const float* gamma, const float* beta, int act, float slope,
                  float* dgamma, float* dbeta, int accumulate, void* ws, size_t ws_bytes, dg_stream_t s);

int dg_bn_train_stats_g(int groups, int share, const float* const* y, int M, int C, float eps, float momentum, float* const* running_mean,
                        float* const* running_var, int64_t* const* num_batches_tracked, float* const* saved, void* const* ws, size_t ws_bytes,
                        dg_stream_t s);
int dg_bn_act_fwd_g(int groups, const float* const* y, float* const* z, int M, int C, const float* const* saved, const float* const* gamma,
                    const float* const* beta, int act, float slope, dg_stream_t s);
int dg_bn_act_bwd_g(int groups, int share, const float* const* dz, const float* const* y, float* const* dy, int M, int C,
                    const float* const* saved, const float* const* gamma, const float* const* beta, int act, float slope,
                    float* const* dgamma, float* const* dbeta, int accumulate, void* const* ws, size_t ws_bytes, dg_stream_t s);

int dg_act_fwd(const float* x, float* y, size_t n, int act, float slope, dg_stream_t s);
int dg_act_bwd(const float* dy, const float* out, float* dx, size_t n, int act, float slope, dg_stream_t s);
int dg_act_fwd_g(int groups, const float* const* x, float* const* y, size_t n, int act, float slope, dg_stream_t s);
int dg_act_bwd_g(int groups, const float* const* dy, const float* const* out, float* const* dx, size_t n, int act, float slope, dg_stream_t s);

size_t dg_loss_workspace_bytes(void);
int dg_mse_fwd(const float* x, const float* t, size_t n, float* loss, void* ws, size_t ws_bytes, dg_stream_t s);
int dg_mse_bwd(const float* x, const float* t, size_t n, const float* gout, float* dx, dg_stream_t s);
int dg_bce_fwd(const float* p, int n, float label, float* loss, void* ws, size_t ws_bytes, dg_stream_t s);
int dg_bce_bwd(const float* p, int n, float label, const float* gout, float* dp, dg_stream_t s);
size_t dg_fm_workspace_bytes(int N, size_t J);
int dg_fm_fwd(const float* real, const float* fake, int N, size_t J, float* diff, float* loss,
              void* ws, size_t ws_bytes, dg_stream_t s);
int dg_fm_bwd(const float* diff, int N, size_t J, const float* gout, float* dreal, float* dfake, dg_stream_t s);
int dg_mse_fwd_g(int groups, const float* const* x, const float* const* t, size_t n, float* const* loss, void* const* ws, size_t ws_bytes, dg_stream_t s);
int dg_mse_bwd_g(int groups, const float* const* x, const float* const* t, size_t n, const float* const* gout, float* const* dx, dg_stream_t s);
int dg_bce_fwd_g(int groups, const float* const* p, int n, const float* label, float* const* loss, dg_stream_t s);
int dg_bce_bwd_g(int groups, const float* const* p, int n, const float* label, const float* const* gout, float* const* dp, dg_stream_t s);
int dg_fm_fwd_g(int groups, const float* const* real, const float* const* fake, int N, size_t J, float* const* diff, float* const* loss,
                void* const* ws, size_t ws_bytes, dg_stream_t s);
int dg_fm_bwd_g(int groups, const float* const* diff, int N, size_t J, const float* const* gout, float* const* dreal, float* const* dfake,
                dg_stream_t s);

int dg_debug_igemm_stamps(void* buf, size_t bytes);

int dg_device_cu_count(void);

int dg_loss_mix_fwd(const float* lossvec, float* out8, int nfm, float rate, int arch, dg_stream_t s);
int dg_loss_mix_bwd(const float* gout, float* gvec, int nfm, float rate, int arch, int which, dg_stream_t s);

int dg_adam_advance(double* state, double lr, double beta1, double beta2, dg_stream_t s);
int dg_adam_step_flat(float* p, const float* g, float* m, float* v, size_t n, const double* state,
                      float beta1, float beta2, float eps, float weight_decay, float grad_scale,
                      dg_stream_t s);
int dg_ema_update_flat(float* ema, const float* p, size_t n, float w, dg_stream_t s);
int dg_swap_flat(float* a, float* b, size_t n, dg_stream_t s);

size_t dg_grad_stats_workspace_bytes(void);
int dg_grad_sumsq_partial(const float* g, size_t n, double* ws, size_t ws_bytes, int slot0, int* slots_used, dg_stream_t s);
int dg_grad_clip_finalize(const double* ws, int slots, double pre_scale, double max_norm, int guard, double* ctl, dg_stream_t s);
int dg_adam_advance_c(double* state, double lr, double beta1, double beta2, const double* ctl, dg_stream_t s);
int dg_adam_step_flat_c(float* p, const float* g, float* m, float* v, size_t n, const double* state,
                        float beta1, float beta2, float eps, float weight_decay, const double* ctl,
                        void* out, int form, size_t plane_elems, dg_stream_t s);

int dg_bce_target_fwd(const float* p, const float* target, int n, float* loss, dg_stream_t s);
int dg_bce_target_bwd(const float* p, const float* target, int n, const float* gout, float* dp, dg_stream_t s);
int dg_hinge_fwd(const float* x, const float* y, size_t n, float margin, float* loss, void* ws, size_t ws_bytes, dg_stream_t s);
int dg_hinge_bwd(const float* x, const float* y, size_t n, float margin, const float* gout, float* dx, dg_stream_t s);

int dg_dp_ready(int* device_out );
int dg_dp_unique_id_bytes(void);
int dg_dp_get_unique_id(void* id_out_host, size_t bytes);
int dg_dp_init(int rank, int world, const void* unique_id_host, size_t bytes);
int dg_dp_world_size(void);
int dg_dp_rank(void);
int dg_dp_allreduce_sum(float* buf, size_t n, dg_stream_t stream);
int dg_dp_allreduce_max(float* buf, size_t n, dg_stream_t stream);
int dg_dp_broadcast(float* buf, size_t n, int root, dg_stream_t stream);
int dg_dp_barrier(float* scratch1 , dg_stream_t stream);
int dg_dp_destroy(void);

int dg_u8hwc_to_f32chw(const uint8_t* src, float* dst, int N, int H, int W, int bgr, dg_stream_t s);
int dg_image_prep(const uint8_t* src, float* dst, int N, int H, int W, int x0, int cw, int erode, int mode, int S, dg_stream_t s);
int dg_sample_grid_u8(const float* const* src, int cols, int rows, int S, int gap, int bg, uint8_t* canvas, dg_stream_t s);
size_t dg_image_metrics_workspace_bytes(int n, int S);
int dg_image_metrics(const float* x, const float* y, int n, int S, float* out , void* ws, size_t ws_bytes, dg_stream_t s);

int dg_adam_step_flat_bf16(float* p, const float* g, float* m, float* v, size_t n, const double* state,
                           float beta1, float beta2, float eps, float weight_decay, float grad_scale,
                           void* p_bf16, dg_stream_t s);
int dg_f32_to_bf16(const float* x, void* y_bf16, size_t n, dg_stream_t s);
int dg_bn_act_fwd_bf16(const float* y, float* z, void* z_bf16, int M, int C, const float* saved, const float* gamma,
                       const float* beta, int act, float slope, dg_stream_t stream);
int dg_bn_act_bwd_bf16(const float* dz, const float* y, float* dy, void* dy_bf16, int M, int C, const float* saved,
                       const float* gamma, const float* beta, int act, float slope, float* dgamma, float* dbeta,
                       int accumulate, void* ws, size_t ws_bytes, dg_stream_t stream);
int dg_conv_bf16_operands_ok(int op, int N, int H, int W, int C, int K, int stride, int pad);
int dg_conv_mixed_bnstats_rows(int op, int N, int H, int W, int C, int K, int stride, int pad, int a_bf16, int b_bf16);
int dg_conv_fwd_mixed(const void* x, int x_bf16, const void* w, int w_bf16, void* y, int y_bf16, int N, int H, int W, int C, int K,
                      int stride, int pad, float* stat, size_t stat_floats, void* ws, size_t ws_bytes, dg_stream_t stream);
int dg_conv_dgrad_mixed(const void* dy, int dy_bf16, const void* w, int w_bf16, void* dx, int dx_bf16, int N, int H, int W, int C, int K,
                        int stride, int pad, float* stat, size_t stat_floats, void* ws, size_t ws_bytes, dg_stream_t stream);
int dg_conv_wgrad_mixed(const void* dy, int dy_bf16, const void* x, int x_bf16, float* dw, int N, int H, int W, int C, int K,
                        int stride, int pad, int accumulate, void* ws, size_t ws_bytes, dg_stream_t stream);

int dg_f32_to_bf16x3(const float* x, void* y_planes, size_t n, size_t plane_elems, dg_stream_t s);
int dg_adam_step_flat_x3(float* p, const float* g, float* m, float* v, size_t n, const double* state,
                         float beta1, float beta2, float eps, float weight_decay, float grad_scale,
                         void* p_planes, size_t plane_elems, dg_stream_t s);
int dg_x3_transpose_planes(const void* src_planes, void* dst_planes, size_t plane_elems, const int64_t* w_off, const int* w_K,
                           const int* w_J, int n, dg_stream_t s);
int dg_bn_act_fwd_x3(const float* y, float* z, void* z_planes, size_t plane_elems, int plane_layout, int M, int C, const float* saved,
                     const float* gamma, const float* beta, int act, float slope, dg_stream_t stream);
int dg_bn_act_bwd_x3(const float* dz, const float* y, float* dy, void* dy_planes, size_t plane_elems, int plane_layout, int M, int C,
                     const float* saved, const float* gamma, const float* beta, int act, float slope, float* dgamma,
                     float* dbeta, int accumulate, void* ws, size_t ws_bytes, dg_stream_t stream);
int dg_conv4x4s2_c3_fwd_x3(const float* x_nchw, const float* w, float* y_nhwc, void* y_planes, size_t plane_elems, int N, int H, int W,
                           int K, int act, float slope, dg_stream_t stream);
int dg_conv_x3_planes_ok(int op, int N, int H, int W, int C, int K, int stride, int pad);
int dg_conv_x3_bnstats_rows(int op, int N, int H, int W, int C, int K, int stride, int pad);
int dg_conv_fwd_x3(const void* x_planes, int64_t x_plane, const void* w_planes, int64_t w_plane, int w_transposed, float* y,
                   int N, int H, int W, int C, int K, int stride, int pad, float* stat, size_t stat_floats, void* ws, size_t ws_bytes,
                   dg_stream_t stream);
int dg_conv_dgrad_x3(const void* dy_planes, int64_t dy_plane, int dy_layout, const void* w_planes, int64_t w_plane, float* dx, int N, int H, int W,
                     int C, int K, int stride, int pad, float* stat, size_t stat_floats, void* ws, size_t ws_bytes, dg_stream_t stream);
int dg_conv_wgrad_x3(const void* dy_planes, int64_t dy_plane, int dy_layout, const void* x_planes, int64_t x_plane, float* dw, int N, int H, int W,
                     int C, int K, int stride, int pad, int accumulate, void* ws, size_t ws_bytes, dg_stream_t stream);

int dg_bn_train_stats_t(const void* y, int io_bf16, int M, int C, float eps, float momentum, float* running_mean,
                        float* running_var, int64_t* num_batches_tracked, float* saved, void* ws, size_t ws_bytes,
                        dg_stream_t stream);
int dg_bn_act_fwd_t(const void* y, void* z, int io_bf16, int M, int C, const float* saved, const float* gamma,
                    const float* beta, int act, float slope, dg_stream_t stream);
int dg_bn_act_bwd_t(const void* dz, const void* y, void* dy, int io_bf16, int M, int C, const float* saved,
                    const float* gamma, const float* beta, int act, float slope, float* dgamma, float* dbeta,
                    int accumulate, void* ws, size_t ws_bytes, dg_stream_t stream);
int dg_act_bwd_t(const void* dy, const void* out, void* dx, int io_bf16, size_t n, int act, float slope, dg_stream_t stream);
int dg_conv4x4s2_c3_fwd_t(const float* x_nchw, const float* w, void* y_nhwc, int y_bf16, int N, int H, int W, int K,
                          int act, float slope, dg_stream_t s);
int dg_conv4x4s2_c3_dgrad_t(const void* dy_nhwc, int dy_bf16, const float* w, float* dx_nchw, int N, int H, int W, int K,
                            int act, void* ws, size_t ws_bytes, dg_stream_t s);
// ... 15 lines not shown
```

Before: 297.4 images/s.

## Fuse tail BatchNorm+ReLU into the 3-channel transposed-conv load path

Adds on-load BatchNorm+ReLU variants of the C3 dgrad-scatter and wgrad kernels. The generator's last BN->ReLU->ConvTranspose(→3ch) block now normalizes the pre-BN tensor inside the conv kernels, so the normalized activation is never written to or read back from memory. Backward recomputes the normalized activation inside the wgrad kernel. The cost is extra per-element FMA/ReLU work in the conv inner loops, plus new kernel template variants that may raise register pressure.

```diff
diff --git a/discogan_modernized_amd/_lib.py b/discogan_modernized_amd/_lib.py
--- a/discogan_modernized_amd/_lib.py
+++ b/discogan_modernized_amd/_lib.py
@@ -34,6 +34,10 @@
     "dg_c3_dgrad_act_ok": (_i, [_i, _i, _i, _i, _i]),
     "dg_conv4x4s2_c3_dgrad_act_p": (_i, [_p, _i, _p, _i, _f, _p, _p, _i, _i, _i, _i, _i, _i, _p, _z, _p]),
     "dg_conv4x4s2_c3_wgrad_p": (_i, [_p, _p, _i, _i, _f, _p, _p, _i, _i, _i, _i, _i, _i, _p, _z, _p]),
+    "dg_c3_dgrad_bn_ok": (_i, [_i, _i, _i, _i, _i]),
+    "dg_conv4x4s2_c3_dgrad_bn_p": (_i, [_p, _p, _p, _p, _i, _p, _p, _i, _i, _i, _i, _i, _i, _p]),
+    "dg_c3_wgrad_bn_ok": (_i, [_i, _i, _i, _i, _i]),
+    "dg_conv4x4s2_c3_wgrad_bn_p": (_i, [_p, _p, _p, _p, _i, _p, _p, _i, _i, _i, _i, _i, _i, _p, _z, _p]),
     "dg_conv4x4s2_c3_fwd_g": (_i, [_i, _p, _p, _p, _i, _i, _i, _i, _i, _f, _i, _p]),
     "dg_conv4x4s2_c3_dgrad_g": (_i, [_i, _p, _p, _p, _i, _i, _i, _i, _i, _i, _p]),
     "dg_conv4x4s2_c3_wgrad_g": (_i, [_i, _i, _p, _p, _i, _f, _p, _p, _i, _i, _i, _i, _i, _i, _p, _z, _p]),
diff --git a/discogan_modernized_amd/csrc/dg_common.h b/discogan_modernized_amd/csrc/dg_common.h
--- a/discogan_modernized_amd/csrc/dg_common.h
+++ b/discogan_modernized_amd/csrc/dg_common.h
@@ -83,6 +83,8 @@
     return u;
 }
 
+__device__ __forceinline__ float bn_norm(float y, float mean, float gs, float beta) { return fmaf(y - mean, gs, beta); }
+
 __device__ __forceinline__ void dg_split3(const f32x4& v, dg_bf16x4_t& hi, dg_bf16x4_t& mid, dg_bf16x4_t& lo) {
     hi = __builtin_convertvector(v, dg_bf16x4_t);
     const f32x4 r = v - __builtin_convertvector(hi, f32x4);
diff --git a/discogan_modernized_amd/csrc/edge.hip b/discogan_modernized_amd/csrc/edge.hip
--- a/discogan_modernized_amd/csrc/edge.hip
+++ b/discogan_modernized_amd/csrc/edge.hip
@@ -165,7 +165,7 @@
 #define CS_PR (CS_TR + 2)
 #define CS_PC 16
 #define CS_LDP 52
-template <bool IN16, bool MF16 = false, bool X3 = false, bool FACT = false>
+template <bool IN16, bool MF16 = false, bool X3 = false, bool FACT = false, bool BNL = false>
 __global__ __launch_bounds__(256, 2) void c3_dgrad_scatter_kernel(const DgPtrs dys, const DgPtrs ws_, const DgPtrs dxs, int N, int H, int W, int act,
                                                                   int tiles_r, int tiles_c, int ntiles, unsigned dybytes, const DgPtrs aos, float slope) {
     const float* __restrict__ dy = dg_pick<const float>(dys, blockIdx.y);
@@ -173,9 +173,11 @@
     float* __restrict__ dx = dg_pick<float>(dxs, blockIdx.y);
     static_assert(!MF16 || IN16, "the bf16 MFMA form takes a bf16 dy");
     static_assert(!X3 || (!IN16 && !MF16), "the f32x3 form takes an fp32 dy");
+    static_assert(!BNL || (!IN16 && !FACT), "the on-load BatchNorm form takes an fp32 dy and fuses nothing else");
     typedef __bf16 bf16x8_d __attribute__((ext_vector_type(8)));
     typedef float f32x8_d __attribute__((ext_vector_type(8)));
     __shared__ __attribute__((aligned(16))) float Ps[CS_PR * CS_PC * CS_LDP];
+    __shared__ __attribute__((aligned(16))) float bnS[BNL ? 3 * CD_K : 4];
     const int tid = threadIdx.x, lane = tid & 63, wave = tid >> 6;
     const int p = lane & 15, kq = lane >> 4;
     const int Ho = H >> 1, Wo = W >> 1;
@@ -259,11 +261,42 @@
     };
     fetch(blockIdx.x, 0);
     apply_act(0);
+    if constexpr (BNL) {
+        const float* saved = (const float*)aos.p[0];
+        if (tid < CD_K) {
+            bnS[tid] = saved[tid];
+            bnS[CD_K + tid] = ((const float*)aos.p[1])[tid] * saved[CD_K + tid];
+            bnS[2 * CD_K + tid] = ((const float*)aos.p[2])[tid];
+        }
+        __syncthreads();
+    }
+    auto apply_bn = [&](int t, int set) {
+        if constexpr (BNL) {
+            const int tc = t % tiles_c, tr = (t / tiles_c) % tiles_r;
+            const int b = tc * CS_TC - 1 + p;
+            bool ok[2];
+#pragma unroll
+            for (int g = 0; g < 2; ++g) ok[g] = (unsigned)(tr * CS_TR - 1 + wave + 4 * g) < (unsigned)Ho && (unsigned)b < (unsigned)Wo;
+#pragma unroll
+            for (int j = 0; j < 4; ++j) {
+                const int k0 = X3 ? 32 * (j >> 1) + 8 * kq + 4 * (j & 1) : 16 * kq + 4 * j;
+                const f32x4 mean = *(const f32x4*)(bnS + k0), gs = *(const f32x4*)(bnS + CD_K + k0), beta = *(const f32x4*)(bnS + 2 * CD_K + k0);
+#pragma unroll
+                for (int g = 0; g < 2; ++g)
+#pragma unroll
+                    for (int e = 0; e < 4; ++e) {
+                        const float z = dg_apply_act(bn_norm(areg[set][g][j][e], mean[e], gs[e], beta[e]), DG_ACT_RELU, 0.f);
+                        areg[set][g][j][e] = ok[g] ? z : 0.f;
+                    }
+            }
+        }
+    };
     auto tile = [&](auto SB, int t) {
         constexpr int S = decltype(SB)::value;
         const int tc = t % tiles_c, tr = (t / tiles_c) % tiles_r, n = t / (tiles_c * tiles_r);
         const int a0 = tr * CS_TR, b0 = tc * CS_TC;
         fetch(t + gridDim.x, S ^ 1);
+        apply_bn(t, S);
         f32x4 acc[2][3];
 #pragma unroll
         for (int g = 0; g < 2; ++g)
@@ -360,6 +393,7 @@
     int dy_bf16, N, H, W, K, act, prec;
     const void* act_out;
     float slope;
+    const float *bn_saved, *bn_gamma, *bn_beta;
     void* ws;
     size_t ws_bytes;
     hipStream_t st;
@@ -405,6 +439,24 @@
 
 static bool c3_dgrad_scatter_fits(int N, int H, int W, int K, int dy_bf16) {
     return K == CD_K && N >= 1 && (long)N * (H / 2) * (W / 2) * CD_K * (dy_bf16 ? 2 : 4) < (1L << 31);
+}
+static bool c3_bn_prec_ok(int prec) {
+    const int p = dg_resolve_prec(prec);
+    return prec >= DG_PREC_DEFAULT && (p == DG_PREC_F32 || p == DG_PREC_F32X3);
+}
+extern "C" int dg_c3_dgrad_bn_ok(int N, int H, int W, int K, int prec) {
+    return c3_dgrad_scatter_fits(N, H, W, K, 0) && dg_get_option(DG_OPT_KT) != 16 && c3_bn_prec_ok(prec) ? 1 : 0;
+}
+extern "C" int dg_conv4x4s2_c3_dgrad_bn_p(const float* y_nhwc, const float* saved, const float* gamma, const float* beta, int bn_act, const float* w,
+                                          float* dx_nchw, int N, int H, int W, int K, int act, int prec, dg_stream_t stream) {
+    C3_CHECK_PREC("dg_conv4x4s2_c3_dgrad_bn_p", prec);
+    DG_CHECK_ARG(saved && gamma && beta && bn_act == DG_ACT_RELU, "dg_conv4x4s2_c3_dgrad_bn_p: needs saved, gamma, beta and a ReLU (bn_act=%d)", bn_act);
+    DG_CHECK_ARG(dg_c3_dgrad_bn_ok(N, H, W, K, prec), "dg_conv4x4s2_c3_dgrad_bn_p: no on-load form for N=%d H=%d W=%d K=%d prec=%d (dg_c3_dgrad_bn_ok)", N,
+                 H, W, K, prec);
+    const void* y = y_nhwc;
+    C3Dgrad c = c3_dgrad_call("dg_conv4x4s2_c3_dgrad_bn_p", &y, 0, &w, &dx_nchw, N, H, W, K, act, prec, nullptr, 0, stream);
+    c.bn_saved = saved; c.bn_gamma = gamma; c.bn_beta = beta;
+    return c3_dgrad(c);
 }
 extern "C" int dg_c3_dgrad_act_ok(int N, int H, int W, int K, int dy_bf16) {
     return c3_dgrad_scatter_fits(N, H, W, K, dy_bf16) && dg_get_option(DG_OPT_KT) != 16 ? 1 : 0;
@@ -444,7 +496,13 @@
                                    dim3(256), 0, c.st, pd, pw, px, N, H, W, c.act, tiles_r, tiles_c, (int)ntiles, dyb, pa, c.slope);
             });
         };
-        if (c.dy_bf16 && c.prec == DG_PREC_BF16) scatter(C3Yes{}, C3Yes{}, C3No{});
+        auto scatter_bn = [&](auto X3) {
+            const void* bn[3] = {c.bn_saved, c.bn_gamma, c.bn_beta};
+            hipLaunchKernelGGL((c3_dgrad_scatter_kernel<false, false, decltype(X3)::value, false, true>), grid, dim3(256), 0, c.st, pd, pw, px, N, H, W, c.act,
+                               tiles_r, tiles_c, (int)ntiles, dyb, dg_ptrs(bn, 3), 0.f);
+        };
+        if (c.bn_saved) c3_with_flag(c.prec == DG_PREC_F32X3, scatter_bn);
+        else if (c.dy_bf16 && c.prec == DG_PREC_BF16) scatter(C3Yes{}, C3Yes{}, C3No{});
         else if (c.dy_bf16) scatter(C3Yes{}, C3No{}, C3No{});
         else if (c.prec == DG_PREC_F32X3) scatter(C3No{}, C3No{}, C3Yes{});
         else scatter(C3No{}, C3No{}, C3No{});
@@ -818,7 +876,7 @@
 }
 
 #define CW_B 8
-template <bool BUF, bool FACT, bool IN16 = false>
+template <bool BUF, bool FACT, bool IN16 = false, bool BNL = false>
 __global__ __launch_bounds__(256, 2) void c3_wgrad_mfma_kernel(const DgPtrs dys, const DgPtrs xs, const DgPtrs parts, int N, int H, int W, int K,
                                                                int lgHo, int lgWo, long npix, int pix_per_wave,
                                                                const DgPtrs act_outs, float slope) {
@@ -926,21 +984,39 @@
             }
         }
     };
-    auto mma_batch = [&](int set) {
+    static_assert(!BNL || (BUF && !FACT && !IN16), "the on-load BatchNorm form: buffer path, fp32 dy, nothing else fused");
+    float bn_mean[2], bn_gs[2], bn_beta[2];
+    if constexpr (BNL) {
+        const float* saved = (const float*)act_outs.p[0];
+#pragma unroll
+        for (int i = 0; i < 2; ++i) {
+            const int ch = kg * 64 + l31 + 32 * i;
+            bn_mean[i] = saved[ch];
+            bn_gs[i] = ((const float*)act_outs.p[1])[ch] * saved[K + ch];
+            bn_beta[i] = ((const float*)act_outs.p[2])[ch];
+        }
+    }
+    auto mma_batch = [&](int set, long p0) {
 #pragma unroll
         for (int st = 0; st < CW_B; ++st)
 #pragma unroll
-            for (int i = 0; i < 2; ++i)
+            for (int i = 0; i < 2; ++i) {
+                float a = fa[set][st][i];
+                if constexpr (BNL) {
+                    a = dg_apply_act(bn_norm(a, bn_mean[i], bn_gs[i], bn_beta[i]), DG_ACT_RELU, 0.f);
+                    a = p0 + 2 * st + lh < p_end ? a : 0.f;
+                }
 #pragma unroll
                 for (int jn = 0; jn < 2; ++jn)
-                    acc[i][jn] = __builtin_amdgcn_mfma_f32_32x32x2f32(fa[set][st][i], fb[set][st][jn], acc[i][jn], 0, 0, 0);
+                    acc[i][jn] = __builtin_amdgcn_mfma_f32_32x32x2f32(a, fb[set][st][jn], acc[i][jn], 0, 0, 0);
+            }
     };
     load_batch(0, p_begin);
     for (long p0 = p_begin; p0 < p_end; p0 += 4 * CW_B) {
         load_batch(1, p0 + 2 * CW_B);
-        mma_batch(0);
+        mma_batch(0, p0);
         load_batch(0, p0 + 4 * CW_B);
-        mma_batch(1);
+        mma_batch(1, p0 + 2 * CW_B);
     }
     __shared__ float slabS[4][64 * 48];
 #pragma unroll
@@ -1090,7 +1166,7 @@
     f(std::integral_constant<int, 2>{});
     f(std::integral_constant<int, 3>{});
 }
-template <bool FACT, bool X3 = false>
+template <bool FACT, bool X3 = false, bool BNL = false>
 __global__ __launch_bounds__(256, X3 ? 1 : 2) void c3_wgrad_lds_kernel(const DgPtrs dys, const DgPtrs xs, const DgPtrs parts, int N, int H, int W, int K,
                                                               long npix, int rows_per_wg, const DgPtrs act_outs, float slope) {
     const float* __restrict__ dy = dg_pick<const float>(dys, blockIdx.z);
@@ -1198,12 +1274,28 @@
         pl[1] = __builtin_convertvector(r1, bf16x8_l);
         pl[2] = __builtin_convertvector(r1 - __builtin_convertvector(pl[1], f32x8_l), bf16x8_l);
     };
+    static_assert(!BNL || (X3 && !FACT), "the on-load BatchNorm form: f32x3, nothing else fused");
+    float bn_mean[2], bn_gs[2], bn_beta[2];
+    if constexpr (BNL) {
+        const float* saved = (const float*)act_outs.p[0];
+#pragma unroll
+        for (int i = 0; i < 2; ++i) {
+            const int ch = kg * 64 + 2 * l31 + i;
+            bn_mean[i] = saved[ch];
+            bn_gs[i] = ((const float*)act_outs.p[1])[ch] * saved[K + ch];
+            bn_beta[i] = ((const float*)act_outs.p[2])[ch];
+        }
+    }
     auto mma_x3 = [&](int set, int st, int b) {
         if constexpr (X3) {
             f32x8_l a0, a1;
 #pragma unroll
             for (int t = 0; t < 8; ++t) {
                 f32x2_w v = fa2[set][t];
+                if constexpr (BNL) {
+                    v[0] = dg_apply_act(bn_norm(v[0], bn_mean[0], bn_gs[0], bn_beta[0]), DG_ACT_RELU, 0.f);
+                    v[1] = dg_apply_act(bn_norm(v[1], bn_mean[1], bn_gs[1], bn_beta[1]), DG_ACT_RELU, 0.f);
+                }
                 if constexpr (FACT) {
                     const f32x2_w o = fo2[set][t];
                     v[0] = o[0] > 0.f ? v[0] : v[0] * slope;
@@ -1376,6 +1468,7 @@
     const void* const* act_out;
     int act;
     float slope;
+    const float *bn_saved, *bn_gamma, *bn_beta;
     float* const* dw;
     int io_bf16, N, H, W, K, prec, accumulate;
     void* const* ws;
@@ -1422,6 +1515,23 @@
     C3Wgrad c = c3_wgrad_call("dg_conv4x4s2_c3_wgrad_g", (const void* const*)dy_nhwc, (const void* const*)act_out_nhwc, 0, act, slope, x_nchw, dw, N, H, W, K,
                               prec, accumulate, ws, ws_bytes, stream);
     c.groups = groups; c.share = share;
+    return c3_wgrad(c);
+}
+static bool c3_wgrad_buf(const C3Wgrad& c);
+extern "C" int dg_c3_wgrad_bn_ok(int N, int H, int W, int K, int prec) {
+    C3Wgrad c = C3Wgrad();
+    c.N = N; c.H = H; c.W = W; c.K = K;
+    return K == 64 && N >= 1 && H >= 2 && W >= 32 && c3_wgrad_buf(c) && c3_bn_prec_ok(prec) ? 1 : 0;
+}
+extern "C" int dg_conv4x4s2_c3_wgrad_bn_p(const float* y_nhwc, const float* saved, const float* gamma, const float* beta, int bn_act, const float* x_nchw,
+                                          float* dw, int N, int H, int W, int K, int prec, int accumulate, void* ws, size_t ws_bytes, dg_stream_t stream) {
+    C3_CHECK_PREC("dg_conv4x4s2_c3_wgrad_bn_p", prec);
+    DG_CHECK_ARG(saved && gamma && beta && bn_act == DG_ACT_RELU, "dg_conv4x4s2_c3_wgrad_bn_p: needs saved, gamma, beta and a ReLU (bn_act=%d)", bn_act);
+    DG_CHECK_ARG(dg_c3_wgrad_bn_ok(N, H, W, K, prec), "dg_conv4x4s2_c3_wgrad_bn_p: no on-load form for N=%d H=%d W=%d K=%d prec=%d (dg_c3_wgrad_bn_ok)", N,
+                 H, W, K, prec);
+    const void* y = y_nhwc;
+    C3Wgrad c = c3_wgrad_call("dg_conv4x4s2_c3_wgrad_bn_p", &y, nullptr, 0, DG_ACT_NONE, 0.f, &x_nchw, &dw, N, H, W, K, prec, accumulate, &ws, ws_bytes, stream);
+    c.bn_saved = saved; c.bn_gamma = gamma; c.bn_beta = beta;
     return c3_wgrad(c);
 }
 static int c3_wgrad_reduce_g(int groups, int share, void* const* ws_tab, float* const* dw_tab, int nb, int total, int accumulate, hipStream_t st) {
@@ -1485,6 +1595,15 @@
                                N, H, W, K, lgHo, lgWo, npix, ppw, pao, slope);
         });
     };
+    if (c.bn_saved) {
+        const void* bn[3] = {c.bn_saved, c.bn_gamma, c.bn_beta};
+        const DgPtrs pbn = dg_ptrs(bn, 3);
+        if (form == C3_WGRAD_LDS_X3)
+            hipLaunchKernelGGL((c3_wgrad_lds_kernel<false, true, true>), grid, dim3(256), 0, c.st, pdy, px, pws, N, H, W, K, npix, rpw, pbn, 0.f);
+        else
+            hipLaunchKernelGGL((c3_wgrad_mfma_kernel<true, false, false, true>), grid, dim3(256), 0, c.st, pdy, px, pws, N, H, W, K, lgHo, lgWo, npix, ppw, pbn,
+                               0.f);
+    } else
     switch (form) {
     case C3_WGRAD_LDS_X3: lds(C3Yes{}); break;
     case C3_WGRAD_LDS_BF16: lds(C3No{}); break;
diff --git a/discogan_modernized_amd/csrc/norm_act.hip b/discogan_modernized_amd/csrc/norm_act.hip
--- a/discogan_modernized_amd/csrc/norm_act.hip
+++ b/discogan_modernized_amd/csrc/norm_act.hip
@@ -40,7 +40,6 @@
     for (int h = 0; h < V / 4; ++h) *(f32x4*)(p + 4 * h) = (f32x4){v[4 * h], v[4 * h + 1], v[4 * h + 2], v[4 * h + 3]};
 }
 
-__device__ __forceinline__ float bn_norm(float y, float mean, float gs, float beta) { return fmaf(y - mean, gs, beta); }
 
 struct BnProb {
     const void* y;
diff --git a/discogan_modernized_amd/functional.py b/discogan_modernized_amd/functional.py
--- a/discogan_modernized_amd/functional.py
+++ b/discogan_modernized_amd/functional.py
@@ -242,6 +242,54 @@
                                            planes_only=ctx.dy_po)
         return (dy, dgamma if ctx.needs_input_grad[1] else None, dbeta if ctx.needs_input_grad[2] else None,
                 None, None, None, None, None, None, None, None, None, None, None, None, None)
+
+
+class BatchNormActConvTransposeC3Fn(Function):
+
+    @_fwd
+    def forward(ctx, y, gamma, beta, running_mean, running_var, nbt, training, eps, momentum, bn_act, partials, w, act, dy_cm=False, dy_po=False):
+        y = ops.as_nhwc(y)
+        if training and partials is not None and partials.numel() > 0:
+            saved = ops.bn_stats_from_partials(partials, y, running_mean, running_var, nbt, eps, momentum)
+        elif training:
+            saved = ops.bn_train_stats(y, running_mean, running_var, nbt, eps, momentum)
+        else:
+            saved = torch.stack([running_mean, torch.rsqrt(running_var + eps)])
+        out = ops.c3_dgrad_bn(y, saved, gamma, beta, w, act, bn_act)
+        ctx.save_for_backward(y, saved, gamma, beta, w, out)
+        ctx.cfg = (bn_act, act, training, bool(dy_cm), bool(dy_po))
+        ctx.prefs = (gamma, beta)
+        ctx.wref = w
+        ctx.final = FINAL_PASS
+        return out
+
+    @_bwd
+    def backward(ctx, dout):
+        y, saved, gamma, beta, w, out = ctx.saved_tensors
+        bn_act, act, training, dy_cm, dy_po = ctx.cfg
+        if not training:
+            raise RuntimeError("BatchNormActConvTransposeC3Fn: backward in eval mode is not supported")
+        none = (None,) * 15
+        g = ops.act_bwd(dout, out, act) if act != ops.ACT_NONE else dout.contiguous()
+        need_p = ctx.needs_input_grad[1] or ctx.needs_input_grad[2]
+        dz = ops.c3_fwd(g, w, ops.ACT_NONE) if ctx.needs_input_grad[0] or need_p else None
+        dw = None
+        if ctx.needs_input_grad[11]:
+            fg = _flat_grad_of(ctx.wref)
+            if fg is not None and fg.is_contiguous():
+                ops.c3_wgrad_bn(y, saved, gamma, beta, g, out=fg, accumulate=True, bn_act=bn_act)
+                _final(ctx.final, ctx.wref)
+            else:
+                dw = ops.c3_wgrad_bn(y, saved, gamma, beta, g, bn_act=bn_act)
+        if dz is None:
+            return none[:11] + (dw,) + none[12:]
+        fgm, fb = _flat_grad_of(ctx.prefs[0]), _flat_grad_of(ctx.prefs[1])
+        if need_p and fgm is not None and fb is not None:
+            dy, _, _ = ops.bn_act_bwd(dz, y, saved, gamma, beta, bn_act, 0.0, out_grads=(fgm, fb), planes_cm=dy_cm, planes_only=dy_po)
+            _final(ctx.final, ctx.prefs[0], ctx.prefs[1])
+            return (dy,) + none[1:11] + (dw,) + none[12:]
+        dy, dgamma, dbeta = ops.bn_act_bwd(dz, y, saved, gamma, beta, bn_act, 0.0, need_param_grads=need_p, planes_cm=dy_cm, planes_only=dy_po)
+        return (dy, dgamma if ctx.needs_input_grad[1] else None, dbeta if ctx.needs_input_grad[2] else None) + none[3:11] + (dw,) + none[12:]
 
 
 class ActFn(Function):
diff --git a/discogan_modernized_amd/model.py b/discogan_modernized_amd/model.py
--- a/discogan_modernized_amd/model.py
+++ b/discogan_modernized_amd/model.py
@@ -201,6 +201,28 @@
     return torch.is_grad_enabled() and nxt.weight.requires_grad and ops._x3_ok(2, n, h // 2, w // 2, nxt.in_channels, nxt.out_channels, 2, 1)
 
 
+TAIL_BN_ONLOAD = __import__("os").environ.get("DG_TAIL_BN_ONLOAD", "1") != "0"
+
+
+def _tail_onload(y, bn, act_mod, rest):
+    if not (TAIL_BN_ONLOAD and isinstance(act_mod, ReLU) and 1 <= len(rest) <= 2):
+        return None
+    convT = rest[0]
+    if not (isinstance(convT, ConvTranspose2d) and convT.out_channels == 3 and convT.stride == 2) or \
+            (len(rest) == 2 and not isinstance(rest[1], Sigmoid)):
+        return None
+    if any(m._forward_hooks or m._forward_pre_hooks for m in (bn, act_mod, *rest)):
+        return None
+    need_wgrad = torch.is_grad_enabled() and convT.weight.requires_grad
+    return rest if ops.c3_tail_bn_ok(y, need_wgrad) else None
+
+
+def _tail_apply(y, bn, act, st, tail, dy_cm=False, dy_po=False):
+    return F.BatchNormActConvTransposeC3Fn.apply(y, bn.weight, bn.bias, bn.running_mean, bn.running_var, bn.num_batches_tracked, bn.training,
+                                                 bn.eps, bn.momentum, act, st, tail[0].weight, tail[1].act if len(tail) == 2 else ops.ACT_NONE,
+                                                 dy_cm, dy_po)
+
+
 def drain(gen):
     try:
         while True:
@@ -224,6 +246,10 @@
         slope = act_mod.negative_slope if act_mod is not None else 0.0
         if bn is not None and bn.training and not ops.X3 and _fuse_stats(conv, x) and conv.emits_bn_stats:
             y, st = conv(x, want_stats=_fuse_stats(conv, x))
+            tail = _tail_onload(y, bn, act_mod, layers[j + 1:])
+            if tail is not None:
+                yield
+                return _tail_apply(y, bn, act, st, tail)
             x = bn(y, act, slope, st)
         elif bn is not None:
             nxt = layers[j + (1 if act_mod is not None else 0)] if j + (1 if act_mod is not None else 0) < n else None
@@ -235,6 +261,9 @@
             else:
                 y = conv(x)
             yield
+            tail = _tail_onload(y, bn, act_mod, layers[j + 1:])
+            if tail is not None:
+                return _tail_apply(y, bn, act, st, tail, dy_cm, dy_po)
             x = bn(y, act, slope, st, z_cm, dy_cm, z_po, dy_po)
         elif isinstance(conv, Conv2d) and conv.in_channels == 3 and act in (ops.ACT_LEAKY, ops.ACT_RELU, ops.ACT_NONE):
             nxt = layers[j + (1 if act_mod is not None else 0)] if j + (1 if act_mod is not None else 0) < n else None
diff --git a/discogan_modernized_amd/ops.py b/discogan_modernized_amd/ops.py
--- a/discogan_modernized_amd/ops.py
+++ b/discogan_modernized_amd/ops.py
@@ -663,6 +663,42 @@
     return dw
 
 
+def c3_tail_bn_ok(y, need_wgrad=True):
+    if _is16(y) or _CUR.act16 or _CUR.shadow:
+        return False
+    n, k, ho, wo = y.shape
+    L = _lib.load()
+    return bool(L.dg_c3_dgrad_bn_ok(n, 2 * ho, 2 * wo, k, _CUR.cprec)) and \
+        (not need_wgrad or bool(L.dg_c3_wgrad_bn_ok(n, 2 * ho, 2 * wo, k, _CUR.cprec)))
+
+
+def c3_dgrad_bn(y, saved, gamma, beta, w, act=ACT_NONE, bn_act=ACT_RELU):
+    _check_dev(y, saved, gamma, beta, w)
+    y = as_nhwc(y)
+    w = w.contiguous()
+    n, k, ho, wo = y.shape
+    dx = torch.empty((n, 3, 2 * ho, 2 * wo), device=y.device, dtype=torch.float32)
+    with _hbm("edge_c3_dgrad", 4.0 * y.numel() + 4.0 * dx.numel()):
+        _lib.check(_lib.load().dg_conv4x4s2_c3_dgrad_bn_p(_ptr(y), _ptr(saved), _ptr(gamma), _ptr(beta), bn_act, _ptr(w), _ptr(dx), n, 2 * ho, 2 * wo,
+                                                          k, act, _CUR.cprec, _stream()), "dg_conv4x4s2_c3_dgrad_bn_p")
+    return dx
+
+
+def c3_wgrad_bn(y, saved, gamma, beta, x_nchw, out=None, accumulate=False, bn_act=ACT_RELU):
+    _check_dev(y, saved, gamma, beta, x_nchw)
+    y = as_nhwc(y)
+    x = x_nchw.contiguous()
+    n, k, ho, wo = y.shape
+    h, wd = x.shape[2], x.shape[3]
+    dw = out if out is not None else torch.empty((k, 3, 4, 4), device=y.device, dtype=torch.float32)
+    L = _lib.load()
+    ws, wsb = _ws(L.dg_c3_wgrad_workspace_bytes(n, h, wd, k), y.device)
+    with _hbm("edge_c3_wgrad", 4.0 * y.numel() + 4.0 * x.numel()):
+        _lib.check(L.dg_conv4x4s2_c3_wgrad_bn_p(_ptr(y), _ptr(saved), _ptr(gamma), _ptr(beta), bn_act, _ptr(x), _ptr(dw), n, h, wd, k, _CUR.cprec,
+                                                int(accumulate), _ptr(ws), wsb, _stream()), "dg_conv4x4s2_c3_wgrad_bn_p")
+    return dw
+
+
 def bn_train_stats(y, running_mean, running_var, nbt, eps, momentum):
     _check_dev(y, allow16=True)
     y = as_nhwc(y)
diff --git a/include/discogan_hip.h b/include/discogan_hip.h
--- a/include/discogan_hip.h
+++ b/include/discogan_hip.h
@@ -114,6 +114,12 @@
 int dg_c3_dgrad_act_ok(int N, int H, int W, int K, int dy_bf16);
 int dg_conv4x4s2_c3_dgrad_act_p(const void* dy_nhwc, int dy_bf16, const void* act_out_nhwc, int in_act, float slope, const float* w,
                                 float* dx_nchw, int N, int H, int W, int K, int act, int prec, void* ws, size_t ws_bytes, dg_stream_t s);
+int dg_c3_dgrad_bn_ok(int N, int H, int W, int K, int prec);
+int dg_conv4x4s2_c3_dgrad_bn_p(const float* y_nhwc, const float* saved, const float* gamma, const float* beta, int bn_act, const float* w,
+                               float* dx_nchw, int N, int H, int W, int K, int act, int prec, dg_stream_t s);
+int dg_c3_wgrad_bn_ok(int N, int H, int W, int K, int prec);
+int dg_conv4x4s2_c3_wgrad_bn_p(const float* y_nhwc, const float* saved, const float* gamma, const float* beta, int bn_act, const float* x_nchw,
+                               float* dw, int N, int H, int W, int K, int prec, int accumulate, void* ws, size_t ws_bytes, dg_stream_t s);
 int dg_conv4x4s2_c3_fwd_g(int groups, const float* const* x_nchw, const float* const* w, float* const* y_nhwc, int N, int H, int W, int K,
                           int act, float slope, int prec, dg_stream_t s);
 int dg_conv4x4s2_c3_dgrad_g(int groups, const float* const* dy_nhwc, const float* const* w, float* const* dx_nchw, int N, int H, int W, int K,
```

New measurement: 300.5 images/s, median of 6. 1.01x the previous value.
